# Excalibur1224/Cuda-v-MPI

Hardware: AMD Instinct MI355X
Metric: Riemann subintervals/sec at N=1e9 fp64; |error| vs analytic π (higher is better)
Workload: dtype fp64

## Files before the change

csrc/cli/miint.cpp:

```cpp
#include <algorithm>
#include <cmath>
#include <cstdio>
#include <string>
#include <vector>

#include "cli_common.hpp"
#include "miint/integrator.hpp"
#include "miint/oracle.hpp"
#include "miint/table2d.hpp"
#include "miint/trainscan.hpp"

using namespace miint;

namespace {

struct BenchRow {
  std::string integrand, dtype, rule;
  double n = 0, result = 0, exact = 0, ms = 0;
  int gpus = 1;
  int block = 0, grid = 0;
  bool multistep = false, close_in_launch = false, allreduce_to_host = false;
  BatchDiag diag;
  std::string timeline_file;
  std::string timeline_work;
// ... 200 lines not shown
}

int comm_sweep(const cli::Args& a, const cli::Topology& topo, double max_bytes, int iters) {
  std::vector<size_t> counts;
  for (size_t c = 1; c * 8.0 <= max_bytes; c *= 8) counts.push_back(c);
  if (counts.empty() || counts.back() * 8.0 < max_bytes) counts.push_back(static_cast<size_t>(max_bytes / 8));
  const char* ops[] = {"allreduce", "allgather", "broadcast"};
  std::vector<double> ms(counts.size() * 3, 0.0);
  std::mutex mu;
  auto body = [&](int , int dev, const Comm* comm) {
    DeviceGuard g(dev);
    Stream s;
    RankAgree agree(comm);
    const size_t cmax = counts.back();
    DeviceBuffer<double> a(cmax), b(cmax * static_cast<size_t>(comm->world()));
    MIINT_HIP(hipMemsetAsync(a.get(), 0, a.bytes(), s.get()));
    Event e0, e1;
    for (size_t k = 0; k < counts.size(); ++k)
      for (int op = 0; op < 3; ++op) {
        auto issue = [&] {
          if (op == 0) comm->allreduce_sum(a.get(), b.get(), counts[k], s.get());
          else if (op == 1) comm->allgather(a.get(), b.get(), counts[k], s.get());
          else comm->broadcast(a.get(), counts[k], 0, s.get());
        };
        for (int w = 0; w < 3; ++w) issue();
        s.sync();
        agree.barrier();
        e0.record(s.get());
        for (int i = 0; i < iters; ++i) issue();
        e1.record(s.get());
        e1.sync();
        comm->check_async();
        const double t = agree.max(Event::elapsed_ms(e0, e1) / iters);
        std::lock_guard<std::mutex> l(mu);
        ms[k * 3 + op] = std::max(ms[k * 3 + op], t);
      }
  };
  capture_rccl_log();
  if (!topo.multiproc && topo.world == 1) {
    auto one = RcclComm::init_all({0});
    body(0, 0, one[0].get());
  } else {
    cli::run_ranks(topo, body);
  }
  if (topo.rank0 != 0) return 0;
  const double P = topo.world;
  const RcclTransport tr = rccl_transport();
  const bool share = ranks_share_devices() && topo.world > 1;
  const std::string terr = transport_error(
      tr, topo.world, topo.multiproc ? cli::env_int("LOCAL_WORLD_SIZE", topo.world) : topo.world,
      share);
  if (!terr.empty()) std::fprintf(stderr, "miint comm: transport check: %s\n", terr.c_str());
  for (size_t k = 0; k < counts.size(); ++k)
    for (int op = 0; op < 3; ++op) {
      const double bytes = counts[k] * 8.0 * (op == 1 ? P : 1.0);
      const double t = ms[k * 3 + op];
      const double alg = bytes / (t * 1e-3) / 1e9;
      const double factor = op == 0 ? 2.0 * (P - 1) / P : (op == 1 ? (P - 1) / P : 1.0);
      cli::emit(a, cli::JsonRecord()
                       .add("op", ops[op])
                       .add("gpus", topo.world)
                       .add("bytes", bytes)
                       .add("us", t * 1e3)
                       .add("algbw_GBps", alg)
                       .add("busbw_GBps", alg * factor)
                       .add("ranks_share_gpus", ranks_share_devices() && topo.world > 1)
                       .add("rccl_transport", tr.transport)
                       .add("rccl_nnodes", tr.nnodes)
                       .add("transport_verified", terr.empty()),
                true);
    }
  return 0;
}

}

constexpr const char* kUsage =
    "usage: miint info\n"
    "       miint bench [--integrand pi4] [--n 1e9] [--dtype fp64|fp32|fp32acc] [--rule left]\n"
    "                   [--iters 200] [--gpus G] [--div series_exact|series|ieee] [--unfused] [--no-graph]\n"
    "                   [--block B] [--grid G] [--step-streams S] [--trig-library] [--settle N]\n"
    "                   [--no-multistep] [--slots K] [--close auto|kernel|launch] [--no-ar-host]\n"
    "                   [--work auto|static|queue] [--queue-wg-per-cu W]\n"
    "                   [--diagnose] [--slice R/W] [--timeline FILE]\n"
    "                   (--timeline: after the timed run, one batch from the timeline build of\n"
    "                   the multi-step launch, per-workgroup device-clock stamps as JSON in FILE;\n"
    "                   read it with tools/timeline_report.py. --slice: rank R's share of W)\n"
    "       miint sweep [--gpus G]\n"
    "       miint table2d [--grid 4096] [--gpus G] [--slice R/W] [--no-graph]\n"
    "                     [--step-streams S] [--min-wg W] [--settle-ms MS] [--no-multistep]\n"
    "                     [--phases P] [--graph-steps K]\n"
    "       miint selfcheck\n"
    "       miint comm [--gpus G] [--max-bytes 144e6] [--iters 20]\n"
    "Every record is one JSON line on stdout; --jsonl FILE also appends it to FILE.\n";

int main(int argc, char** argv) {
  try {
    cli::Args a(argc, argv);
    if (cli::usage_requested(a, kUsage)) return 0;
    const std::string cmd = a.positional().empty() ? "info" : a.positional()[0];
    if (cmd == "info") {
      const int nd = device_count();
      std::printf("miint: %d HIP device(s), RCCL %s\n", nd, nd ? RcclComm::version().c_str() : "-");
      for (int d = 0; d < nd; ++d) {
        const DeviceInfo i = device_info(d);
        std::printf("  [%d] %s %s  %d CUs  %.1f GHz  %.1f GB  L2 %d KB  LDS %zu KB/CU (%zu KB/block)\n",
                    d, i.name.c_str(), i.arch.c_str(), i.num_cus, i.clock_khz / 1e6,
                    i.total_mem / 1e9, i.l2_bytes / 1024, i.lds_per_cu / 1024,
                    i.lds_per_block / 1024);
      }
      return 0;
    }
    if (cmd == "selfcheck") return selfcheck();
    {
      int r = 0, w = 0;
      cli::parse_slice(a, &r, &w);
    }
    const cli::Topology topo = cli::topology(a);
    const int iters = static_cast<int>(a.integer("iters", 100));
    const bool graphs = !a.flag("no-graph");
    if (cmd == "bench") {
      RiemannConfig c = make_cfg(a.str("integrand", "pi4"), a.num("n", 1e9), a.str("dtype", "fp64"),
                                 a.str("rule", "left"), a.str("div", "series_exact"));
      c.fused = !a.flag("unfused");
      c.grid = static_cast<int>(a.integer("grid", 0));
      c.block = static_cast<int>(a.integer("block", kRiemannBlock));
      c.step_streams = static_cast<int>(a.integer("step-streams", 0));
      c.multistep = !a.flag("no-multistep");
      c.slots = static_cast<int>(a.integer("slots", c.slots));
      c.close = a.str("close", c.close);
      c.work = a.str("work", c.work);
      c.queue_wg_per_cu = static_cast<int>(a.integer("queue-wg-per-cu", 0));
      c.allreduce_to_host = !a.flag("no-ar-host");
      cli::parse_slice(a, &c.slice_rank, &c.slice_world);
      TimelineRequest tl;
      tl.file = a.str("timeline", "");
      tl.integrand = a.str("integrand", "pi4");
      tl.dtype = a.str("dtype", "fp64");
      tl.div = a.str("div", "series_exact");
      if (!tl.file.empty() && c.close == "launch")
        fail(std::string("--timeline: ") + kTimelineNoCloseInLaunch, __FILE__, __LINE__);
      if (a.flag("trig-library")) set_trig_library(true);
      MIINT_CHECK(riemann_block_ok(c.block), "--block must be 64, 128, 256, 512 or 1024");
      c.waves_per_cu = static_cast<int>(a.integer("waves-per-cu", 32));
      const BenchRow r = bench_one(topo, c, iters, graphs,
                                   static_cast<int>(a.integer("settle", -1)),
                                   a.flag("diagnose"), tl);
      if (topo.rank0 == 0)
        print_row(a, r, a.str("integrand", "pi4").c_str(), a.str("dtype", "fp64").c_str(),
                  a.str("rule", "left").c_str());
      return 0;
    }
    if (cmd == "table2d") {
      Table2DConfig c;
      c.grid = static_cast<int>(a.integer("grid", 4096));
      c.bucket = !a.flag("no-bucket");
      c.chain = !a.flag("no-chain");
      c.step_streams = static_cast<int>(a.integer("step-streams", 0));
      c.min_wg = static_cast<int>(a.integer("min-wg", 0));
      c.settle_ms = a.num("settle-ms", c.settle_ms);
      c.multistep = !a.flag("no-multistep");
      c.phases = static_cast<int>(a.integer("phases", 0));
      c.graph_steps = static_cast<int>(a.integer("graph-steps", 0));
      cli::parse_slice(a, &c.rank, &c.world);
      double value = 0.0, timed = 0.0, ms = 0.0;
      bool bucketed = false, chained = false, multistep = false;
      int streams = 1, phases = 0, resident = 0, min_wg = 0, wgs = 0, gsteps = 0;
      cli::RankFacts facts;
      std::mutex mu;
      cli::run_ranks(topo, [&](int rank, int dev, const Comm* comm) {
        Table2DPlan plan(c, dev, comm);
        RankAgree agree(comm);
        const double v = plan.run();
        const double t = agree.max(plan.time(iters, graphs));
        std::lock_guard<std::mutex> g(mu);
        if (rank == topo.rank0) {
          facts.note(comm);
          value = v;
          timed = plan.last_result();
          bucketed = plan.bucketed() && graphs;
          chained = plan.chained() && graphs;
          multistep = plan.multistep() && graphs;
          streams = chained ? plan.step_streams() : 1;
          phases = multistep ? plan.phases() : 0;
          resident = plan.resident_per_cu();
          min_wg = plan.min_wg();
          wgs = plan.workgroups();
          gsteps = graphs ? plan.graph_steps() : 0;
        }
        if (t > ms) ms = t;
      });
      if (topo.rank0 == 0) {
        cli::JsonRecord r;
        r.add("program", "table2d").add("grid", c.grid);
        r.add("step_streams", streams).add("multistep", multistep).add("phases", phases);
        r.add("resident_per_cu", resident).add("min_wg", min_wg).add("workgroups", wgs);
        r.add("graph_steps", gsteps);
        facts.add(r, topo);
        if (c.world > 1) {
          r.add("slice", std::to_string(c.rank) + "/" + std::to_string(c.world))
              .add("partial", value);
        } else {
          const double want = table2d_oracle(c.grid);
          const double exact = 122000.004 * 122000.004;
          r.add("gpus", topo.world)
              .add("result", value)
              .add("timed_result", timed)
              .add("bucketed_allreduce", bucketed)
              .add("chained", chained)
              .add("midpoint_oracle", want)
              .add("rel_err_vs_oracle", std::fabs(value - want) / want)
              .add("rel_err_vs_exact", std::fabs(value - exact) / exact)
              .add("samples_per_s", static_cast<double>(c.grid) * c.grid / (ms * 1e-3));
        }
// ... 29 lines not shown
```

csrc/include/miint/common.hpp:

```cpp
#pragma once

#include <hip/hip_runtime.h>

#include <cstdint>
#include <stdexcept>
#include <string>

namespace miint {

struct Error : std::runtime_error {
  using std::runtime_error::runtime_error;
};

[[noreturn]] inline void fail(const std::string& what, const char* file, int line) {
  throw Error(std::string(file) + ":" + std::to_string(line) + ": " + what);
}

}

#define MIINT_HIP(expr)                                                                     \
  do {                                                                                      \
    hipError_t miint_e_ = (expr);                                                           \
    if (miint_e_ != hipSuccess)                                                             \
      ::miint::fail(std::string(#expr) + " -> " + hipGetErrorString(miint_e_), __FILE__,    \
                    __LINE__);                                                              \
  } while (0)

#define MIINT_CHECK(cond, msg)                                                   \
  do {                                                                           \
    if (!(cond)) ::miint::fail(std::string("check failed: ") + (msg), __FILE__, __LINE__); \
  } while (0)

namespace miint {

enum class Integrand : int {
  kPi4 = 0,
  kSin = 1,
  kPoly = 2,
  kTrainVel = 3,
  kTable = 4,
};

enum class Rule : int { kLeft = 0, kMid = 1, kRight = 2 };

enum class DivMode : int { kSeries = 0, kIeee = 1, kSeriesDirect = 2, kSeriesExact = 3 };

inline double rule_offset(Rule r) {
  return r == Rule::kLeft ? 0.0 : (r == Rule::kMid ? 0.5 : 1.0);
}

constexpr int kMaxPolyCoeffs = 16;

constexpr int kSinTrig = 28;

struct RiemannParams {
  double a;
  double h;
  double off;
  uint64_t i_begin;
  uint64_t n;
  int integrand;
  int ncoef;
  double coef[kMaxPolyCoeffs];
  double coef_h[kMaxPolyCoeffs];
  double p0, p1;
  double trig[kSinTrig];
  float trig32[kSinTrig];
};

}
```

csrc/include/miint/integrands.hpp:

```cpp
#pragma once

#include <hip/hip_runtime.h>

#include "miint/common.hpp"
#include "miint/fast_trig.hpp"

namespace miint {

template <class D>
struct TileDefaults {
  template <DivMode M>
  __host__ __device__ static constexpr int tile_len() { return 32; }
  template <int U, DivMode M>
  __device__ static constexpr double anchor() { return 0.0; }
  template <int U, DivMode M>
  __device__ __forceinline__ double tile_acc(double x0, double h, double acc) const {
    return acc + static_cast<const D*>(this)->template tile<U, M>(x0, h);
  }
};

struct Pi4 : TileDefaults<Pi4> {
  static constexpr double kScale = 4.0;
  static constexpr int kPairs = 16;
  static constexpr int kSub = 2 * kPairs;
// ... 229 lines not shown
#pragma unroll
      for (int q = 0; q < kSubs; ++q) {
        const int i = q < kSubs / 2 ? kSubs / 2 - 1 - q : q - kSubs / 2;
        if (q < kSubs / 2) {
          ecs[i] = centres_f32(sf, i);
          aqs[i] = slopes_f32(sf, i);
        }
        if (q == 0) subtile_squares<true, true>(t2, tb, aqs[i], ecs[i]);
        else if (q < kSubs / 2) subtile_squares<true, false>(t2, tb, aqs[i], ecs[i]);
        else subtile_squares<false, false>(t2, tb, aqs[i], ecs[i]);
      }
      t2 += tb;
#else
#pragma unroll
      for (int q = 0; q < kSubs; ++q) {
        const int i = q < kSubs / 2 ? kSubs / 2 - 1 - q : q - kSubs / 2;
        if (q < kSubs / 2) {
          ecs[i] = centres_f32(sf, i);
          aqs[i] = slopes_f32(sf, i);
        }
        const float ecq = q < kSubs / 2 ? ecs[i].y : ecs[i].x;
        const float aq = q < kSubs / 2 ? aqs[i].y : aqs[i].x;
        const f32x2 ec = {ecq, ecq}, a = {aq, aq};
#pragma unroll
        for (int j = 0; j < kPairs; ++j) {
          const f32x2 e = __builtin_elementwise_fma(pkf[j], a, ec);
          t2 = __builtin_elementwise_fma(e, e, t2);
          asm volatile("" : "+v"(t2));
        }
      }
#endif
      const double t = lin + (static_cast<double>(t2.x) + static_cast<double>(t2.y));
      return fma(sd.s, t, fma(sd.s, static_cast<double>(U), acc));
    } else {
      return acc + tile<U, M>(xa, h);
    }
  }

  __device__ __forceinline__ double series_exact_point(double xm, double h, int u) const {
    const Seed sd = seed_exact(xm, h);
    const double b2 = 2.0 * sd.b;
    const int q = u / kSub, w = u % kSub;
    const double ec = centre_g(sd, q);
    const double a = centre_slope(sd, b2, q);
    const int j = w >= kSub / 2 ? w - kSub / 2 : kSub / 2 - 1 - w;
    const double kj = w >= kSub / 2 ? pk[j] : -pk[j];
    const double e = fma(kj, a, fma(fma(kj, kj, -kMeanK2), sd.b, ec));
    const SeedF32 sf = seed_f32(sd);
    const int i = q < kSubs / 2 ? kSubs / 2 - 1 - q : q - kSubs / 2;
    const f32x2 ecs = centres_f32(sf, i), aqs = slopes_f32(sf, i);
    const float e_sq = fmaf(static_cast<float>(kj), q < kSubs / 2 ? aqs.y : aqs.x,
                            q < kSubs / 2 ? ecs.y : ecs.x);
    const float sq = e_sq * e_sq;
    return fma(sd.s, e + static_cast<double>(sq), sd.s);
  }

  __device__ __forceinline__ double series_point(double xm, double h, int u) const {
    const Seed sd = seed_half(xm, h);
    const double b2 = 2.0 * sd.b;
    const int q = u / kSub, w = u % kSub;
    const double eh = centre_g(sd, q);
    const double a = centre_slope(sd, b2, q);
    const int j = w >= kSub / 2 ? w - kSub / 2 : kSub / 2 - 1 - w;
    const double c = fma(pk2[j], sd.b, eh);
    const double g = w >= kSub / 2 ? fma(pk[j], a, c) : fma(-pk[j], a, c);
    return sd.s * fma(g, g, 0.75);
  }
};

struct Pi4Wide : TileDefaults<Pi4Wide> {
  static constexpr double kScale = 4.0;
  __device__ __forceinline__ double point(double x) const { return 1.0 / fma(x, x, 1.0); }
  template <int U, DivMode M>
  __device__ __forceinline__ double tile(double x0, double h) const {
    static_assert(M == DivMode::kIeee, "wide-domain Pi4 runs IEEE division only");
    double acc = 0.0;
#pragma unroll
    for (int u = 0; u < U; ++u) acc += point(fma(static_cast<double>(u), h, x0));
    return acc;
  }
};
constexpr double kPi4NarrowMaxX = 0x1p249;

__device__ __forceinline__ void tile_sincos(double th, double& S, double& C) {
  constexpr double kTwoOverPi = 6.36619772367581382433e-01;
  constexpr double kPio2Hi = 1.57079632673412561417e+00;
  constexpr double kPio2Lo = 6.07710050650619224932e-11;
  const double n = rint(th * kTwoOverPi);
  const double r = fma(-n, kPio2Lo, fma(-n, kPio2Hi, th));
  const int q = static_cast<int>(n);
  const double z = r * r, w = z * z;
  const double s26 = fma(z, fma(z, fma(z, fma(z, 1.58969099521155010221e-10,
                                                -2.50507602534068634195e-08),
                                           2.75573137070700676789e-06),
                                      -1.98412698298579493134e-04),
                         8.33333333332248946124e-03);
  const double sr = fma(r * z, fma(z, s26, -1.66666666666666324348e-01), r);
  const double c13 = fma(z, fma(z, 2.48015872894767294178e-05, -1.38888888888741095749e-03),
                         4.16666666666666019037e-02);
  const double c46 = fma(z, fma(z, -1.13596475577881948265e-11, 2.08757232129817482790e-09),
                         -2.75573143513906633035e-07);
  const double rc = fma(w * w, c46, z * c13);
  const double hz = 0.5 * z, cw = 1.0 - hz;
  const double cc = cw + (((1.0 - cw) - hz) + z * rc);
  const bool swap = (q & 1) != 0;
  const double a = swap ? cc : sr, b = swap ? sr : cc;
  S = (q & 2) ? -a : a;
  C = ((q + 1) & 2) ? -b : b;
}

template <int Subs>
struct AngleSeries {
  static constexpr int kPairs = 8;
  static constexpr int kSub = 2 * kPairs;
  static constexpr int kSubs = Subs;
  static constexpr int kSeriesTile = kSub * kSubs;
  static_assert(2 * kPairs + kSubs <= kSinTrig, "RiemannParams::trig layout");
  double ck[kPairs], sk[kPairs];
  double cc[kSubs / 2], sc[kSubs / 2];

  __device__ __forceinline__ void init_trig(const double* trig) {
#pragma unroll
    for (int j = 0; j < kPairs; ++j) {
      ck[j] = trig[j];
      sk[j] = trig[kPairs + j];
    }
#pragma unroll
    for (int i = 0; i < kSubs / 2; ++i) {
      cc[i] = trig[2 * kPairs + 2 * i];
      sc[i] = trig[2 * kPairs + 2 * i + 1];
    }
  }
  __device__ __forceinline__ void centre(double S, double C, int q, double& Sq,
                                         double& Cq) const {
    const int i = q < kSubs / 2 ? kSubs / 2 - 1 - q : q - kSubs / 2;
    const double c = cc[i], s = q < kSubs / 2 ? -sc[i] : sc[i];
    Sq = fma(C, s, S * c);
    Cq = fma(-S, s, C * c);
  }
  template <bool COS>
  __device__ __forceinline__ double tile_sum(double theta_m) const {
    double S, C;
    tile_sincos(theta_m, S, C);
    double t = 0.0;
#pragma unroll
    for (int q = 0; q < kSubs; ++q) {
      double Sq, Cq;
      centre(S, C, q, Sq, Cq);
      const double base = COS ? Cq : Sq, side = COS ? -Sq : Cq;
#pragma unroll
      for (int j = 0; j < kPairs; ++j) {
        const double u = base * ck[j];
        t += fma(side, sk[j], u);
        t += fma(-side, sk[j], u);
        asm volatile("" : "+v"(t));
      }
    }
    return t;
  }
  template <bool COS>
  __device__ __forceinline__ double point_of(double theta_m, int u) const {
    double S, C, Sq, Cq;
    tile_sincos(theta_m, S, C);
    const int q = u / kSub, w = u % kSub;
    centre(S, C, q, Sq, Cq);
    const double base = COS ? Cq : Sq, side = COS ? -Sq : Cq;
// ... 420 lines not shown
```

csrc/include/miint/integrator.hpp:

```cpp
#pragma once

#include <hip/hip_runtime.h>

#include <cstdint>
#include <map>
#include <memory>
#include <string>
#include <vector>

#include "miint/comm.hpp"
#include "miint/common.hpp"
#include "miint/kernels.hpp"
#include "miint/runtime.hpp"

namespace miint {

constexpr int kAutoStepStreams = 4;
constexpr uint64_t kStepStreamsMaxCount = 600000000ull;

struct RiemannConfig {
  Integrand integrand = Integrand::kPi4;
  double a = 0.0, b = 1.0;
  uint64_t n = 1000000000ull;
  Rule rule = Rule::kLeft;
  DType dtype = DType::kF64;
  DivMode div = DivMode::kSeriesExact;
  std::vector<double> coef;
  double p0 = 0.0, p1 = 0.0;
  std::vector<double> table;
  int grid = 0;
  int block = kRiemannBlock;
  int waves_per_cu = 32;
  bool fused = true;
  bool chain = true;
  bool host_direct = true;
  int slots = 16;
  bool bucket = true;
  int rank = 0, world = 1;
  bool force_collective = false;
  bool multistep = true;
  std::string close = "auto";
  std::string work = "auto";
  int queue_wg_per_cu = 0;
  bool allreduce_to_host = true;
  int step_streams = 0;
  int slice_rank = 0, slice_world = 0;
  double timeout_s = 300.0;
};

inline std::string resolve_work(const std::string& work, const char* env, bool pays,
                                bool keeps_static = false) {
  MIINT_CHECK(work == "auto" || work == "static" || work == "queue",
              "work must be auto, static or queue (got " + work + ")");
  if (keeps_static) return "static";
  if (work != "auto") return work;
  if (env && *env) {
    const std::string e(env);
    MIINT_CHECK(e == "static" || e == "queue", "MIINT_MS_WORK must be static or queue (got " + e + ")");
    return e;
  }
  return pays ? "queue" : "static";
}

inline void rank_slice(uint64_t n, int r, int w, uint64_t* begin, uint64_t* count) {
  const uint64_t q = n / static_cast<uint64_t>(w), rem = n % static_cast<uint64_t>(w);
  const uint64_t ur = static_cast<uint64_t>(r);
  *count = q + (ur < rem ? 1 : 0);
  *begin = ur * q + (ur < rem ? ur : rem);
}

struct StepTiming {
  double wall_s = 0.0;
  double device_ms = 0.0;
  int steps = 0;
};

struct OneShotTiming {
  std::string mode;
  int reps = 0;
  double median_us = 0.0, min_us = 0.0, max_us = 0.0;
  double device_median_us = 0.0, device_min_us = 0.0;
  double value = 0.0;
};

struct BatchDiag {
  int steps = 0;
  double compute_us = 0.0;
  double close_us = 0.0;
  double allreduce_us = 0.0;
  double copy_us = 0.0;
  double marker_us = 0.0;
  double device_us = 0.0;
  double staged_us = 0.0;
  double wall_us = 0.0;
  double tail_us() const { return close_us + allreduce_us + copy_us; }
  double boundary_us() const { return device_us - compute_us - tail_us(); }
};

struct BatchTimeline {
  int steps = 0, grid = 0, block = 0;
  int clock_khz = 0;
  std::vector<uint64_t> stamps;
  std::vector<uint64_t> shader_clock;
  std::vector<uint32_t> hw;
  double device_us = 0.0;
  std::vector<double> values;
  std::string work = "static";
  int workgroups = 0;
  std::vector<uint64_t> wg_stamps;
  std::vector<uint64_t> item_stamp;
  std::vector<uint32_t> item_owner;
};
constexpr uint64_t kTimelineUnsetStamp = 0;
constexpr uint32_t kTimelineUnsetId = 0xffffffffu;

class RiemannPlan {
 public:
  RiemannPlan(const RiemannConfig& cfg, int device, const Comm* comm = nullptr);
  ~RiemannPlan();
  RiemannPlan(const RiemannPlan&) = delete;
  RiemannPlan& operator=(const RiemannPlan&) = delete;

  const RiemannConfig& config() const { return cfg_; }
  int device() const { return device_; }
  int rank() const { return rank_; }
  int world() const { return world_; }
  uint64_t begin() const { return params_.i_begin; }
  uint64_t count() const { return params_.n; }
  double h() const { return params_.h; }
  double scale() const { return scale_; }
  LaunchShape shape() const { return shape_; }
  DivMode effective_div() const;
  bool direct() const { return direct_; }

  void enqueue_compute(hipStream_t s, int slot, int host_index) const;
  void enqueue_reduce(hipStream_t s, int slot) const;
  void enqueue_copyout(hipStream_t s, int slot, int host_index) const;
  void enqueue(hipStream_t s, int slot, int host_index) const;

  double* device_result(int slot) const { return result_.get() + slot; }
  double host_result(int host_index) const { return host_[host_index]; }
  int host_capacity() const { return static_cast<int>(host_.size()); }
  int slots() const { return cfg_.slots; }

  double run();
  void capture_graphs();
  void prepare_steps(int steps);
  bool graphs_ready() const { return !graphs_.empty() && graph_error_.empty(); }
  const std::string& graph_error() const { return graph_error_; }
  size_t graph_nodes() const;
  long graph_launches() const { return graph_launches_; }
  long direct_steps() const { return direct_steps_; }

  StepTiming run_steps(int steps, bool pipeline, bool graphs);
  BatchDiag diagnose_batch(int nsteps);
  BatchTimeline timeline_batch(int nsteps, const std::string& form = "auto");
  void barrier();
  OneShotTiming time_one_shot(int reps, const std::string& mode, int warmup = 400);
  void launch_steps(int steps, bool pipeline, bool graphs);
  void sync() const;
  int host_index_of(int k, bool graphs) const;
  hipStream_t compute_stream() const { return compute_.get(); }
  hipStream_t comm_stream() const { return comm_stream_.get(); }

  bool collective() const { return comm_ && (world_ > 1 || cfg_.force_collective); }
  bool bucketed() const { return collective() && cfg_.bucket; }
  bool chained() const { return cfg_.fused && cfg_.chain && (!collective() || bucketed()); }
  bool multistep() const { return chained() && multistep_; }
  bool close_in_launch() const { return multistep() && close_launch_; }
  const char* work() const { return multistep() && work_queue_ ? "queue" : "static"; }
  int queue_workgroups() const { return multistep() && work_queue_ ? queue_wgs_ : 0; }
  bool allreduce_to_host() const {
    return bucketed() && cfg_.allreduce_to_host && ar_host_ok_;
  }
  void check_allreduce_to_host();

 private:
  void enqueue_batch(hipStream_t cs, hipStream_t rs, int nsteps, bool overlap);
  void enqueue_bucket_reduce(hipStream_t s, int nsteps) const;
  void enqueue_chain(hipStream_t s, int nsteps) const;
  void enqueue_chain_streams(hipStream_t cs, int nsteps);
 public:
  int step_streams(int nsteps) const;
 private:
  const Graph* batch_graph(int nsteps);
  bool use_graphs(bool requested, int steps);
  double* result_ptr(int j) const { return direct_ ? host_.device_ptr() + j : result_.get() + j; }

  RiemannConfig cfg_;
  int device_;
  const Comm* comm_;
  int rank_ = 0, world_ = 1;
  bool direct_ = false;
  RiemannParams params_{};
  double scale_ = 1.0;
  LaunchShape shape_{1, kRiemannBlock};
  DeviceBuffer<double> partials_;
  DeviceBuffer<double> slots_;
  DeviceBuffer<double> ms_partials_;
  bool multistep_ = false;
  bool close_launch_ = false;
  bool capturing_ = false;
  bool ar_host_ok_ = true;
  bool ar_host_checked_ = false;
  DeviceBuffer<unsigned int> ms_ticket_;
  bool work_queue_ = false;
  int queue_wgs_ = 0;
  DeviceBuffer<unsigned int> queue_;
  void reset_queue() const;
  void enqueue_multistep(hipStream_t s, int nsteps, bool close_kernel) const;
  DeviceBuffer<uint64_t> qtl_item_stamp_, qtl_wg_stamps_, qtl_shader_;
  DeviceBuffer<uint32_t> qtl_item_owner_, qtl_hw_;
  DeviceBuffer<uint64_t> tl_stamps_, tl_shader_;
  DeviceBuffer<uint32_t> tl_hw_;
  DeviceBuffer<double> result_;
  DeviceBuffer<double> sync_;
  DeviceBuffer<unsigned int> ticket_;
  DeviceBuffer<double> table_;
  PinnedBuffer<double> host_;
  Stream compute_;
  Stream comm_stream_;
  std::vector<Stream> step_streams_;
  std::vector<std::unique_ptr<Event>> ev_step_join_;
  std::vector<std::unique_ptr<Event>> ev_computed_, ev_drained_;
  Event ev_fork_, ev_join_;
  Event ev_t0_, ev_t1_;
  std::map<int, std::unique_ptr<Graph>> graphs_;
  std::string graph_error_;
  long graph_launches_ = 0, direct_steps_ = 0;
  int last_mode_ = -1;
};

}
```

csrc/include/miint/kernels.hpp:

```cpp
#pragma once

#include <hip/hip_runtime.h>

#include <algorithm>
#include <cmath>
#include <cstddef>
#include <cstdint>

#include "miint/common.hpp"

namespace miint {

enum class DType : int { kF64 = 0, kF32 = 1, kF32Acc32 = 2 };
inline bool is_fp32(DType t) { return t == DType::kF32 || t == DType::kF32Acc32; }

constexpr int kRiemannTile = 32;
constexpr int kRiemannBlock = 256;
constexpr int kSeriesHalfSpan = 192;
constexpr int kSeriesHalfSpanF32 = 96;

constexpr int kDirectHalfSpan = 16;

inline bool series_ok(double h) { return kSeriesHalfSpan * (h < 0 ? -h : h) <= 2e-6; }
inline bool series_ok_f32(double h) { return kSeriesHalfSpanF32 * (h < 0 ? -h : h) <= 2e-6; }
inline bool direct_ok(double h) { return kDirectHalfSpan * (h < 0 ? -h : h) <= 2e-6; }

inline DivMode effective_div(DivMode d, double h) {
  if (d == DivMode::kIeee) return d;
  if ((d == DivMode::kSeries || d == DivMode::kSeriesExact) && series_ok(h)) return d;
  return direct_ok(h) ? DivMode::kSeriesDirect : DivMode::kIeee;
}
inline bool series_request(DivMode d) { return d == DivMode::kSeries || d == DivMode::kSeriesExact; }
inline DivMode effective_div(DivMode d, double h, Integrand f) {
  if (f == Integrand::kSin || f == Integrand::kTrainVel || f == Integrand::kTable)
    return series_request(d) ? DivMode::kSeries : DivMode::kIeee;
  if (f != Integrand::kPi4) return DivMode::kIeee;
  return effective_div(d, h);
}

constexpr int kPolySeriesMaxCoeffs = 8;

inline DivMode effective_div(DivMode d, double h, Integrand f, DType t, int ncoef = 0) {
  if (is_fp32(t)) {
    if (d == DivMode::kIeee) return DivMode::kIeee;
    if (f == Integrand::kPi4) return series_ok_f32(h) ? DivMode::kSeries : DivMode::kIeee;
    if (f == Integrand::kPoly)
      return (ncoef >= 1 && ncoef <= kPolySeriesMaxCoeffs) ? DivMode::kSeries : DivMode::kIeee;
    return DivMode::kSeries;
  }
  if (f == Integrand::kPoly)
    return (series_request(d) && ncoef >= 1 && ncoef <= kPolySeriesMaxCoeffs)
               ? DivMode::kSeries
               : DivMode::kIeee;
  return effective_div(d, h, f);
}

constexpr double kTrigSeriesMaxN = 2147418112.0;
inline bool trig_series_in_range(const RiemannParams& p) {
  const Integrand f = static_cast<Integrand>(p.integrand);
  if (f != Integrand::kSin && f != Integrand::kTrainVel) return true;
  const double first = static_cast<double>(p.i_begin) + p.off;
  const double last = static_cast<double>(p.i_begin + (p.n > 0 ? p.n - 1 : 0)) + p.off;
  const double w = f == Integrand::kTrainVel ? 1.0 / p.p0 : 1.0;
  const double n0 = std::fabs(std::fma(first, p.h, p.a) * w) * 6.36619772367581382433e-01;
  const double n1 = std::fabs(std::fma(last, p.h, p.a) * w) * 6.36619772367581382433e-01;
  return n0 <= kTrigSeriesMaxN && n1 <= kTrigSeriesMaxN;
}
constexpr double kPi4SeriesMaxX = 0x1p249;
constexpr double kPi4SeriesMaxXF32 = 0x1p62;
inline bool pi4_series_in_range(const RiemannParams& p, DType t) {
  if (static_cast<Integrand>(p.integrand) != Integrand::kPi4) return true;
  const double lim = is_fp32(t) ? kPi4SeriesMaxXF32 : kPi4SeriesMaxX;
  const double first = static_cast<double>(p.i_begin) + p.off;
  const double last = static_cast<double>(p.i_begin + (p.n > 0 ? p.n - 1 : 0)) + p.off;
  return std::fabs(std::fma(first, p.h, p.a)) < lim && std::fabs(std::fma(last, p.h, p.a)) < lim;
}
inline bool poly_series_in_range(const RiemannParams& p) {
  if (static_cast<Integrand>(p.integrand) != Integrand::kPoly) return true;
  if (!(std::isfinite(p.h) && p.h != 0.0 && std::isfinite(1.0 / p.h))) return false;
  long double hp = 1.0L;
  for (int i = 0; i < p.ncoef && i < kMaxPolyCoeffs; ++i) {
    const double cs = static_cast<double>(static_cast<long double>(p.coef[i]) * hp);
    if (p.coef[i] != 0.0 && !std::isnormal(cs)) return false;
    hp *= static_cast<long double>(p.h);
  }
  return true;
}
inline DivMode effective_div(const RiemannParams& p, DivMode d, DType t) {
  const DivMode e = effective_div(d, p.h, static_cast<Integrand>(p.integrand), t, p.ncoef);
  return (e != DivMode::kIeee &&
          !(trig_series_in_range(p) && pi4_series_in_range(p, t) && poly_series_in_range(p)))
             ? DivMode::kIeee
             : e;
}

struct LaunchShape {
  int grid;
  int block;
};

bool riemann_block_ok(int block);
LaunchShape default_riemann_shape(int num_cus, int waves_per_cu = 32, int block = kRiemannBlock);

void launch_riemann_partials(const RiemannParams& p, DType dtype, DivMode div,
                             LaunchShape shape, const double* table, int table_n,
                             double* partials, hipStream_t stream);

void launch_finalize(const double* partials, int n, double scale, double* out,
                     hipStream_t stream, int block = kRiemannBlock);

constexpr unsigned kUnsetSlotWord = 0xFFFAFFFAu;
void fill_unset_slots(double* p, size_t count, hipStream_t stream);

constexpr int kTicketGroups = 16;
constexpr int kTicketStride = 64;
constexpr int kTicketWords = (kTicketGroups + 1) * kTicketStride;

void launch_riemann_fused(const RiemannParams& p, DType dtype, DivMode div, LaunchShape shape,
                          const double* table, int table_n, double* partials,
                          unsigned int* ticket, double scale, double* out, hipStream_t stream);

void launch_riemann_chained(const RiemannParams& p, DType dtype, DivMode div, LaunchShape shape,
                            const double* table, int table_n, double* partials,
                            const double* prev, int nprev, double scale, double* out_prev,
                            hipStream_t stream);

constexpr int kMaxMultiSteps = 64;
int riemann_multistep_grid(const RiemannParams& p, DType dtype, DivMode div, int block,
                           int num_cus, bool close = false);
void launch_riemann_multistep(const RiemannParams& p, DType dtype, DivMode div,
                              LaunchShape shape, const double* table, int table_n,
                              double* partials, int steps, double scale, double* out,
                              hipStream_t stream, unsigned int* ticket = nullptr,
                              bool close_kernel = true);
constexpr const char* kTimelineNoCloseInLaunch =
    "the timeline instruments the kernel-closed multi-step launch only (not close = launch)";
int riemann_timeline_grid(const RiemannParams& p, DType dtype, DivMode div, int block,
                          int num_cus);
void launch_riemann_timeline(const RiemannParams& p, DType dtype, DivMode div,
                             LaunchShape shape, const double* table, int table_n,
                             double* partials, int steps, double scale, double* out,
                             hipStream_t stream, uint64_t* stamps, uint64_t* shader_clock,
                             uint32_t* hw, unsigned int* ticket = nullptr,
                             bool close_kernel = true);
constexpr int kQueueWords = 2 * kTicketStride;
struct QueueTimeline {
  uint64_t* item_stamp;
  uint32_t* item_owner;
  uint64_t* wg_stamps;
  uint64_t* shader_clock;
  uint32_t* hw;
};
int riemann_queue_grid(const RiemannParams& p, DType dtype, DivMode div, int block, int num_cus,
                       bool timeline = false);
bool riemann_queue_pays(const RiemannParams& p, DType dtype, DivMode div);
void launch_riemann_queue(const RiemannParams& p, DType dtype, DivMode div, LaunchShape shape,
                          int workgroups, const double* table, int table_n, double* partials,
                          int steps, double scale, double* out, hipStream_t stream,
                          unsigned int* queue, bool close_kernel = true,
                          const QueueTimeline* timeline = nullptr);
void launch_multistep_close(const double* partials, int grid, int steps, double scale,
                            double* out, int block, hipStream_t stream);

void launch_riemann_point_values(const RiemannParams& p, DivMode div, const double* table,
                                 int table_n, double* out, hipStream_t stream);

void launch_pi4_recip_narrow(const double* d, uint64_t n, double* out, hipStream_t stream);
void launch_pi4_recip_narrow_f32(const float* d, uint64_t n, float* out, hipStream_t stream);
void set_pi4_library_division(bool on);
bool pi4_ieee_narrow(const RiemannParams& p, DType dtype);
void set_trig_library(bool on);
void set_lds_poison(bool on);
void set_lds_poison_trainscan(bool on);
void set_lds_poison_table(bool on);

int riemann_tile_len(const RiemannParams& p, DType dtype, DivMode div);

double integrand_scale(Integrand f);

int default_reduce_grid(int num_cus);
void launch_sum_array(const double* x, uint64_t n, double scale, double* partials, int grid,
                      double* out, hipStream_t stream);

void launch_interp_fill(const double* table, int table_n, double dt, uint64_t i0, uint64_t n,
                        double* y, hipStream_t stream);

size_t scan_state_bytes(uint64_t n);
void launch_inclusive_scan(const double* in, double* out, uint64_t n, void* state,
                           const double* carry_in, hipStream_t stream);
void launch_interp_scan(const double* table, int table_n, double dt, uint64_t i0, uint64_t n,
                        double* out, void* state, const double* carry_in, hipStream_t stream);
void launch_interp_scan_window(const double* table, int table_n, double dt, uint64_t i0,
                               uint64_t n, uint64_t win_lo, uint64_t win_hi, double* out,
                               void* state, const double* carry_in, hipStream_t stream);
unsigned scan_timeout_flag(const void* state, hipStream_t stream);
void launch_add_carry(double* x, uint64_t n, const double* carry, hipStream_t stream);

struct Table2DParams {
  const double* table;
  int nx, ny;
  double X, Y;
  int gx, gy;
  int row0, row1;
  int min_wg = 0;
};
int table2d_grid(const Table2DParams& p);
const char* table2d_path(const Table2DParams& p);
struct Table2DShapeInfo {
  bool stream;
  int rows_per_wave, tile_rows, tile_cols, grid_x, grid_y, tile;
};
Table2DShapeInfo table2d_shape_info(const Table2DParams& p);
constexpr int kT2AutoPhases = 16;
constexpr long kT2AutoWorkgroups = 4096;
constexpr int kT2MaxPhases = 32;
constexpr int kT2MaxReplaySteps = 1024;
bool table2d_multistep_ok(const Table2DParams& p, int num_cus);
int table2d_multistep_resident(const Table2DParams& p);
int table2d_multistep_phases(const Table2DParams& p, int num_cus, int steps, int want = 0);
void launch_table2d_multistep(const Table2DParams& p, double* partials, int steps, double* outs,
                              hipStream_t stream, int phases = 1);
void launch_table2d_partials(const Table2DParams& p, double* partials, hipStream_t stream);
void launch_table2d_fused(const Table2DParams& p, double* partials, unsigned* ticket,
                          double* out, hipStream_t stream);
void launch_table2d_chained(const Table2DParams& p, double* partials, const double* prev,
                            double* prev_out, hipStream_t stream);
void launch_table2d_finalize(const double* partials, int n, double* out, hipStream_t stream);
void launch_outer_product(const double* v, int n, double* table, hipStream_t stream);

}
```

csrc/kernels/riemann.hip:

```cpp
#include <hip/hip_runtime.h>

#include <atomic>
#include <cmath>
#include <string>

#include "miint/common.hpp"
#include "miint/handoff.hpp"
#include "miint/integrands.hpp"
#include "miint/integrands_f32.hpp"
#include "miint/kernels.hpp"
#include "miint/wave_reduce.hpp"

namespace miint {
namespace {

constexpr int B = kRiemannBlock;
constexpr int kMaxBlock = 1024;

__device__ __forceinline__ uint64_t readlane_u64(uint64_t v, int lane) {
  const uint32_t lo = __builtin_amdgcn_readlane(static_cast<uint32_t>(v), lane);
  const uint32_t hi = __builtin_amdgcn_readlane(static_cast<uint32_t>(v >> 32), lane);
  return (static_cast<uint64_t>(hi) << 32) | lo;
}

template <class F> struct AccOf { using type = double; };

struct TileSplit {
  uint64_t lanes, q;
  uint32_t bs, rem;
};
template <int T>
__device__ __forceinline__ TileSplit tile_split(uint64_t n) {
  const uint32_t bs = blockDim.x;
  const uint64_t lanes = static_cast<uint64_t>(gridDim.x) * bs;
  const uint64_t ntile = n / T;
  const uint64_t q = ntile / lanes;
  return {lanes, q, bs, static_cast<uint32_t>(ntile - q * lanes)};
}

template <DivMode M, class F>
__device__ __forceinline__ typename AccOf<F>::type lane_sum(const RiemannParams& p, const F& f,
                                                            unsigned block, const TileSplit& sp) {
  using Acc = typename AccOf<F>::type;
  constexpr int T = F::template tile_len<M>();
  const uint64_t lanes = sp.lanes;
  const uint32_t b0 = block * sp.bs;
  const uint32_t g32 = b0 + threadIdx.x;
  const uint64_t gid = g32;
  const uint32_t w0 =
      b0 + static_cast<uint32_t>(__builtin_amdgcn_readfirstlane(threadIdx.x / kWave)) * kWave;
  const bool all_extra = w0 + (kWave - 1) < sp.rem;
  const bool extra = !all_extra && g32 < sp.rem;
  const double base = static_cast<double>(p.i_begin) + p.off;
  const double istep = static_cast<double>(lanes * T);
  double ib = base + static_cast<double>(gid * T) + F::template anchor<T, M>();
  Acc acc = 0;
  for (uint64_t left = readlane_u64(sp.q + (all_extra ? 1 : 0), 0); left != 0; --left, ib += istep)
    acc = f.template tile_acc<T, M>(fma(ib, p.h, p.a), p.h, acc);
  if (extra) acc = f.template tile_acc<T, M>(fma(ib, p.h, p.a), p.h, acc);
  const uint64_t done = (sp.q * lanes + sp.rem) * T;
  for (uint64_t k = gid; k < p.n - done; k += lanes)
    acc += static_cast<Acc>(f.point(fma(base + static_cast<double>(done + k), p.h, p.a)));
  return acc;
}
template <DivMode M, class F>
__device__ __forceinline__ typename AccOf<F>::type lane_sum(const RiemannParams& p, const F& f,
                                                            unsigned block) {
  return lane_sum<M>(p, f, block, tile_split<F::template tile_len<M>()>(p.n));
}

constexpr int kMaxTable = 2048;


struct Pi4F32 : TileDefaults<Pi4F32> {
  static constexpr double kScale = 4.0;
  __device__ __forceinline__ double point(double xd) const {
    const float x = static_cast<float>(xd);
    return static_cast<double>(1.0f / fmaf(x, x, 1.0f));
  }
  __device__ __forceinline__ static f32x2 recip_narrow(f32x2 d) {
    const f32x2 one = {1.0f, 1.0f};
    const f32x2 nd = -d;
    f32x2 r = {__builtin_amdgcn_rcpf(d.x), __builtin_amdgcn_rcpf(d.y)};
    r = pk_fma(pk_fma(nd, r, one), r, r);
    const f32x2 q = pk_fma(pk_fma(nd, r, one), r, r);
    return pk_fma(pk_fma(nd, q, one), r, q);
// ... 111 lines not shown
      acc0 += 1.0f / fmaf(xa, xa, 1.0f);
      acc1 += 1.0f / fmaf(xb, xb, 1.0f);
    }
    return static_cast<double>(acc0) + static_cast<double>(acc1);
  }
  template <int UU, DivMode M>
  __device__ __forceinline__ double tile_acc(double x0d, double h, double acc) const {
    return acc + tile<UU, M>(x0d, h);
  }
};
constexpr double kPi4F32NarrowMaxX = 0x1p49;

struct Pi4F32Acc32 : Pi4F32 {
  template <int UU, DivMode M>
  __device__ __forceinline__ float tile_acc(double xmd, double h, float acc) const {
    if constexpr (M == DivMode::kSeries) {
      static_assert(UU == kSubs * kSubLen, "fp32 series tiles are kSubs 32-sample sub-tiles");
      const float xm = static_cast<float>(xmd);
      const float hf = static_cast<float>(h);
      const float dm = fmaf(xm, xm, 1.0f);
      float s = __builtin_amdgcn_rcpf(dm);
      s = fmaf(s, fmaf(-dm, s, 1.0f), s);
      const float em = fmaf(-dm, s, 1.0f);
      const float a = (-2.0f * hf) * xm * s;
      const float b = -(hf * hf) * s;
      const f32x2 bb = {b, b};
      const f32x2 aa = {a, a};
      const f32x2 emv = {em, em};
      f32x2 ecs[kSubs / 2], aqs[kSubs / 2];
#pragma unroll
      for (int p2 = 0; p2 < kSubs / 2; ++p2) {
        const f32x2 c0v = {(2 * p2 - 0.5f * (kSubs - 1)) * kSubLen,
                           (2 * p2 + 1 - 0.5f * (kSubs - 1)) * kSubLen};
        ecs[p2] = pk_fma(c0v, pk_fma(c0v, bb, aa), emv);
        aqs[p2] = pk_fma(c0v + c0v, bb, aa);
      }
      f32x2 t, t1;
#pragma unroll
      for (int q = 0; q < kSubs; ++q) {
        const float ec = (q & 1) ? ecs[q / 2].y : ecs[q / 2].x;
        const float aq = (q & 1) ? aqs[q / 2].y : aqs[q / 2].x;
        const f32x2 av = {aq, aq};
        f32x2 cc = pk_fma(f32x2{0.25f, 2.25f}, bb, f32x2{ec, ec});
#pragma unroll
        for (int j = 0; j < kSubLen / 2; j += 2) {
          const f32x2 k0 = {j + 0.5f, -(j + 0.5f)};
          const f32x2 k1 = {j + 1.5f, -(j + 1.5f)};
          const f32x2 e0 = pk_fma(k0, av, f32x2{cc.x, cc.x});
          const f32x2 e1 = pk_fma(k1, av, f32x2{cc.y, cc.y});
          if (q == 0 && j == 0) {
            t = e0;
            t1 = e1;
          } else {
            t += e0;
            t1 += e1;
          }
          if (j + 2 < kSubLen / 2)
            cc = pk_fma(f32x2{4.0f * j + 6.0f, 4.0f * j + 10.0f}, bb, cc);
        }
      }
      t += t1;
      return fmaf(s, static_cast<float>(UU) + (t.x + t.y), acc);
    } else {
      const float x0 = static_cast<float>(xmd);
      const float hf = static_cast<float>(h);
      const f32x2 xb = {x0, x0}, hh = {hf, hf}, one = {1.0f, 1.0f};
      f32x2 a2 = {0.0f, 0.0f};
#pragma unroll
      for (int u = 0; u < UU; u += 2) {
        const f32x2 uu = {static_cast<float>(u), static_cast<float>(u + 1)};
        const f32x2 x = pk_fma(uu, hh, xb);
        a2 += recip_narrow(pk_fma(x, x, one));
      }
      return acc + (a2.x + a2.y);
    }
  }
};
template <> struct AccOf<Pi4F32Acc32> { using type = float; };

static_assert(2 * AngleSeries<12>::kPairs + 12 == kSinTrig, "trig table sized for Sin");
static_assert(Pi4::kSeriesTile / 2 == kSeriesHalfSpan &&
                  Pi4F32::kSubs * Pi4F32::kSubLen / 2 == kSeriesHalfSpanF32,
              "kSeriesHalfSpan(F32) must be half the Pi4 series tile lengths");

template <class F> struct Maker;
template <> struct Maker<Pi4> {
  static constexpr int kLds = 1;
  __device__ static Pi4 make(const RiemannParams&, const double*, int, double*) {
    Pi4 f;
    f.init();
    return f;
  }
};
template <> struct Maker<Pi4Wide> {
  static constexpr int kLds = 1;
  __device__ static Pi4Wide make(const RiemannParams&, const double*, int, double*) { return {}; }
};
template <> struct Maker<Pi4F32Wide> {
  static constexpr int kLds = 1;
  __device__ static Pi4F32Wide make(const RiemannParams&, const double*, int, double*) {
    return {};
  }
};
template <> struct Maker<Pi4F32Acc32> {
  static constexpr int kLds = 1;
  __device__ static Pi4F32Acc32 make(const RiemannParams&, const double*, int, double*) {
    return {};
  }
};
template <> struct Maker<Pi4F32> {
  static constexpr int kLds = 1;
  __device__ static Pi4F32 make(const RiemannParams&, const double*, int, double*) { return {}; }
};
template <> struct Maker<Sin> {
  static constexpr int kLds = 1;
  __device__ static Sin make(const RiemannParams& p, const double*, int, double*) {
    Sin f;
    f.init(p.trig);
    return f;
  }
};
template <> struct Maker<SinLib> {
  static constexpr int kLds = 1;
  __device__ static SinLib make(const RiemannParams&, const double*, int, double*) { return {}; }
};
template <int NC> struct Maker<Poly<NC>> {
  static constexpr int kLds = 1;
  __device__ static Poly<NC> make(const RiemannParams& p, const double*, int, double*) {
    Poly<NC> f;
    f.init(p.coef, p.ncoef);
    return f;
  }
};
template <> struct Maker<TrainVel> {
  static constexpr int kLds = 1;
  __device__ static TrainVel make(const RiemannParams& p, const double*, int, double*) {
    TrainVel f;
    f.init_trig(p.trig);
    f.inv_ts = 1.0 / p.p0;
    f.vs = p.p1;
    return f;
  }
};
template <> struct Maker<TrainVelLib> {
  static constexpr int kLds = 1;
  __device__ static TrainVelLib make(const RiemannParams& p, const double*, int, double*) {
    TrainVelLib f;
    f.inv_ts = 1.0 / p.p0;
    f.vs = p.p1;
    return f;
  }
};
template <> struct Maker<SinF32> {
  static constexpr int kLds = 1;
  __device__ static SinF32 make(const RiemannParams& p, const double*, int, double*) {
    SinF32 f;
    f.init(p.trig32);
    return f;
  }
};
template <> struct Maker<TrainVelF32> {
  static constexpr int kLds = 1;
  __device__ static TrainVelF32 make(const RiemannParams& p, const double*, int, double*) {
    TrainVelF32 f;
    f.init_trig(p.trig32);
    f.inv_ts = 1.0 / p.p0;
    f.vs = p.p1;
    return f;
  }
};
template <int NC> struct Maker<PolyF32<NC>> {
  static constexpr int kLds = 1;
// ... 406 lines not shown
  unsigned* done = queue + kTicketStride;
  unsigned c = 0;
  if (threadIdx.x == 0) c = queue_claim(head);
  if (!one_wave) {
    if (threadIdx.x == 0) next_item[1] = c;
    __syncthreads();
    c = next_item[1];
  }
  unsigned i = __builtin_amdgcn_readfirstlane(c);
  unsigned sbase = 0;
  for (unsigned seq = 0; i < total; ++seq) {
    unsigned nxt = 0;
    if (threadIdx.x == 0) nxt = queue_claim(head);
    while (i - sbase >= nb) sbase += nb;
    const unsigned vb = i - sbase;
    RiemannParams q = p;
    asm volatile("" : "+s"(q.a));
    const Acc l = lane_sum<M>(q, f, vb, sp);
    asm volatile("" : "+v"(nxt));
    if (!one_wave && threadIdx.x == 0) next_item[seq & 1] = nxt;
    double v;
    if constexpr (__is_same(Acc, double)) v = block_sum_dyn(l, red[seq & 1]);
    else v = static_cast<double>(block_sum_dyn(l, red_acc[seq & 1]));
    if (threadIdx.x == 0) {
      if constexpr (TL) {
        unsigned wg = blockIdx.x;
        asm volatile("" : "+v"(wg));
        tl.item_stamp[i] = timeline_realtime_after(v);
        tl.item_owner[i] = wg;
      }
      partials[i] = v;
    }
    i = __builtin_amdgcn_readfirstlane(one_wave ? nxt : next_item[seq & 1]);
  }
  if (threadIdx.x == 0) {
    if constexpr (TL) {
      const unsigned long long t = timeline_realtime();
      unsigned long long* clk = timeline_row(tl.shader_clock, 2);
      clk[0] = te.clk;
      clk[1] = timeline_shader_clock();
      unsigned long long* st = timeline_row(tl.wg_stamps, 2);
      st[0] = te.t;
      st[1] = t;
      unsigned xcc, hw;
      asm volatile("s_getreg_b32 %0, hwreg(HW_REG_XCC_ID)" : "=s"(xcc));
      asm volatile("s_getreg_b32 %0, hwreg(HW_REG_HW_ID)" : "=s"(hw));
      unsigned* id = timeline_row(tl.hw, 2);
      id[0] = xcc;
      id[1] = hw;
    }
    const unsigned d = __hip_atomic_fetch_add(done, 1u, __ATOMIC_RELAXED, __HIP_MEMORY_SCOPE_AGENT);
    if (d == gridDim.x - 1) {
      __hip_atomic_store(head, 0u, __ATOMIC_RELAXED, __HIP_MEMORY_SCOPE_AGENT);
      __hip_atomic_store(done, 0u, __ATOMIC_RELAXED, __HIP_MEMORY_SCOPE_AGENT);
    }
  }
}
template <DivMode M, class F>
__global__ __launch_bounds__(kMaxBlock) void riemann_queue_kernel(
    RiemannParams p, const double* table, int table_n, double* partials, int steps, unsigned nb,
    unsigned* queue) {
  queue_body<M, F>(p, table, table_n, partials, steps, nb, queue);
}
template <DivMode M, class F>
__global__ __launch_bounds__(kMaxBlock) kFullOccupancy void riemann_queue_kernel_o8(
    RiemannParams p, const double* table, int table_n, double* partials, int steps, unsigned nb,
    unsigned* queue) {
  queue_body<M, F>(p, table, table_n, partials, steps, nb, queue);
}
template <DivMode M, class F>
__global__ __launch_bounds__(kMaxBlock) void riemann_queue_timeline_kernel(
    RiemannParams p, const double* table, int table_n, double* partials, int steps, unsigned nb,
    unsigned* queue, QueueTimelineOut tl) {
  queue_body<M, F, true>(p, table, table_n, partials, steps, nb, queue, tl);
}
template <DivMode M, class F>
__global__ __launch_bounds__(kMaxBlock) kFullOccupancy void riemann_queue_timeline_kernel_o8(
    RiemannParams p, const double* table, int table_n, double* partials, int steps, unsigned nb,
    unsigned* queue, QueueTimelineOut tl) {
  queue_body<M, F, true>(p, table, table_n, partials, steps, nb, queue, tl);
}
template <DivMode M, class F>
constexpr bool queue_pays() {
  return M == DivMode::kSeriesExact && __is_same(F, Pi4);
}

__global__ __launch_bounds__(kMaxBlock) void multistep_close_kernel(const double* partials,
                                                                   int nb, double scale,
                                                                   double* out) {
  __shared__ double red[kMaxBlock / kWave];
  const double t = ordered_partials<0, false>(partials + static_cast<size_t>(blockIdx.x) * nb, nb);
  const double tot = block_sum_dyn(t, red);
  if (threadIdx.x == 0) out[blockIdx.x] = tot * scale;
}

template <DivMode M, class F>
__global__ __launch_bounds__(B) void point_values_kernel(RiemannParams p, const double* table,
                                                         int table_n, double* out) {
  constexpr int T = F::template tile_len<M>();
  __shared__ double lds[lds_words<M, F>()];
  const F f = make_functor<M, F>(p, table, table_n, lds);
  const uint64_t t = static_cast<uint64_t>(blockIdx.x) * B + threadIdx.x;
  if (t * T >= p.n) return;
  const double x0 = fma(static_cast<double>(p.i_begin) + p.off + static_cast<double>(t * T),
                        p.h, p.a);
  const double xm = fma(0.5 * (T - 1), p.h, x0);
  const bool full = (t + 1) * T <= p.n;
  for (int u = 0; u < T && t * T + u < p.n; ++u) {
    const double x = fma(static_cast<double>(u), p.h, x0);
    double v;
    if constexpr (M == DivMode::kSeries && __is_same(F, Pi4)) {
      v = full ? f.series_point(xm, p.h, u) : f.point(x);
    } else if constexpr (M == DivMode::kSeriesExact && __is_same(F, Pi4)) {
      v = full ? f.series_exact_point(xm, p.h, u) : f.point(x);
    } else if constexpr (M == DivMode::kSeries && IsPolyF64<F>::value) {
      v = full ? f.series_point(xm, u) : f.point(x);
    } else if constexpr (M == DivMode::kSeries && __is_same(F, Table)) {
      v = full ? f.series_point(xm, p.h, u) : f.point(x);
    } else if constexpr (M == DivMode::kSeries && (__is_same(F, Sin) || __is_same(F, TrainVel))) {
      v = full ? f.series_point(xm, u) : f.point(x);
    } else if constexpr (M == DivMode::kSeriesDirect && __is_same(F, Pi4)) {
      const Pi4::Seed sd = Pi4::seed(xm, p.h);
      const double e = fma(-fma(x, x, 1.0), sd.s, 1.0);
      v = fma(sd.s, e + e * e, sd.s);
    } else if constexpr (M == DivMode::kIeee && __is_same(F, Pi4)) {
      v = full ? Pi4::recip_narrow(fma(x, x, 1.0)) : f.point(x);
    } else if constexpr (M == DivMode::kIeee &&
                         (__is_same(F, Sin) || __is_same(F, SinLib) ||
                          __is_same(F, TrainVel) || __is_same(F, TrainVelLib))) {
      v = full ? f.template ieee_point<T>(x0, p.h, u) : f.point(x);
    } else {
      v = f.point(x);
    }
    out[t * T + u] = v * F::kScale;
  }
}

__global__ __launch_bounds__(B) void recip_narrow_kernel(const double* d, uint64_t n,
                                                         double* out) {
  const uint64_t stride = static_cast<uint64_t>(gridDim.x) * B;
  for (uint64_t i = static_cast<uint64_t>(blockIdx.x) * B + threadIdx.x; i < n; i += stride)
    out[i] = Pi4::recip_narrow(d[i]);
}
__global__ __launch_bounds__(B) void recip_narrow_f32_kernel(const float* d, uint64_t n,
                                                             float* out) {
  const uint64_t stride = static_cast<uint64_t>(gridDim.x) * B;
  for (uint64_t i = static_cast<uint64_t>(blockIdx.x) * B + threadIdx.x; i < n; i += stride)
    out[i] = Pi4F32::recip_narrow(f32x2{d[i], d[i]}).x;
}

template <DivMode M, class F>
void launch_partials_t(const RiemannParams& p, LaunchShape shape, const double* table,
                       int table_n, double* partials, hipStream_t stream) {
  if constexpr (occupancy_hint<M, F>())
    riemann_kernel_o8<M, F><<<shape.grid, shape.block, 0, stream>>>(p, table, table_n, partials);
  else
    riemann_kernel<M, F><<<shape.grid, shape.block, 0, stream>>>(p, table, table_n, partials);
}
template <DivMode M, class F>
void launch_fused_t(const RiemannParams& p, LaunchShape shape, const double* table, int table_n,
                    double* partials, unsigned* ticket, double scale, double* out,
                    hipStream_t stream) {
  if constexpr (occupancy_hint<M, F>())
    riemann_fused_kernel_o8<M, F>
        <<<shape.grid, shape.block, 0, stream>>>(p, table, table_n, partials, ticket, scale, out);
  else
    riemann_fused_kernel<M, F>
        <<<shape.grid, shape.block, 0, stream>>>(p, table, table_n, partials, ticket, scale, out);
}

template <DivMode M, class F>
void launch_chained_t(const RiemannParams& p, LaunchShape shape, const double* table,
                      int table_n, double* partials, const double* prev, int nprev, double scale,
                      double* out_prev, hipStream_t stream) {
  if constexpr (occupancy_hint<M, F>())
    riemann_chained_kernel_o8<M, F><<<shape.grid, shape.block, 0, stream>>>(p, table, table_n, partials,
                                                                  prev, nprev, scale, out_prev);
  else
    riemann_chained_kernel<M, F><<<shape.grid, shape.block, 0, stream>>>(p, table, table_n, partials,
                                                               prev, nprev, scale, out_prev);
}

template <DivMode M, class F, bool CLOSE>
void launch_multistep_c(const RiemannParams& p, LaunchShape shape, const double* table,
                        int table_n, double* partials, int steps, unsigned rot,
                        unsigned* ticket, double scale, double* out, hipStream_t stream) {
  if constexpr (multistep_o8<M, F>())
    riemann_multistep_kernel_o8<M, F, CLOSE><<<shape.grid, shape.block, 0, stream>>>(
        p, table, table_n, partials, steps, rot, ticket, scale, out);
  else
    riemann_multistep_kernel<M, F, CLOSE><<<shape.grid, shape.block, 0, stream>>>(
        p, table, table_n, partials, steps, rot, ticket, scale, out);
}
template <DivMode M, class F>
void launch_multistep_t(const RiemannParams& p, LaunchShape shape, const double* table,
                        int table_n, double* partials, int steps, unsigned rot,
                        unsigned* ticket, double scale, double* out, hipStream_t stream) {
  if constexpr (multistep_pays<M, F>()) {
    if constexpr (multistep_close_ok<M, F>()) {
      if (ticket) {
        launch_multistep_c<M, F, true>(p, shape, table, table_n, partials, steps, rot, ticket,
                                       scale, out, stream);
        return;
      }
    } else {
      MIINT_CHECK(ticket == nullptr, "this integrand closes multi-step batches by a kernel");
    }
    launch_multistep_c<M, F, false>(p, shape, table, table_n, partials, steps, rot, ticket,
                                    scale, out, stream);
  } else {
    fail("this integrand/division keeps chained batches (no multi-step kernel)", __FILE__,
         __LINE__);
  }
}
template <DivMode M, class F, bool CLOSE>
int multistep_occupancy(int block) {
  int n = 0;
  if constexpr (multistep_o8<M, F>())
    MIINT_HIP(hipOccupancyMaxActiveBlocksPerMultiprocessor(
        &n, reinterpret_cast<const void*>(&riemann_multistep_kernel_o8<M, F, CLOSE>), block, 0));
  else
    MIINT_HIP(hipOccupancyMaxActiveBlocksPerMultiprocessor(
        &n, reinterpret_cast<const void*>(&riemann_multistep_kernel<M, F, CLOSE>), block, 0));
  return n;
}
template <DivMode M, class F>
// ... 3 lines not shown
  else if constexpr (!multistep_close_ok<M, F>())
    *out = close ? 0 : multistep_occupancy<M, F, false>(block);
  else
    *out = close ? multistep_occupancy<M, F, true>(block) : multistep_occupancy<M, F, false>(block);
}

template <DivMode M, class F>
void launch_timeline_t(const RiemannParams& p, LaunchShape shape, const double* table,
                       int table_n, double* partials, int steps, unsigned rot, TimelineOut tl,
                       hipStream_t stream) {
  if constexpr (!multistep_pays<M, F>())
    fail("this integrand/division keeps chained batches (no multi-step kernel, no timeline)",
         __FILE__, __LINE__);
  else if constexpr (multistep_o8<M, F>())
    riemann_timeline_kernel_o8<M, F><<<shape.grid, shape.block, 0, stream>>>(
        p, table, table_n, partials, steps, rot, tl);
  else
    riemann_timeline_kernel<M, F><<<shape.grid, shape.block, 0, stream>>>(
        p, table, table_n, partials, steps, rot, tl);
}
template <DivMode M, class F>
void timeline_per_cu_t(int block, int* out) {
  *out = 0;
  if constexpr (multistep_pays<M, F>()) {
    if constexpr (multistep_o8<M, F>())
      MIINT_HIP(hipOccupancyMaxActiveBlocksPerMultiprocessor(
          out, reinterpret_cast<const void*>(&riemann_timeline_kernel_o8<M, F>), block, 0));
    else
      MIINT_HIP(hipOccupancyMaxActiveBlocksPerMultiprocessor(
          out, reinterpret_cast<const void*>(&riemann_timeline_kernel<M, F>), block, 0));
  }
}

template <DivMode M, class F>
void launch_queue_t(const RiemannParams& p, LaunchShape shape, int wgs, const double* table,
                    int table_n, double* partials, int steps, unsigned* queue,
                    const QueueTimelineOut* tl, hipStream_t stream) {
  const unsigned nb = static_cast<unsigned>(shape.grid);
  if constexpr (!multistep_pays<M, F>()) {
    fail("this integrand/division keeps chained batches (no multi-step kernel, no queue)",
         __FILE__, __LINE__);
  } else if constexpr (multistep_o8<M, F>()) {
    if (tl)
      riemann_queue_timeline_kernel_o8<M, F><<<wgs, shape.block, 0, stream>>>(
          p, table, table_n, partials, steps, nb, queue, *tl);
    else
      riemann_queue_kernel_o8<M, F><<<wgs, shape.block, 0, stream>>>(p, table, table_n, partials,
                                                                     steps, nb, queue);
  } else {
    if (tl)
      riemann_queue_timeline_kernel<M, F><<<wgs, shape.block, 0, stream>>>(
          p, table, table_n, partials, steps, nb, queue, *tl);
    else
      riemann_queue_kernel<M, F><<<wgs, shape.block, 0, stream>>>(p, table, table_n, partials,
                                                                  steps, nb, queue);
  }
}
template <DivMode M, class F>
void queue_per_cu_t(int block, bool timeline, int* out) {
  *out = 0;
  if constexpr (multistep_pays<M, F>()) {
    const void* k;
    if constexpr (multistep_o8<M, F>())
      k = timeline ? reinterpret_cast<const void*>(&riemann_queue_timeline_kernel_o8<M, F>)
                   : reinterpret_cast<const void*>(&riemann_queue_kernel_o8<M, F>);
    else
      k = timeline ? reinterpret_cast<const void*>(&riemann_queue_timeline_kernel<M, F>)
                   : reinterpret_cast<const void*>(&riemann_queue_kernel<M, F>);
    MIINT_HIP(hipOccupancyMaxActiveBlocksPerMultiprocessor(out, k, block, 0));
  }
}

std::atomic<bool> g_pi4_library_division{false};
std::atomic<bool> g_trig_library{false};
inline bool trig_library() { return g_trig_library.load(std::memory_order_relaxed); }
inline bool pi4_narrow(const RiemannParams& p, double max_x = kPi4NarrowMaxX) {
  if (g_pi4_library_division.load(std::memory_order_relaxed)) return false;
  const double first = static_cast<double>(p.i_begin) + p.off;
  const double last = static_cast<double>(p.i_begin + (p.n > 0 ? p.n - 1 : 0)) + p.off;
  return std::fabs(std::fma(first, p.h, p.a)) < max_x &&
         std::fabs(std::fma(last, p.h, p.a)) < max_x;
}

template <template <DivMode, class> class Op, class... A>
void dispatch(const RiemannParams& p, DType dtype, DivMode m, A&&... a) {
  const Integrand f = static_cast<Integrand>(p.integrand);
  if (dtype == DType::kF32Acc32) {
    MIINT_CHECK(f == Integrand::kPi4, "fp32 accumulation (fp32acc) is implemented for pi4 only");
    if (m == DivMode::kSeries) Op<DivMode::kSeries, Pi4F32Acc32>::run(a...);
    else if (pi4_narrow(p, kPi4F32NarrowMaxX)) Op<DivMode::kIeee, Pi4F32Acc32>::run(a...);
    else fail("fp32acc: coordinates beyond 2^49 need the wide division (use fp32)", __FILE__,
              __LINE__);
    return;
  }
  if (dtype == DType::kF32) {
    const bool ser = m == DivMode::kSeries;
    switch (f) {
      case Integrand::kPi4:
        if (ser) Op<DivMode::kSeries, Pi4F32>::run(a...);
        else if (pi4_narrow(p, kPi4F32NarrowMaxX)) Op<DivMode::kIeee, Pi4F32>::run(a...);
        else Op<DivMode::kIeee, Pi4F32Wide>::run(a...);
        return;
      case Integrand::kSin:
        if (ser) Op<DivMode::kSeries, SinF32>::run(a...);
        else if (!trig_series_in_range(p)) Op<DivMode::kIeee, Sin>::run(a...);
        else Op<DivMode::kIeee, SinF32>::run(a...);
        return;
      case Integrand::kTrainVel:
        if (ser) Op<DivMode::kSeries, TrainVelF32>::run(a...);
        else if (!trig_series_in_range(p)) Op<DivMode::kIeee, TrainVel>::run(a...);
        else Op<DivMode::kIeee, TrainVelF32>::run(a...);
        return;
      case Integrand::kTable:
        if (ser) Op<DivMode::kSeries, TableF32>::run(a...);
        else Op<DivMode::kIeee, TableF32>::run(a...);
        return;
      case Integrand::kPoly:
        if (ser && p.ncoef <= 4) Op<DivMode::kSeries, PolyF32<4>>::run(a...);
        else if (ser && p.ncoef <= 6) Op<DivMode::kSeries, PolyF32<6>>::run(a...);
        else if (ser && p.ncoef == 7) Op<DivMode::kSeries, PolyF32<7>>::run(a...);
        else if (ser && p.ncoef <= 8) Op<DivMode::kSeries, PolyF32<8>>::run(a...);
        else if (p.ncoef <= 4) Op<DivMode::kIeee, PolyF32<4>>::run(a...);
        else if (p.ncoef <= 8) Op<DivMode::kIeee, PolyF32<8>>::run(a...);
        else Op<DivMode::kIeee, PolyF32<16>>::run(a...);
        return;
    }
    fail("unknown integrand", __FILE__, __LINE__);
  }
  switch (f) {
    case Integrand::kPi4:
      if (m == DivMode::kSeries) Op<DivMode::kSeries, Pi4>::run(a...);
      else if (m == DivMode::kSeriesExact) Op<DivMode::kSeriesExact, Pi4>::run(a...);
      else if (m == DivMode::kSeriesDirect) Op<DivMode::kSeriesDirect, Pi4>::run(a...);
      else if (pi4_narrow(p)) Op<DivMode::kIeee, Pi4>::run(a...);
      else Op<DivMode::kIeee, Pi4Wide>::run(a...);
      return;
    case Integrand::kSin:
      if (m == DivMode::kSeries) Op<DivMode::kSeries, Sin>::run(a...);
      else if (trig_library()) Op<DivMode::kIeee, SinLib>::run(a...);
      else Op<DivMode::kIeee, Sin>::run(a...);
      return;
    case Integrand::kPoly:
      if (m == DivMode::kSeries && p.ncoef <= 4) Op<DivMode::kSeries, Poly<4>>::run(a...);
      else if (m == DivMode::kSeries && p.ncoef <= 6) Op<DivMode::kSeries, Poly<6>>::run(a...);
      else if (m == DivMode::kSeries && p.ncoef == 7) Op<DivMode::kSeries, Poly<7>>::run(a...);
      else if (m == DivMode::kSeries && p.ncoef <= 8) Op<DivMode::kSeries, Poly<8>>::run(a...);
      else if (p.ncoef <= 4) Op<DivMode::kIeee, Poly<4>>::run(a...);
      else if (p.ncoef <= 8) Op<DivMode::kIeee, Poly<8>>::run(a...);
      else Op<DivMode::kIeee, Poly<16>>::run(a...);
      return;
    case Integrand::kTrainVel:
      if (m == DivMode::kSeries) Op<DivMode::kSeries, TrainVel>::run(a...);
      else if (trig_library()) Op<DivMode::kIeee, TrainVelLib>::run(a...);
      else Op<DivMode::kIeee, TrainVel>::run(a...);
      return;
    case Integrand::kTable:
      if (m == DivMode::kSeries) Op<DivMode::kSeries, Table>::run(a...);
      else Op<DivMode::kIeee, Table>::run(a...);
      return;
  }
  fail("unknown integrand", __FILE__, __LINE__);
}

template <DivMode M, class F> struct PartialsOp {
  template <class... A> static void run(A... a) { launch_partials_t<M, F>(a...); }
};
template <DivMode M, class F> struct FusedOp {
  template <class... A> static void run(A... a) { launch_fused_t<M, F>(a...); }
};
template <DivMode M, class F> struct ChainedOp {
  template <class... A> static void run(A... a) { launch_chained_t<M, F>(a...); }
};
template <DivMode M, class F> struct MultiStepOp {
  template <class... A> static void run(A... a) { launch_multistep_t<M, F>(a...); }
};
template <DivMode M, class F> struct MultiStepOccOp {
  static void run(int block, bool close, int* out) { multistep_per_cu_t<M, F>(block, close, out); }
};
template <DivMode M, class F> struct TimelineOp {
  template <class... A> static void run(A... a) { launch_timeline_t<M, F>(a...); }
};
template <DivMode M, class F> struct TimelineOccOp {
  static void run(int block, int* out) { timeline_per_cu_t<M, F>(block, out); }
};
template <DivMode M, class F> struct QueueOp {
  template <class... A> static void run(A... a) { launch_queue_t<M, F>(a...); }
};
template <DivMode M, class F> struct QueueOccOp {
  static void run(int block, bool timeline, int* out) { queue_per_cu_t<M, F>(block, timeline, out); }
};
template <DivMode M, class F> struct QueuePaysOp {
  static void run(bool* out) { *out = multistep_pays<M, F>() && queue_pays<M, F>(); }
};
template <DivMode M, class F> struct TileLenOp {
  static void run(int* out) { *out = F::template tile_len<M>(); }
};
template <DivMode M, class F> struct PointsOp {
  static void run(const RiemannParams& p, const double* table, int table_n, double* out,
                  hipStream_t stream) {
    constexpr int T = F::template tile_len<M>();
    const uint64_t ntile = (p.n + T - 1) / T;
    const int grid = static_cast<int>((ntile + B - 1) / B);
    point_values_kernel<M, F><<<grid, B, 0, stream>>>(p, table, table_n, out);
  }
};

}

bool riemann_block_ok(int block) {
  return block == 64 || block == 128 || block == 256 || block == 512 || block == 1024;
}

LaunchShape default_riemann_shape(int num_cus, int waves_per_cu, int block) {
  MIINT_CHECK(riemann_block_ok(block), "unsupported Riemann block size");
// ... 165 lines not shown
  static_assert(sizeof(unsigned long long) == sizeof(uint64_t), "stamp words are 64-bit");
  const TimelineOut tl{reinterpret_cast<unsigned long long*>(stamps),
                       reinterpret_cast<unsigned long long*>(shader_clock), hw};
  dispatch<TimelineOp>(p, dtype, eff, prepared(p, eff), shape, table, table_n, partials, steps,
                       rot, tl, stream);
  MIINT_HIP(hipGetLastError());
  if (!close_kernel) return;
  launch_multistep_close(partials, shape.grid, steps, scale, out, shape.block, stream);
}

int riemann_queue_grid(const RiemannParams& p, DType dtype, DivMode div, int block, int num_cus,
                       bool timeline) {
  MIINT_CHECK(riemann_block_ok(block), "unsupported Riemann block size");
  int per_cu = 0;
  dispatch<QueueOccOp>(p, dtype, effective_div(p, div, dtype), block, timeline, &per_cu);
  return per_cu * num_cus;
}

bool riemann_queue_pays(const RiemannParams& p, DType dtype, DivMode div) {
  bool pays = false;
  dispatch<QueuePaysOp>(p, dtype, effective_div(p, div, dtype), &pays);
  return pays;
}

void launch_riemann_queue(const RiemannParams& p, DType dtype, DivMode div, LaunchShape shape,
                          int workgroups, const double* table, int table_n, double* partials,
                          int steps, double scale, double* out, hipStream_t stream,
                          unsigned int* queue, bool close_kernel, const QueueTimeline* timeline) {
  check_shape(shape);
  check_params(p, table, table_n);
  MIINT_CHECK(workgroups >= 1 && workgroups <= (1 << 20), "queue launch: workgroups out of range");
  MIINT_CHECK(steps >= 1 && steps <= kMaxMultiSteps, "queue launch: 1..64 steps");
  MIINT_CHECK(partials != nullptr && out != nullptr && queue != nullptr,
              "queue launch needs partials, results and the queue words");
  static_assert(sizeof(unsigned long long) == sizeof(uint64_t), "stamp words are 64-bit");
  QueueTimelineOut tl{};
  if (timeline) {
    MIINT_CHECK(timeline->item_stamp && timeline->item_owner && timeline->wg_stamps &&
                    timeline->shader_clock && timeline->hw,
                "queue timeline launch needs its five buffers");
    tl = {reinterpret_cast<unsigned long long*>(timeline->item_stamp), timeline->item_owner,
          reinterpret_cast<unsigned long long*>(timeline->wg_stamps),
          reinterpret_cast<unsigned long long*>(timeline->shader_clock), timeline->hw};
  }
  const DivMode eff = effective_div(p, div, dtype);
  dispatch<QueueOp>(p, dtype, eff, prepared(p, eff), shape, workgroups, table, table_n, partials,
                    steps, queue, timeline ? &tl : nullptr, stream);
  MIINT_HIP(hipGetLastError());
  if (!close_kernel) return;
  launch_multistep_close(partials, shape.grid, steps, scale, out, shape.block, stream);
}

void launch_multistep_close(const double* partials, int grid, int steps, double scale,
                            double* out, int block, hipStream_t stream) {
  MIINT_CHECK(steps >= 1 && steps <= kMaxMultiSteps && grid >= 1 && riemann_block_ok(block),
              "multi-step close: 1..64 steps, a Riemann block size");
  multistep_close_kernel<<<steps, block, 0, stream>>>(partials, grid, scale, out);
  MIINT_HIP(hipGetLastError());
}

void launch_riemann_point_values(const RiemannParams& p, DivMode div, const double* table,
                                 int table_n, double* out, hipStream_t stream) {
  check_params(p, table, table_n);
  MIINT_CHECK(p.n >= 1, "empty range");
  const DivMode eff = effective_div(p, div, DType::kF64);
  dispatch<PointsOp>(p, DType::kF64, eff, prepared(p, eff), table, table_n, out, stream);
  MIINT_HIP(hipGetLastError());
}

void set_pi4_library_division(bool on) { g_pi4_library_division.store(on); }
bool pi4_ieee_narrow(const RiemannParams& p, DType dtype) {
  return pi4_narrow(p, is_fp32(dtype) ? kPi4F32NarrowMaxX : kPi4NarrowMaxX);
}
void set_trig_library(bool on) { g_trig_library.store(on); }

void launch_pi4_recip_narrow(const double* d, uint64_t n, double* out, hipStream_t stream) {
  if (n == 0) return;
  const uint64_t blocks = (n + B - 1) / B;
  const int grid = static_cast<int>(blocks < 8192 ? blocks : 8192);
  recip_narrow_kernel<<<grid, B, 0, stream>>>(d, n, out);
  MIINT_HIP(hipGetLastError());
}

void launch_pi4_recip_narrow_f32(const float* d, uint64_t n, float* out, hipStream_t stream) {
  if (n == 0) return;
  const uint64_t blocks = (n + B - 1) / B;
  const int grid = static_cast<int>(blocks < 8192 ? blocks : 8192);
  recip_narrow_f32_kernel<<<grid, B, 0, stream>>>(d, n, out);
  MIINT_HIP(hipGetLastError());
}

}
```

csrc/python/module.cpp:

```cpp
#include <pybind11/numpy.h>
#include <pybind11/pybind11.h>
#include <pybind11/stl.h>

#include <algorithm>
#include <cmath>
#include <cstdint>
#include <string>
#include <vector>

#include "miint/comm.hpp"
#include "miint/expr.hpp"
#include "miint/fast_trig.hpp"
#include "miint/host.hpp"
#include "miint/integrator.hpp"
#include "miint/kernels.hpp"
#include "miint/oracle.hpp"
#include "miint/runtime.hpp"
#include "miint/selftest.hpp"
#include "miint/table2d.hpp"
#include "miint/trace.hpp"
#include "miint/trainscan.hpp"

namespace py = pybind11;
using namespace miint;

namespace {

template <typename T>
T* ptr(uintptr_t p) { return reinterpret_cast<T*>(p); }
hipStream_t stream(uintptr_t s) { return reinterpret_cast<hipStream_t>(s); }

RiemannParams make_params(int integrand, double a, double h, double off, uint64_t i_begin,
                          uint64_t n, const std::vector<double>& coef, double p0, double p1) {
  RiemannParams p{};
  p.a = a;
  p.h = h;
  p.off = off;
  p.i_begin = i_begin;
  p.n = n;
  p.integrand = integrand;
  MIINT_CHECK(coef.size() <= static_cast<size_t>(kMaxPolyCoeffs), "too many coefficients");
  p.ncoef = static_cast<int>(coef.size());
  for (size_t i = 0; i < coef.size(); ++i) p.coef[i] = coef[i];
  p.p0 = p0;
  p.p1 = p1;
  return p;
}

using ParamRows = py::object;
std::vector<double> param_rows(const ParamRows& obj, int nparams, uint64_t* rows) {
  auto arr = py::array_t<double, py::array::c_style | py::array::forcecast>::ensure(obj);
  if (!arr) {
    PyErr_Clear();
    fail("expression sweep: params must be K rows of " + std::to_string(nparams) +
             " numbers (a list of rows or a 2-D float64 array)", __FILE__, __LINE__);
  }
  if (arr.size() == 0 && arr.ndim() >= 1 && arr.shape(0) == 0) {
    *rows = 0;
    return {};
  }
  MIINT_CHECK(arr.ndim() == 2, "expression sweep: params must be 2-D (K rows x nparams)");
  MIINT_CHECK(arr.shape(1) == nparams,
              "expression sweep: rows of " + std::to_string(arr.shape(1)) +
                  " values, the expression was built for nparams = " + std::to_string(nparams));
  *rows = static_cast<uint64_t>(arr.shape(0));
  return std::vector<double>(arr.data(), arr.data() + arr.size());
}

template <class... A>
auto compiled(std::string (*compile)(A...)) {
  return [compile](A... a) {
    std::string code;
    {
      py::gil_scoped_release nogil;
      code = compile(a...);
    }
    return py::bytes(code);
  };
}

}

static const char* scan_algo_name(ScanAlgo a) {
  return a == ScanAlgo::kFused ? "fused" : a == ScanAlgo::kOnePass ? "onepass" : "lookback";
}
static ScanAlgo scan_algo_of(const std::string& s) {
  MIINT_CHECK(s == "fused" || s == "lookback" || s == "onepass",
              "algo must be onepass|fused|lookback");
  return s == "fused" ? ScanAlgo::kFused : s == "onepass" ? ScanAlgo::kOnePass : ScanAlgo::kLookback;
}

PYBIND11_MODULE(_miint, m) {
  m.doc() = "miint: MI355X-native numerical integration (HIP/gfx950 kernels, RCCL, hipGraph)";
  py::register_exception<miint::Error>(m, "MiintError", PyExc_RuntimeError);
  install_crash_handler_from_env();

  py::enum_<Integrand>(m, "Integrand")
      .value("pi4", Integrand::kPi4)
      .value("sin", Integrand::kSin)
      .value("poly", Integrand::kPoly)
      .value("train", Integrand::kTrainVel)
      .value("table", Integrand::kTable);
  py::enum_<Rule>(m, "Rule").value("left", Rule::kLeft).value("mid", Rule::kMid).value("right", Rule::kRight);
  py::enum_<DType>(m, "DType")
      .value("fp64", DType::kF64)
      .value("fp32", DType::kF32)
      .value("fp32acc", DType::kF32Acc32);
  py::enum_<DivMode>(m, "DivMode")
      .value("series", DivMode::kSeries)
      .value("ieee", DivMode::kIeee)
      .value("series_direct", DivMode::kSeriesDirect)
      .value("series_exact", DivMode::kSeriesExact);

  m.attr("TICKET_WORDS") = kTicketWords;
  m.attr("UNSET_SLOT_WORD") = kUnsetSlotWord;
  m.def("fill_unset_slots", [](uintptr_t p, size_t count, uintptr_t s) {
    fill_unset_slots(ptr<double>(p), count, stream(s));
  });
  m.attr("RIEMANN_TILE") = kRiemannTile;
  m.attr("RIEMANN_BLOCK") = kRiemannBlock;
  m.def("series_ok", &series_ok);
  m.def("series_ok_f32", &series_ok_f32);
  m.def("integrand_scale", &integrand_scale);

  m.def("device_count", &device_count);
  m.def("device_info", [](int d) {
    DeviceInfo i = device_info(d);
    py::dict r;
// ... 68 lines not shown
      .def_static("version", &RcclComm::version);
  py::class_<LoopbackComm, Comm>(m, "LoopbackComm");
  py::class_<LoopbackGroup, std::shared_ptr<LoopbackGroup>>(m, "LoopbackGroup",
      "W logical ranks on one device (test transport; drive rank r from its own thread)")
      .def(py::init(&LoopbackGroup::create), py::arg("world"), py::arg("device") = 0,
           py::arg("timeout_s") = 120.0)
      .def_property_readonly("world", &LoopbackGroup::world)
      .def_property_readonly("device", &LoopbackGroup::device)
      .def("comm", &LoopbackGroup::comm, py::arg("rank"), py::return_value_policy::reference_internal)
      .def("barrier", &LoopbackGroup::barrier, py::arg("rank"), py::call_guard<py::gil_scoped_release>())
      .def("mark_broken", &LoopbackGroup::mark_broken)
      .def_property_readonly("broken", &LoopbackGroup::broken)
      .def_property_readonly("collectives", &LoopbackGroup::collectives)
      .def_property_readonly("graph_launches", &LoopbackGroup::graph_launches);
  m.def(
      "rendezvous_unique_id",
      [](const std::string& addr, int port, int rank, int world, double timeout_s) {
        std::string id;
        {
          py::gil_scoped_release rel;
          id = rendezvous_unique_id(addr, port, rank, world, timeout_s);
        }
        return py::bytes(id);
      },
      py::arg("addr"), py::arg("port"), py::arg("rank"), py::arg("world"),
      py::arg("timeout_s") = 120.0);
  auto transport_dict = [](const RcclTransport& t) {
    py::dict d;
    d["transport"] = t.transport;
    d["nranks"] = t.nranks;
    d["nnodes"] = t.nnodes;
    d["local_ranks"] = t.local_ranks;
    d["connections"] = t.connections;
    d["comms"] = t.comms;
    d["uses_net"] = t.uses_net();
    d["log"] = t.log;
    return d;
  };
  m.def("parse_rccl_log", [transport_dict](const std::string& text) {
    return transport_dict(parse_rccl_log(text));
  });
  m.def("capture_rccl_log", &capture_rccl_log,
        "route RCCL's INIT log into a per-process file (call before the first RCCL call)");
  m.def("rccl_log_path", &rccl_log_path);
  m.def("rccl_transport", [transport_dict]() { return transport_dict(rccl_transport()); });
  m.def(
      "transport_error",
      [](const std::string& log_text, int world, int local_world, bool share) {
        return transport_error(parse_rccl_log(log_text), world, local_world, share);
      },
      "the native CLIs' fail-closed transport verdict on an RCCL INIT log (\"\" = ok)",
      py::arg("log_text"), py::arg("world"), py::arg("local_world"), py::arg("share"));

  py::class_<RiemannConfig>(m, "RiemannConfig")
      .def(py::init<>())
      .def_readwrite("integrand", &RiemannConfig::integrand)
      .def_readwrite("a", &RiemannConfig::a)
      .def_readwrite("b", &RiemannConfig::b)
      .def_readwrite("n", &RiemannConfig::n)
      .def_readwrite("rule", &RiemannConfig::rule)
      .def_readwrite("dtype", &RiemannConfig::dtype)
      .def_readwrite("div", &RiemannConfig::div)
      .def_readwrite("coef", &RiemannConfig::coef)
      .def_readwrite("p0", &RiemannConfig::p0)
      .def_readwrite("p1", &RiemannConfig::p1)
      .def_readwrite("table", &RiemannConfig::table)
      .def_readwrite("grid", &RiemannConfig::grid)
      .def_readwrite("block", &RiemannConfig::block)
      .def_readwrite("waves_per_cu", &RiemannConfig::waves_per_cu)
      .def_readwrite("fused", &RiemannConfig::fused)
      .def_readwrite("slots", &RiemannConfig::slots)
      .def_readwrite("bucket", &RiemannConfig::bucket)
      .def_readwrite("rank", &RiemannConfig::rank)
      .def_readwrite("world", &RiemannConfig::world)
      .def_readwrite("force_collective", &RiemannConfig::force_collective)
      .def_readwrite("step_streams", &RiemannConfig::step_streams)
      .def_readwrite("multistep", &RiemannConfig::multistep)
      .def_readwrite("slice_rank", &RiemannConfig::slice_rank)
      .def_readwrite("slice_world", &RiemannConfig::slice_world)
      .def_readwrite("timeout_s", &RiemannConfig::timeout_s)
      .def_readwrite("host_direct", &RiemannConfig::host_direct)
      .def_readwrite("close", &RiemannConfig::close)
      .def_readwrite("work", &RiemannConfig::work)
      .def_readwrite("queue_wg_per_cu", &RiemannConfig::queue_wg_per_cu)
      .def_readwrite("allreduce_to_host", &RiemannConfig::allreduce_to_host)
      .def_readwrite("chain", &RiemannConfig::chain);

  py::class_<RiemannPlan>(m, "RiemannPlan")
      .def(py::init<const RiemannConfig&, int, const Comm*>(), py::arg("config"),
           py::arg("device"), py::arg("comm") = nullptr, py::keep_alive<1, 4>())
      .def_property_readonly("device", &RiemannPlan::device)
      .def_property_readonly("rank", &RiemannPlan::rank)
      .def_property_readonly("world", &RiemannPlan::world)
      .def("step_streams", &RiemannPlan::step_streams, py::arg("nsteps"))
      .def_property_readonly("begin", &RiemannPlan::begin)
      .def_property_readonly("count", &RiemannPlan::count)
      .def_property_readonly("h", &RiemannPlan::h)
      .def_property_readonly("scale", &RiemannPlan::scale)
      .def_property_readonly("grid", [](const RiemannPlan& p) { return p.shape().grid; })
      .def_property_readonly("block", [](const RiemannPlan& p) { return p.shape().block; })
      .def_property_readonly("effective_div", &RiemannPlan::effective_div)
      .def_property_readonly("compute_stream", [](const RiemannPlan& p) { return reinterpret_cast<uintptr_t>(p.compute_stream()); })
      .def_property_readonly("comm_stream", [](const RiemannPlan& p) { return reinterpret_cast<uintptr_t>(p.comm_stream()); })
      .def("run", &RiemannPlan::run, py::call_guard<py::gil_scoped_release>())
      .def("capture_graphs", &RiemannPlan::capture_graphs, py::call_guard<py::gil_scoped_release>())
      .def("prepare_steps", &RiemannPlan::prepare_steps, py::arg("steps"),
           py::call_guard<py::gil_scoped_release>())
      .def_property_readonly("graph_launches", &RiemannPlan::graph_launches)
      .def_property_readonly("direct_steps", &RiemannPlan::direct_steps)
      .def("launch_steps", &RiemannPlan::launch_steps, py::arg("steps"), py::arg("pipeline") = true,
           py::arg("graphs") = true, py::call_guard<py::gil_scoped_release>())
      .def("sync", &RiemannPlan::sync, py::call_guard<py::gil_scoped_release>())
      .def("run_steps", [](RiemannPlan& p, int steps, bool pipeline, bool graphs) {
             StepTiming t;
             {
               py::gil_scoped_release nogil;
               t = p.run_steps(steps, pipeline, graphs);
             }
             py::dict r;
             r["wall_s"] = t.wall_s;
             r["device_ms"] = t.device_ms;
             r["steps"] = t.steps;
             return r;
           }, py::arg("steps"), py::arg("pipeline") = true, py::arg("graphs") = true)
      .def("barrier", &RiemannPlan::barrier, py::call_guard<py::gil_scoped_release>())
      .def("time_one_shot", [](RiemannPlan& p, int reps, const std::string& mode, int warmup) {
             OneShotTiming t;
             {
               py::gil_scoped_release nogil;
               t = p.time_one_shot(reps, mode, warmup);
             }
             py::dict r;
             r["mode"] = t.mode;
             r["reps"] = t.reps;
             r["median_us"] = t.median_us;
             r["min_us"] = t.min_us;
             r["max_us"] = t.max_us;
             r["device_median_us"] = t.device_median_us;
             r["device_min_us"] = t.device_min_us;
             r["value"] = t.value;
             return r;
           }, py::arg("reps"), py::arg("mode") = "direct", py::arg("warmup") = 400)
      .def("diagnose_batch", [](RiemannPlan& p, int steps) {
             BatchDiag d;
             {
               py::gil_scoped_release nogil;
               d = p.diagnose_batch(steps);
             }
             py::dict r;
             r["steps"] = d.steps;
             r["compute_us"] = d.compute_us;
             r["close_us"] = d.close_us;
             r["allreduce_us"] = d.allreduce_us;
             r["copy_us"] = d.copy_us;
             r["tail_us"] = d.tail_us();
             r["boundary_us"] = d.boundary_us();
             r["marker_us"] = d.marker_us;
             r["device_us"] = d.device_us;
             r["staged_us"] = d.staged_us;
             r["wall_us"] = d.wall_us;
             return r;
           }, py::arg("steps"))
      .def("timeline_batch", [](RiemannPlan& p, int steps, const std::string& form) {
             BatchTimeline t;
             {
               py::gil_scoped_release nogil;
               t = p.timeline_batch(steps, form);
             }
             auto arr64 = [](const std::vector<uint64_t>& v, py::ssize_t rows, py::ssize_t cols) {
               py::array_t<uint64_t> a({rows, cols});
               std::copy(v.begin(), v.end(), a.mutable_data());
               return a;
             };
             const bool queue = t.work == "queue";
             const py::ssize_t rows = queue ? t.workgroups : t.grid;
             py::array_t<uint32_t> hw({rows, py::ssize_t(2)});
             std::copy(t.hw.begin(), t.hw.end(), hw.mutable_data());
             py::dict r;
             r["steps"] = t.steps;
             r["grid"] = t.grid;
             r["block"] = t.block;
             r["clock_khz"] = t.clock_khz;
             r["device_us"] = t.device_us;
             r["work"] = t.work;
             if (queue) {
               r["workgroups"] = t.workgroups;
               r["wg_stamps"] = arr64(t.wg_stamps, rows, 2);
               r["item_stamp"] = arr64(t.item_stamp, t.steps, t.grid);
               py::array_t<uint32_t> owner({static_cast<py::ssize_t>(t.steps),
                                            static_cast<py::ssize_t>(t.grid)});
               std::copy(t.item_owner.begin(), t.item_owner.end(), owner.mutable_data());
               r["item_owner"] = owner;
             } else {
               r["stamps"] = arr64(t.stamps, t.grid, t.steps + 2);
             }
             r["shader_clock"] = arr64(t.shader_clock, rows, 2);
             r["hw"] = hw;
             r["values"] = t.values;
             return r;
           }, py::arg("steps"), py::arg("form") = "auto")
      .def("host_result", &RiemannPlan::host_result)
      .def_property_readonly("host_capacity", &RiemannPlan::host_capacity)
      .def_property_readonly("slots", &RiemannPlan::slots)
      .def_property_readonly("bucketed", &RiemannPlan::bucketed)
      .def_property_readonly("chained", &RiemannPlan::chained)
      .def_property_readonly("multistep", &RiemannPlan::multistep)
      .def_property_readonly("close_in_launch", &RiemannPlan::close_in_launch)
      .def_property_readonly("work", [](const RiemannPlan& p) { return std::string(p.work()); })
      .def_property_readonly("queue_workgroups", &RiemannPlan::queue_workgroups)
      .def_property_readonly("allreduce_to_host", &RiemannPlan::allreduce_to_host)
      .def_property_readonly("direct", &RiemannPlan::direct)
      .def_property_readonly("graph_nodes", &RiemannPlan::graph_nodes)
      .def_property_readonly("graphs_ready", &RiemannPlan::graphs_ready)
      .def_property_readonly("graph_error", &RiemannPlan::graph_error)
      .def_property_readonly("collective", &RiemannPlan::collective)
      .def("host_index_of", &RiemannPlan::host_index_of, py::arg("k"), py::arg("graphs"))
      .def("enqueue", [](const RiemannPlan& p, uintptr_t s, int slot, int hidx) { p.enqueue(stream(s), slot, hidx); })
      .def("device_result", [](const RiemannPlan& p, int slot) { return reinterpret_cast<uintptr_t>(p.device_result(slot)); });

  m.def("launch_riemann_partials",
        [](int integrand, double a, double h, double off, uint64_t i_begin, uint64_t n,
           std::vector<double> coef, double p0, double p1, DType dtype, DivMode div, int grid,
           uintptr_t table, int table_n, uintptr_t partials, uintptr_t s) {
          const RiemannParams p = make_params(integrand, a, h, off, i_begin, n, coef, p0, p1);
          launch_riemann_partials(p, dtype, div, {grid, kRiemannBlock}, ptr<const double>(table),
                                  table_n, ptr<double>(partials), stream(s));
        });
  m.def("riemann_tile_len",
        [](int integrand, double a, double h, double off, uint64_t i_begin, uint64_t n,
           std::vector<double> coef, double p0, double p1, DType dtype, DivMode div) {
          return riemann_tile_len(make_params(integrand, a, h, off, i_begin, n, coef, p0, p1),
                                  dtype, div);
        });
  m.def("riemann_effective_div",
        [](int integrand, double a, double h, double off, uint64_t i_begin, uint64_t n,
           std::vector<double> coef, double p0, double p1, DType dtype, DivMode div) {
          return effective_div(make_params(integrand, a, h, off, i_begin, n, coef, p0, p1), div,
                               dtype);
        });
  m.def("riemann_pi4_ieee_narrow",
        [](int integrand, double a, double h, double off, uint64_t i_begin, uint64_t n,
           std::vector<double> coef, double p0, double p1, DType dtype) {
          return pi4_ieee_narrow(make_params(integrand, a, h, off, i_begin, n, coef, p0, p1),
                                 dtype);
        });
  m.def("resolve_work",
        [](const std::string& work, py::object env, bool pays, bool keeps_static) {
          const std::string e = env.is_none() ? std::string() : env.cast<std::string>();
          return resolve_work(work, env.is_none() ? nullptr : e.c_str(), pays, keeps_static);
        },
        py::arg("work"), py::arg("env") = py::none(), py::arg("pays") = false,
        py::arg("keeps_static") = false);
  m.def("riemann_queue_pays",
        [](int integrand, double a, double h, double off, uint64_t i_begin, uint64_t n,
           std::vector<double> coef, double p0, double p1, DType dtype, DivMode div) {
          return riemann_queue_pays(make_params(integrand, a, h, off, i_begin, n, coef, p0, p1),
                                    dtype, div);
        });
  m.attr("TRIG_SERIES_MAX_N") = kTrigSeriesMaxN;
  m.attr("FAST_TRIG_MAX_N") = kFastTrigMaxN;
  m.attr("PI4_SERIES_MAX_X") = kPi4SeriesMaxX;
  m.attr("PI4_F32_SERIES_MAX_X") = kPi4SeriesMaxXF32;
  m.def("launch_riemann_fused",
        [](int integrand, double a, double h, double off, uint64_t i_begin, uint64_t n,
           std::vector<double> coef, double p0, double p1, DType dtype, DivMode div, int grid,
           uintptr_t table, int table_n, uintptr_t partials, uintptr_t ticket, double scale,
           uintptr_t out, uintptr_t s) {
          const RiemannParams p = make_params(integrand, a, h, off, i_begin, n, coef, p0, p1);
          launch_riemann_fused(p, dtype, div, {grid, kRiemannBlock}, ptr<const double>(table),
                               table_n, ptr<double>(partials), ptr<unsigned>(ticket), scale,
                               ptr<double>(out), stream(s));
        });
  m.def("launch_riemann_point_values",
        [](int integrand, double a, double h, double off, uint64_t i_begin, uint64_t n,
           std::vector<double> coef, double p0, double p1, DivMode div, uintptr_t table,
           int table_n, uintptr_t out, uintptr_t s) {
          const RiemannParams p = make_params(integrand, a, h, off, i_begin, n, coef, p0, p1);
          launch_riemann_point_values(p, div, ptr<const double>(table), table_n, ptr<double>(out),
                                      stream(s));
        });
  m.def("launch_pi4_recip_narrow", [](uintptr_t d, uint64_t n, uintptr_t out, uintptr_t s) {
    launch_pi4_recip_narrow(ptr<const double>(d), n, ptr<double>(out), stream(s));
  });
  m.def("launch_pi4_recip_narrow_f32", [](uintptr_t d, uint64_t n, uintptr_t out, uintptr_t s) {
    launch_pi4_recip_narrow_f32(ptr<const float>(d), n, ptr<float>(out), stream(s));
  });
  m.def("set_lds_poison", &set_lds_poison, py::arg("on"),
        "validation: staged-window kernels fill their LDS with NaN first (current device)");
  m.def("set_trig_library", &set_trig_library, py::arg("on"),
        "validation: kIeee sin/cos by ocml per sample (SinLib / TrainVelLib)");
  m.def("fast_trig_host", [](uintptr_t x, uint64_t n, int shift, uintptr_t val, uintptr_t ulp) {
    const double* xs = reinterpret_cast<const double*>(x);
    double* v = reinterpret_cast<double*>(val);
    double* e = reinterpret_cast<double*>(ulp);
    for (uint64_t i = 0; i < n; ++i) {
      double out;
      if (!fast_trig_point(xs[i], shift, out)) {
        v[i] = e[i] = std::nan("");
        continue;
      }
      const long double ref = shift ? cosl(static_cast<long double>(xs[i]))
                                    : sinl(static_cast<long double>(xs[i]));
      const double rd = static_cast<double>(ref);
      const double sp = std::nextafter(std::fabs(rd), INFINITY) - std::fabs(rd);
      v[i] = out;
      e[i] = static_cast<double>((static_cast<long double>(out) - ref) / sp);
    }
  });
  m.def("set_pi4_library_division", &set_pi4_library_division,
        "validation: kIeee Pi4 launches use the full library division (bitwise the same sums)");
  m.def("riemann_block_ok", &riemann_block_ok);
  m.def("launch_finalize", [](uintptr_t partials, int n, double scale, uintptr_t out, uintptr_t s,
                              int block) {
    launch_finalize(ptr<const double>(partials), n, scale, ptr<double>(out), stream(s), block);
  }, py::arg("partials"), py::arg("n"), py::arg("scale"), py::arg("out"), py::arg("stream"),
     py::arg("block") = kRiemannBlock);
  m.def("default_riemann_grid", [](int cus, int waves) { return default_riemann_shape(cus, waves).grid; });
  m.def("default_reduce_grid", &default_reduce_grid);
  m.def("launch_sum_array", [](uintptr_t x, uint64_t n, double scale, uintptr_t partials, int grid,
                               uintptr_t out, uintptr_t s) {
    launch_sum_array(ptr<const double>(x), n, scale, ptr<double>(partials), grid, ptr<double>(out), stream(s));
  });
  m.def("launch_interp_fill", [](uintptr_t table, int tn, double dt, uint64_t i0, uint64_t n,
                                 uintptr_t y, uintptr_t s) {
    launch_interp_fill(ptr<const double>(table), tn, dt, i0, n, ptr<double>(y), stream(s));
  });
  m.def("scan_state_bytes", &scan_state_bytes);
  m.def("launch_inclusive_scan", [](uintptr_t in, uintptr_t out, uint64_t n, uintptr_t state,
                                    uintptr_t carry, uintptr_t s) {
    launch_inclusive_scan(ptr<const double>(in), ptr<double>(out), n, ptr<void>(state),
                          ptr<const double>(carry), stream(s));
  });
  m.def("launch_interp_scan", [](uintptr_t table, int tn, double dt, uint64_t i0, uint64_t n,
                                 uint64_t win_lo, uint64_t win_hi, uintptr_t out, uintptr_t state,
                                 uintptr_t carry, uintptr_t s) {
    launch_interp_scan_window(ptr<const double>(table), tn, dt, i0, n, win_lo, win_hi,
                              ptr<double>(out), ptr<void>(state), ptr<const double>(carry), stream(s));
  });
  m.def("scan_timeout_flag", [](uintptr_t state, uintptr_t s) { return scan_timeout_flag(ptr<const void>(state), stream(s)); });
  m.def("launch_add_carry", [](uintptr_t x, uint64_t n, uintptr_t carry, uintptr_t s) {
    launch_add_carry(ptr<double>(x), n, ptr<const double>(carry), stream(s));
  });
  m.def("table2d_grid", [](int nx, int ny, double X, double Y, int gx, int gy, int row0, int row1) {
    Table2DParams p{nullptr, nx, ny, X, Y, gx, gy, row0, row1};
    return table2d_grid(p);
  });
  m.def("table2d_path", [](int nx, int ny, double X, double Y, int gx, int gy, int row0, int row1) {
    Table2DParams p{nullptr, nx, ny, X, Y, gx, gy, row0, row1};
    return std::string(table2d_path(p));
  });
  m.def("table2d_shape_info", [](int nx, int ny, double X, double Y, int gx, int gy, int row0,
                                 int row1, int min_wg) {
    Table2DParams p{nullptr, nx, ny, X, Y, gx, gy, row0, row1, min_wg};
    const Table2DShapeInfo i = table2d_shape_info(p);
    py::dict d;
    d["stream"] = i.stream;
    d["rows_per_wave"] = i.rows_per_wave;
    d["tile_rows"] = i.tile_rows;
    d["tile_cols"] = i.tile_cols;
    d["grid"] = py::make_tuple(i.grid_x, i.grid_y);
    d["tile"] = i.tile;
    return d;
  }, py::arg("nx"), py::arg("ny"), py::arg("X"), py::arg("Y"), py::arg("gx"), py::arg("gy"),
     py::arg("row0"), py::arg("row1"), py::arg("min_wg") = 0);
  m.def("launch_table2d_partials", [](uintptr_t table, int nx, int ny, double X, double Y, int gx,
                                      int gy, int row0, int row1, uintptr_t partials, uintptr_t s) {
// ... 489 lines not shown
```

csrc/runtime/integrator.cpp:

```cpp
#include "miint/integrator.hpp"

#include <algorithm>
#include <atomic>
#include <cstdlib>
#include <cstring>
#include <limits>
#include <string>
#include <vector>

#include "miint/fault.hpp"
#include "miint/trace.hpp"

namespace miint {

namespace {
constexpr int kHostRing = 4096;
}

RiemannPlan::RiemannPlan(const RiemannConfig& cfg, int device, const Comm* comm)
    : cfg_(cfg), device_(device), comm_(comm), compute_((set_device(device), Stream())),
      comm_stream_(), ev_fork_(false), ev_join_(false) {
  MIINT_CHECK(cfg.n >= 1, "n must be >= 1");
  MIINT_CHECK(cfg.b != cfg.a, "empty interval");
  MIINT_CHECK(cfg.slots >= 1 && cfg.slots <= 64, "slots must be in [1, 64]");
  if (comm) {
    rank_ = comm->rank();
    world_ = comm->world();
    MIINT_CHECK(comm->device() == device, "communicator bound to another device");
  } else {
    MIINT_CHECK(cfg.world >= 1 && cfg.rank >= 0 && cfg.rank < cfg.world, "bad rank/world");
    rank_ = cfg.rank;
    world_ = cfg.world;
  }
  direct_ = cfg.host_direct && !(comm_ && (world_ > 1 || cfg.force_collective));
  DeviceGuard g(device);
  params_.a = cfg.a;
  params_.h = (cfg.b - cfg.a) / static_cast<double>(cfg.n);
  params_.off = rule_offset(cfg.rule);
  if (cfg.slice_world > 0) {
    MIINT_CHECK(cfg.slice_rank >= 0 && cfg.slice_rank < cfg.slice_world, "bad slice rank");
    rank_slice(cfg.n, cfg.slice_rank, cfg.slice_world, &params_.i_begin, &params_.n);
  } else {
    rank_slice(cfg.n, rank_, world_, &params_.i_begin, &params_.n);
  }
  params_.integrand = static_cast<int>(cfg.integrand);
  params_.ncoef = static_cast<int>(cfg.coef.size());
  MIINT_CHECK(cfg.coef.size() <= static_cast<size_t>(kMaxPolyCoeffs), "too many coefficients");
  for (size_t i = 0; i < cfg.coef.size(); ++i) params_.coef[i] = cfg.coef[i];
  params_.p0 = cfg.p0;
  params_.p1 = cfg.p1;
  scale_ = params_.h * integrand_scale(cfg.integrand);

  const DeviceInfo info = device_info(device);
  MIINT_CHECK(riemann_block_ok(cfg.block),
              "block must be 64, 128, 256, 512 or 1024 threads (got " + std::to_string(cfg.block) +
                  ")");
  const uint64_t bs = static_cast<uint64_t>(cfg.block);
  shape_ = default_riemann_shape(info.num_cus, cfg.waves_per_cu, cfg.block);
  if (cfg.grid > 0) shape_.grid = cfg.grid;
  const uint64_t tl = static_cast<uint64_t>(riemann_tile_len(params_, cfg.dtype, cfg.div));
  const uint64_t tiles = (params_.n + tl - 1) / tl;
  const uint64_t need = std::max<uint64_t>(1, (tiles + bs - 1) / bs);
  shape_.grid = static_cast<int>(std::min<uint64_t>(static_cast<uint64_t>(shape_.grid), need));
  if (cfg.grid <= 0) {
    const uint64_t cus = static_cast<uint64_t>(info.num_cus);
    const uint64_t four =
        std::max<uint64_t>(cus, (tiles + 4 * bs - 1) / (4 * bs));
    uint64_t g = std::min<uint64_t>(static_cast<uint64_t>(shape_.grid), four);
    if (g > cus) g -= g % cus;
    shape_.grid = static_cast<int>(g);
  }
  MIINT_CHECK(cfg.close == "auto" || cfg.close == "kernel" || cfg.close == "launch",
              "close must be auto, kernel or launch (got " + cfg.close + ")");
  if (cfg.multistep && chained()) {
    const int res_kernel =
        riemann_multistep_grid(params_, cfg.dtype, cfg.div, cfg.block, info.num_cus, false);
    close_launch_ = cfg.close == "launch";
    const int res_close =
        close_launch_
            ? riemann_multistep_grid(params_, cfg.dtype, cfg.div, cfg.block, info.num_cus, true)
            : 0;
    if (res_close == 0) close_launch_ = false;
    const int resident = close_launch_ ? res_close : res_kernel;
    if (resident > 0 && cfg.grid <= 0 && shape_.grid > resident) shape_.grid = resident;
    multistep_ = resident > 0 && shape_.grid <= resident;
    if (!multistep_) close_launch_ = false;
  }
  {
    const std::string w =
        resolve_work(cfg.work, std::getenv("MIINT_MS_WORK"),
                     multistep_ && riemann_queue_pays(params_, cfg.dtype, cfg.div),
                     !multistep_ || close_launch_);
    MIINT_CHECK(cfg.queue_wg_per_cu >= 0, "queue_wg_per_cu must be >= 0");
    const int per_cu_max =
        w == "queue" ? riemann_queue_grid(params_, cfg.dtype, cfg.div, cfg.block, 1) : 0;
    if (per_cu_max > 0) {
      const int per_cu =
          cfg.queue_wg_per_cu > 0 ? std::min(cfg.queue_wg_per_cu, per_cu_max) : per_cu_max;
      const uint64_t items = static_cast<uint64_t>(shape_.grid) * static_cast<uint64_t>(cfg.slots);
      queue_wgs_ = static_cast<int>(
          std::min<uint64_t>(static_cast<uint64_t>(per_cu) * info.num_cus, items));
      work_queue_ = true;
    }
  }

  const int lanes = step_streams(cfg.slots);
  partials_ = DeviceBuffer<double>(2 * static_cast<size_t>(std::max(1, lanes)) *
                                   static_cast<size_t>(shape_.grid));
  for (int l = 1; l < lanes; ++l) {
    step_streams_.emplace_back();
    ev_step_join_.emplace_back(new Event(false));
  }
  slots_ = DeviceBuffer<double>(static_cast<size_t>(shape_.grid));
  fill_unset_slots(slots_.get(), slots_.size(), nullptr);
  if (multistep_)
    ms_partials_ = DeviceBuffer<double>(static_cast<size_t>(cfg.slots) * shape_.grid);
  if (close_launch_) {
    ms_ticket_ = DeviceBuffer<unsigned int>(kTicketWords);
    MIINT_HIP(hipMemset(ms_ticket_.get(), 0, ms_ticket_.bytes()));
  }
  if (work_queue_) {
    queue_ = DeviceBuffer<unsigned int>(kQueueWords);
    MIINT_HIP(hipMemset(queue_.get(), 0, queue_.bytes()));
  }
  result_ = DeviceBuffer<double>(static_cast<size_t>(cfg.slots));
  sync_ = DeviceBuffer<double>(1);
  MIINT_HIP(hipMemset(sync_.get(), 0, sync_.bytes()));
  ticket_ = DeviceBuffer<unsigned int>(kTicketWords);
  MIINT_HIP(hipMemset(ticket_.get(), 0, ticket_.bytes()));
  MIINT_HIP(hipMemset(result_.get(), 0, result_.bytes()));
  if (cfg.integrand == Integrand::kTable) {
    MIINT_CHECK(cfg.table.size() >= 2, "table integrand needs a table");
    table_ = DeviceBuffer<double>(cfg.table.size());
    MIINT_HIP(hipMemcpy(table_.get(), cfg.table.data(), table_.bytes(), hipMemcpyHostToDevice));
  }
  host_ = PinnedBuffer<double>(static_cast<size_t>(std::max(kHostRing, cfg.slots)));
  for (int i = 0; i < cfg.slots; ++i) {
    ev_computed_.emplace_back(new Event(false));
    ev_drained_.emplace_back(new Event(false));
  }
  MIINT_HIP(hipDeviceSynchronize());
}

RiemannPlan::~RiemannPlan() {
  (void)hipSetDevice(device_);
  (void)hipStreamSynchronize(compute_.get());
  (void)hipStreamSynchronize(comm_stream_.get());
  for (const auto& s : step_streams_) (void)hipStreamSynchronize(s.get());
}

// ... 628 lines not shown
```

cuda_v_mpi_amd/integrate.py:

```python
from __future__ import annotations

import dataclasses
import math
import time

import torch

from .models import integrands
from .parallel import decomposition
from .parallel.dist import DistContext, native_comm


@dataclasses.dataclass
class IntegrationResult:
    value: float
    analytic: float
    n: int
    integrand: str
    rule: str
    dtype: str
    gpus: int
    seconds_wall: float
    seconds_device: float

    @property
    def abs_err(self) -> float:
        return abs(self.value - self.analytic)

    @property
    def rel_err(self) -> float:
        return self.abs_err / abs(self.analytic) if self.analytic else float("nan")

    @property
    def subintervals_per_s(self) -> float:
        t = self.seconds_device if self.seconds_device > 0 else self.seconds_wall
        return self.n / t if t > 0 else float("nan")

    def as_dict(self) -> dict:
        d = dataclasses.asdict(self)
        d.update(abs_err=self.abs_err, rel_err=self.rel_err,
                 subintervals_per_s=self.subintervals_per_s)
        return d


class Integrator:
    def __init__(self, integrand: str | integrands.IntegrandSpec = "pi4", n: int = 10**9,
                 rule: str = "left", dtype: str = "fp64", div: str = "series_exact",
                 backend: str = "hip", ctx: DistContext | None = None, comm: str = "native",
                 fused: bool = True, grid: int = 0, slots: int = 16, a: float | None = None,
                 b: float | None = None, force_collective: bool = False, bucket: bool = True,
                 chain: bool = True, comm_obj=None, threads: int = 0,
                 slice_of: tuple[int, int] | None = None, step_streams: int = 0,
                 block: int = 256, multistep: bool = True, close: str = "auto",
                 allreduce_to_host: bool = True, timeout_s: float = 300.0,
                 work: str = "auto", queue_wg_per_cu: int = 0, **spec_kw):
        spec = integrands.get(integrand, **spec_kw) if isinstance(integrand, str) else integrand
        if a is not None or b is not None:
            spec = dataclasses.replace(spec, a=spec.a if a is None else a,
                                       b=spec.b if b is None else b)
        if n < 1:
            raise ValueError("n must be >= 1")
        if rule not in ("left", "mid", "right"):
            raise ValueError("rule must be left|mid|right")
        if dtype not in ("fp64", "fp32", "fp32acc"):
            raise ValueError("dtype must be fp64|fp32|fp32acc")
        self.spec, self.n, self.rule, self.dtype, self.div = spec, int(n), rule, dtype, div
        self.backend, self.comm_kind = backend, comm
        if comm_obj is not None:
            ctx = DistContext(rank=comm_obj.rank, world=comm_obj.world, device=comm_obj.device,
                              backend=comm_obj.kind)
        self.ctx = ctx or DistContext()
        self.begin, self.count = decomposition.rank_slice(self.n, self.ctx.rank, self.ctx.world)
        self._plan = None
        self._comm = None
        self._pool = None
        if backend in ("hip", "host"):
            from ._native import native

            m = native()
            if backend == "hip" and m.device_count() < 1:
                raise RuntimeError("backend='hip' needs a HIP device; use backend='host' or "
                                   "'cpu' explicitly")
            cfg = m.RiemannConfig()
            cfg.integrand = getattr(m.Integrand, spec.name)
            cfg.a, cfg.b, cfg.n = spec.a, spec.b, self.n
            cfg.rule = getattr(m.Rule, rule)
            cfg.dtype = getattr(m.DType, dtype)
            cfg.div = getattr(m.DivMode, div)
            cfg.coef = list(spec.coef)
            cfg.p0, cfg.p1 = spec.p0, spec.p1
            cfg.table = spec.native_table()
            cfg.grid, cfg.fused, cfg.slots = grid, fused, slots
            cfg.block = block
            cfg.force_collective = force_collective
            cfg.bucket = bucket
            cfg.chain = chain
            cfg.step_streams = step_streams
            cfg.multistep = multistep
            cfg.close = close
            if work not in ("auto", "static", "queue"):
                raise ValueError("work must be auto|static|queue")
            cfg.work = work
            cfg.queue_wg_per_cu = queue_wg_per_cu
            cfg.allreduce_to_host = allreduce_to_host
            cfg.timeout_s = timeout_s
            if slice_of is not None:
                cfg.slice_rank, cfg.slice_world = int(slice_of[0]), int(slice_of[1])
            self._m = m
            if backend == "host":
                self._cfg = cfg
                self._pool = m.HostPool(threads)
                return
            if comm_obj is not None:
                self._comm = comm_obj
                self._plan = m.RiemannPlan(cfg, comm_obj.device, comm_obj)
            elif (self.ctx.world > 1 or force_collective) and comm == "native":
                self._comm = native_comm(self.ctx)
                self._plan = m.RiemannPlan(cfg, self.ctx.device, self._comm)
            else:
                cfg.rank, cfg.world = self.ctx.rank, self.ctx.world
                self._plan = m.RiemannPlan(cfg, self.ctx.device)
        elif backend != "cpu":
            raise ValueError("backend must be 'hip', 'host' or 'cpu'")

    @property
    def plan(self):
        return self._plan

    @property
    def h(self) -> float:
        return (self.spec.b - self.spec.a) / self.n

    def describe(self) -> dict:
        d = dict(integrand=self.spec.name, n=self.n, rule=self.rule, dtype=self.dtype,
                 backend=self.backend, rank=self.ctx.rank, world=self.ctx.world,
                 begin=self.begin, count=self.count)
        if self._plan is not None:
            d.update(grid=self._plan.grid, block=self._plan.block,
                     div=str(self._plan.effective_div).split(".")[-1])
        return d

    def _torch_reduce(self, value: float) -> float:
        dev = "cuda" if self.ctx.backend == "nccl" else "cpu"
        t = torch.tensor([value], dtype=torch.float64, device=dev)
        self.ctx.all_reduce_sum(t)
        return float(t.item())

    def _cpu_local(self) -> float:
        spec, h = self.spec, self.h
        off = {"left": 0.0, "mid": 0.5, "right": 1.0}[self.rule]
        dt = torch.float64 if self.dtype == "fp64" else torch.float32
        chunk = 1 << 22
        parts = []
        for s in range(self.begin, self.begin + self.count, chunk):
            i = torch.arange(s, min(self.begin + self.count, s + chunk), dtype=torch.float64)
            x = (spec.a + (i + off) * h).to(dt)
            parts.append(float(spec.f_torch(x).to(torch.float64).sum()))
        return math.fsum(parts) * h

    def run(self) -> IntegrationResult:
        t0 = time.perf_counter()
        dev_s = 0.0
        if self.backend == "cpu":
            value = self._torch_reduce(self._cpu_local()) if self.ctx.world > 1 else self._cpu_local()
        elif self.backend == "host":
            t = time.perf_counter()
            value = self._m.host_riemann(self._cfg, self.begin, self.count, self._pool)
            dev_s = time.perf_counter() - t
            if self.ctx.world > 1:
                value = self._torch_reduce(value)
        else:
            if self._comm is not None or self.ctx.world == 1:
                t = self._plan.run_steps(1, pipeline=False, graphs=False)
                value = self._plan.host_result(0)
                dev_s = t["device_ms"] * 1e-3
            else:
                t = self._plan.run_steps(1, pipeline=False, graphs=False)
                value = self._torch_reduce(self._plan.host_result(0))
                dev_s = t["device_ms"] * 1e-3
        wall = time.perf_counter() - t0
        return IntegrationResult(value=value, analytic=self.spec.analytic(), n=self.n,
                                 integrand=self.spec.name, rule=self.rule, dtype=self.dtype,
                                 gpus=self.ctx.world, seconds_wall=wall, seconds_device=dev_s)

    def run_steps(self, steps: int, pipeline: bool = True, graphs: bool = True) -> dict:
        if self._plan is None:
# ... 263 lines not shown
```

cuda_v_mpi_amd/ops/kernels.py:

```python
from __future__ import annotations

import math

import torch

from .._native import native
from ..models.integrands import IntegrandSpec

_RULE_OFF = {"left": 0.0, "mid": 0.5, "right": 1.0}


def _stream() -> int:
    return torch.cuda.current_stream().cuda_stream


def _check(t: torch.Tensor, dtype=torch.float64, name: str = "tensor") -> None:
    if not t.is_cuda:
        raise ValueError(f"{name} must be on a HIP device (got {t.device})")
    if t.dtype != dtype:
        raise ValueError(f"{name} must be {dtype} (got {t.dtype})")
    if not t.is_contiguous():
        raise ValueError(f"{name} must be contiguous")


def _device() -> torch.device:
    if not torch.cuda.is_available():
        raise RuntimeError("HIP device required (torch.cuda.is_available() is False)")
    return torch.device("cuda", torch.cuda.current_device())


def _enums(dtype: str, div: str):
    m = native()
    return getattr(m.DType, dtype), getattr(m.DivMode, div)


def default_grid() -> int:
    m = native()
    cus = torch.cuda.get_device_properties(torch.cuda.current_device()).multi_processor_count
    return m.default_riemann_grid(cus, 32)


def riemann_partials(spec: IntegrandSpec, n: int, rule: str = "left", dtype: str = "fp64",
                     div: str = "series_exact", grid: int | None = None, i_begin: int = 0,
                     n_local: int | None = None) -> torch.Tensor:
    m = native()
    dev = _device()
    grid = grid or default_grid()
    n_local = n if n_local is None else n_local
    h = (spec.b - spec.a) / n
    partials = torch.empty(grid, dtype=torch.float64, device=dev)
    table = _table_tensor(spec, dev)
    dt, dv = _enums(dtype, div)
    m.launch_riemann_partials(spec.native_id, spec.a, h, _RULE_OFF[rule], i_begin, n_local,
                              list(spec.coef), spec.p0, spec.p1, dt, dv, grid,
                              table.data_ptr() if table is not None else 0,
                              table.numel() if table is not None else 0,
                              partials.data_ptr(), _stream())
    return partials


_TABLE_CACHE: dict = {}


def _table_tensor(spec: IntegrandSpec, dev: torch.device):
    if spec.name != "table":
        return None
    key = (dev.index, spec.table)
    t = _TABLE_CACHE.get(key)
    if t is None:
        t = torch.tensor(spec.native_table(), dtype=torch.float64, device=dev)
        _TABLE_CACHE[key] = t
    return t


def finalize(partials: torch.Tensor, scale: float, out: torch.Tensor | None = None) -> torch.Tensor:
    _check(partials, name="partials")
    out = torch.empty(1, dtype=torch.float64, device=partials.device) if out is None else out
    native().launch_finalize(partials.data_ptr(), partials.numel(), scale, out.data_ptr(), _stream())
    return out


def unset_slots(n: int, device) -> torch.Tensor:
    word = native().UNSET_SLOT_WORD
    bits = (word << 32) | word
    return torch.full((n,), bits - (1 << 64), dtype=torch.int64, device=device).view(torch.float64)


class FusedWorkspace:

    def __init__(self, grid: int, device: torch.device | None = None):
        dev = device or _device()
        self.grid = grid
        self.partials = unset_slots(grid, dev)
        self.ticket = torch.zeros(native().TICKET_WORDS, dtype=torch.int32, device=dev)


def riemann(spec: IntegrandSpec, n: int, rule: str = "left", dtype: str = "fp64",
            div: str = "series_exact", grid: int | None = None, i_begin: int = 0,
            n_local: int | None = None, out: torch.Tensor | None = None,
            workspace: FusedWorkspace | None = None, fused: bool = True) -> torch.Tensor:
    m = native()
    dev = _device()
    grid = grid or (workspace.grid if workspace else default_grid())
    n_local = n if n_local is None else n_local
    h = (spec.b - spec.a) / n
    scale = h * spec.scale
    out = torch.empty(1, dtype=torch.float64, device=dev) if out is None else out
    if not fused:
        p = riemann_partials(spec, n, rule, dtype, div, grid, i_begin, n_local)
        return finalize(p, scale, out)
    ws = workspace or FusedWorkspace(grid, dev)
    table = _table_tensor(spec, dev)
    dt, dv = _enums(dtype, div)
    m.launch_riemann_fused(spec.native_id, spec.a, h, _RULE_OFF[rule], i_begin, n_local,
                           list(spec.coef), spec.p0, spec.p1, dt, dv, ws.grid,
                           table.data_ptr() if table is not None else 0,
                           table.numel() if table is not None else 0,
                           ws.partials.data_ptr(), ws.ticket.data_ptr(), scale, out.data_ptr(),
                           _stream())
    return out


def point_values(spec: IntegrandSpec, n: int, rule: str = "left", div: str = "series",
                 i_begin: int = 0, n_local: int | None = None) -> torch.Tensor:
    m = native()
    dev = _device()
    n_local = n if n_local is None else n_local
    out = torch.empty(n_local, dtype=torch.float64, device=dev)
    table = _table_tensor(spec, dev)
    m.launch_riemann_point_values(spec.native_id, spec.a, (spec.b - spec.a) / n, _RULE_OFF[rule],
                                  i_begin, n_local, list(spec.coef), spec.p0, spec.p1,
                                  getattr(m.DivMode, div),
                                  table.data_ptr() if table is not None else 0,
                                  table.numel() if table is not None else 0,
                                  out.data_ptr(), _stream())
    return out


def pi4_recip_narrow(d: torch.Tensor) -> torch.Tensor:
    f32 = d.dtype == torch.float32
    _check(d, dtype=torch.float32 if f32 else torch.float64, name="d")
    out = torch.empty_like(d)
    launch = native().launch_pi4_recip_narrow_f32 if f32 else native().launch_pi4_recip_narrow
    launch(d.data_ptr(), d.numel(), out.data_ptr(), _stream())
    return out


def sum_array(x: torch.Tensor, scale: float = 1.0) -> torch.Tensor:
    _check(x, name="x")
    m = native()
    cus = torch.cuda.get_device_properties(x.device).multi_processor_count
    grid = m.default_reduce_grid(cus)
    partials = torch.empty(grid, dtype=torch.float64, device=x.device)
    out = torch.empty(1, dtype=torch.float64, device=x.device)
    m.launch_sum_array(x.data_ptr(), x.numel(), scale, partials.data_ptr(), grid, out.data_ptr(),
                       _stream())
    return out


def profile_tensor(device=None) -> torch.Tensor:
    from ..models import integrands
    dev = device or _device()
    return _table_tensor(integrands.table(), torch.device(dev))


def _scan_table(table: torch.Tensor | None, dev) -> torch.Tensor:
    if table is None:
        return profile_tensor(dev)
    _check(table, name="table")
    if table.dim() != 1:
        raise ValueError("table must be one-dimensional")
    return table


def interp_fill(n: int, i0: int = 0, dt: float = 1e-4, out: torch.Tensor | None = None,
                table: torch.Tensor | None = None) -> torch.Tensor:
    dev = _device()
    tab = _scan_table(table, dev)
    out = torch.empty(n, dtype=torch.float64, device=dev) if out is None else out
    _check(out, name="out")
    native().launch_interp_fill(tab.data_ptr(), tab.numel(), dt, i0, n, out.data_ptr(), _stream())
    return out


def _scan_state(n: int, dev) -> torch.Tensor:
    nbytes = native().scan_state_bytes(n)
    return torch.empty(nbytes, dtype=torch.uint8, device=dev)


def inclusive_scan(x: torch.Tensor, carry: torch.Tensor | None = None,
                   out: torch.Tensor | None = None) -> torch.Tensor:
    _check(x, name="x")
    out = torch.empty_like(x) if out is None else out
    st = _scan_state(x.numel(), x.device)
    native().launch_inclusive_scan(x.data_ptr(), out.data_ptr(), x.numel(), st.data_ptr(),
                                   carry.data_ptr() if carry is not None else 0, _stream())
    _check_timeout(st)
    return out


def interp_scan(n: int, i0: int = 0, dt: float = 1e-4, window: tuple[int, int] | None = None,
                carry: torch.Tensor | None = None,
                table: torch.Tensor | None = None) -> torch.Tensor:
    dev = _device()
    tab = _scan_table(table, dev)
    out = torch.empty(n, dtype=torch.float64, device=dev)
    st = _scan_state(n, dev)
    lo, hi = window if window is not None else (0, (1 << 64) - 1)
    native().launch_interp_scan(tab.data_ptr(), tab.numel(), dt, i0, n, lo, hi, out.data_ptr(),
                                st.data_ptr(), carry.data_ptr() if carry is not None else 0,
                                _stream())
    _check_timeout(st)
    return out


def trainscan(n: int, i0: int = 0, dt: float = 1e-4, window: tuple[int, int] | None = None,
              carries: torch.Tensor | None = None, algo: str = "fused",
              table: torch.Tensor | None = None):
    if algo not in ("fused", "fold", "onepass"):
        raise ValueError("algo must be fused|fold|onepass")
    if algo == "onepass" and carries is not None:
        raise ValueError("the one-pass scan takes no carries (single-GPU form)")
    if algo == "fold" and carries is not None:
        raise RuntimeError("fold mode is single-GPU (no rank carries)")
    m = native()
    if algo == "fold" and not m.trainscan_fold_applies(dt, n):
        raise RuntimeError("fold mode needs dt = 1/sps and at most 64 blocks of 256 tiles")
# ... 196 lines not shown
```

cuda_v_mpi_amd/utils/pi4_truth.py:

```python
from __future__ import annotations

import dataclasses
import math
from fractions import Fraction

import mpmath
import numpy as np

from .trig_truth import RULE_OFF, U32, U64

PREC = 200
MP = mpmath.MPContext()
MP.prec = 2 * PREC

SCALE = 4.0
TILE64 = 384
TILE32 = 192
TILE_PER_SAMPLE = 32
HALF_SPAN_H = 2.0e-6
BLOCK = 256
WAVE = 64

PI4_NARROW_MAX_X = 2.0 ** 249
PI4_F32_NARROW_MAX_X = 2.0 ** 49
PI4_SERIES_MAX_X = 2.0 ** 249
PI4_F32_SERIES_MAX_X = 2.0 ** 62

EM_RAW64 = 2.0 ** -22
EM_NEWTON32 = 2.0 ** -23
SECOND_ORDER = 1.0 + 1.0e-5

PATHS = ("fp64-series_exact", "fp64-series", "fp64-series_direct", "fp64-ieee",
         "fp32-series", "fp32-ieee", "fp32acc-series", "fp32acc-ieee")
SERIES_PATHS = ("fp64-series_exact", "fp64-series", "fp64-series_direct", "fp32-series",
                "fp32acc-series")


def tile_len(path: str) -> int:
    return {"fp64-series_exact": TILE64, "fp64-series": TILE64, "fp32-series": TILE32,
            "fp32acc-series": TILE32}.get(path, TILE_PER_SAMPLE)


def seed_residual(path: str) -> float:
    return {"fp64-series_exact": EM_RAW64, "fp64-series": EM_RAW64,
            "fp64-series_direct": 2.0 ** -45}.get(path, EM_NEWTON32)


def _mpq(fr: Fraction):
    return MP.mpf(fr.numerator) / MP.mpf(fr.denominator)


@dataclasses.dataclass(frozen=True)
class Geometry:
    a: float
    h: float
    off: Fraction
    i_begin: int
    count: int

    def x(self, i) -> Fraction:
        return Fraction(self.a) + (self.i_begin + Fraction(i) + self.off) * Fraction(self.h)

    @property
    def x_abs_max(self) -> float:
        return float(max(abs(self.x(0)), abs(self.x(self.count - 1))))

    @property
    def x_abs_min(self) -> float:
        x0, x1 = self.x(0), self.x(self.count - 1)
        return 0.0 if (x0 <= 0 <= x1 or x1 <= 0 <= x0) else float(min(abs(x0), abs(x1)))


def geometry(spec, n: int, rule: str, i_begin: int = 0, count: int | None = None) -> Geometry:
    if spec.name != "pi4":
        raise ValueError("pi4_truth covers pi4")
    h = (spec.b - spec.a) / n
    count = n if count is None else count
    if count < 1 or i_begin < 0:
        raise ValueError("need count >= 1 and i_begin >= 0")
    return Geometry(float(spec.a), h, RULE_OFF[rule], int(i_begin), int(count))


def f_true(x: Fraction):
    return 1 / (1 + _mpq(x) ** 2)


def true_values(g: Geometry):
    exact = [f_true(g.x(i)) for i in range(g.count)]
    return np.array([float(v) for v in exact], dtype=np.float64), exact


def direct_sum(g: Geometry):
    return MP.fsum(f_true(g.x(i)) for i in range(g.count))


def progression_sum(x0: Fraction, h: Fraction, m: int):
    if h == 0:
        return m * f_true(x0)
    if h < 0:
        x0, h = x0 + (m - 1) * h, -h
    wr = x0 / h
    mag = abs(wr) + 1 / h + m + 2
    bits = 2 * PREC + 3 * (mag.numerator.bit_length() - mag.denominator.bit_length() + 2)
    with MP.workprec(max(MP.prec, bits)):
        hh = _mpq(h)
        w = MP.mpc(_mpq(wr), -1 / hh)
        return +((MP.digamma(m + w) - MP.digamma(w)).imag / hh)


def true_sum(g: Geometry):
    return progression_sum(g.x(0), Fraction(g.h), g.count)


def true_value(g: Geometry):
    return MP.mpf(SCALE) * MP.mpf(g.h) * true_sum(g)


def rnd64(fr: Fraction) -> float:
    try:
        return float(fr)
    except OverflowError:
        return math.inf if fr > 0 else -math.inf


def rnd32(fr: Fraction) -> np.float32:
    if fr == 0:
        return np.float32(0.0)
    sign, q = (-1.0 if fr < 0 else 1.0), abs(fr)
    e = q.numerator.bit_length() - q.denominator.bit_length()
    if Fraction(2) ** e > q:
        e -= 1
    e = max(e, -126)
    scaled = q / Fraction(2) ** (e - 23)
    n, r = divmod(scaled.numerator, scaled.denominator)
    if 2 * r > scaled.denominator or (2 * r == scaled.denominator and n & 1):
        n += 1
    v = math.ldexp(float(n), e - 23)
    return np.float32(sign * v) if v < 2.0 ** 128 else np.float32(sign * math.inf)


def _fr(v) -> Fraction:
    return Fraction(float(v))


def fma64(a: float, b: float, c: float) -> float:
    if not (math.isfinite(a) and math.isfinite(b) and math.isfinite(c)):
        return a * b + c
    return rnd64(_fr(a) * _fr(b) + _fr(c))


def fma32(a, b, c) -> np.float32:
    a, b, c = float(a), float(b), float(c)
    if not (math.isfinite(a) and math.isfinite(b) and math.isfinite(c)):
        return np.float32(a * b + c)
    return rnd32(_fr(a) * _fr(b) + _fr(c))


def recip64(d: float) -> float:
    return 0.0 if math.isinf(d) else rnd64(1 / _fr(d))


def recip32(d) -> np.float32:
    return np.float32(0.0) if math.isinf(float(d)) else rnd32(1 / _fr(d))


def _pow2(v: float) -> bool:
    return v != 0.0 and math.frexp(abs(v))[0] == 0.5


def coords_exact(g: Geometry) -> bool:
    if not _pow2(g.h):
        return False
    q = Fraction(abs(g.h)) / 2
    if (Fraction(g.a) / q).denominator != 1:
        return False
    far = max(abs(g.x(0)), abs(g.x(g.count - 1))) + 512 * Fraction(abs(g.h))
    return far / q < 2 ** 53


def base_index(g: Geometry) -> float:
    return float(g.i_begin) + float(g.off)


def tile_anchor(g: Geometry, path: str, tile: int = 0) -> float:
    T = tile_len(path)
    mid = path in ("fp64-series_exact", "fp64-series", "fp32-series", "fp32acc-series")
    ib = base_index(g) + float(tile * T) + (0.5 * (T - 1) if mid else 0.0)
    return fma64(ib, g.h, g.a)


def ulp32(v: float) -> float:
    a = max(abs(v), 2.0 ** -126)
    return 2.0 ** (math.frexp(a)[1] - 24)


def rel_slope(g: Geometry) -> float:
    lo, hi = g.x_abs_min, g.x_abs_max
    if lo <= 1.0 <= hi:
        return 1.0
    x = hi if hi < 1.0 else lo
    return 2.0 * x / (1.0 + x * x) if x < 1e150 else 2.0 / x


def coord_rel(g: Geometry, roundings64: int, fp32: bool = False, exact: bool | None = None) -> float:
    exact = coords_exact(g) if exact is None else exact
    dx = 0.0 if exact else roundings64 * 0.5 * math.ulp(g.x_abs_max)
    if fp32:
        dx += 0.5 * ulp32(g.x_abs_max)
    return rel_slope(g) * dx * SECOND_ORDER


def _offsets(T: int):
    return [Fraction(2 * j + 1 - T, 2) for j in range(T)]


def defined_inputs(path: str, g: Geometry, tile: int = 0) -> dict:
    xa = tile_anchor(g, path, tile)
    if path in ("fp32-series", "fp32acc-series"):
        xm = np.float32(xa)
        hf = np.float32(g.h)
        return {"xm": _fr(xm), "h": _fr(hf), "dm": _fr(fma32(xm, xm, np.float32(1.0)))}
    if path == "fp64-series":
        return {"xm": _fr(xa), "h": Fraction(g.h), "dm": _fr(fma64(xa, xa, 1.0))}
    if path == "fp64-series_exact":
        return {"xm": _fr(xa), "h": Fraction(g.h), "dm": 1 + _fr(xa) ** 2}
    raise ValueError(path)


def defined_tile_sum(path: str, g: Geometry, tile: int = 0):
    T = tile_len(path)
    if path == "fp64-series_direct":
        x0 = tile_anchor(g, path, tile)
        tot = MP.mpf(0)
        for u in range(T):
            x = fma64(float(u), g.h, x0)
            tot += 1 / _mpq(_fr(fma64(x, x, 1.0)))
        return tot
    p = defined_inputs(path, g, tile)
    return MP.fsum(1 / _mpq(p["dm"] + 2 * p["xm"] * p["h"] * k + p["h"] ** 2 * k * k)
                   for k in _offsets(T))


def _per_sample_kind(path: str) -> str:
    if path.startswith("fp64"):
        return "fp64"
    return "fp32acc" if path.startswith("fp32acc") else "fp32"


def model_point(path: str, g: Geometry, i: int):
    x = fma64(base_index(g) + float(i), g.h, g.a)
    if _per_sample_kind(path) == "fp64":
        return recip64(fma64(x, x, 1.0))
    with np.errstate(over="ignore"):
        xf = np.float32(x)
    return float(recip32(fma32(xf, xf, np.float32(1.0))))


def model_tile(path: str, g: Geometry, tile: int = 0):
    if path.split("-")[1] != "ieee":
        raise ValueError("bitwise models exist for the per-sample (ieee) tiles")
    x0 = tile_anchor(g, path, tile)
    kind = _per_sample_kind(path)
    if kind == "fp64":
        acc = 0.0
        for u in range(TILE_PER_SAMPLE):
            x = fma64(float(u), g.h, x0)
            acc += recip64(fma64(x, x, 1.0))
        return acc
    lanes = [np.float32(0.0), np.float32(0.0)]
    with np.errstate(all="ignore"):
        x0f, hf, one = np.float32(x0), np.float32(g.h), np.float32(1.0)
        for u in range(TILE_PER_SAMPLE):
            x = fma32(np.float32(u), hf, x0f)
            lanes[u & 1] = np.float32(lanes[u & 1] + recip32(fma32(x, x, one)))
        if kind == "fp32":
            return float(lanes[0]) + float(lanes[1])
        return float(np.float32(lanes[0] + lanes[1]))


def _dpp_sum(v: list, add, steps: int) -> list:
    perms = (lambda i: i ^ 1, lambda i: i ^ 2, lambda i: (i & ~7) | (7 - (i & 7)),
             lambda i: (i & ~15) | (15 - (i & 15)))
    for p in perms[:steps]:
        v = [add(v[i], v[p(i)]) for i in range(len(v))]
    return v


def model_block_sum(lane_values: list, add=lambda a, b: a + b, zero=0.0):
    nw = len(lane_values) // WAVE
    totals = []
    for w in range(nw):
        v = _dpp_sum(list(lane_values[w * WAVE:(w + 1) * WAVE]), add, 4)
        v = [add(v[i], v[(i // 16) * 16 - 1]) if (i // 16) in (1, 3) else v[i] for i in range(WAVE)]
        v = [add(v[i], v[31]) if i >= 32 else v[i] for i in range(WAVE)]
        totals.append(v[63])
    if nw == 1:
        return totals[0]
    r = totals + [zero] * (WAVE - nw)
    return _dpp_sum(r, add, 2 if nw <= 4 else 4)[0]


def model_partials(path: str, g: Geometry, grid: int, block: int = BLOCK) -> list:
    T = tile_len(path)
    if g.count >= T and path.split("-")[1] != "ieee":
        raise ValueError("no bitwise model of a series tile")
    kind = _per_sample_kind(path)
    f32 = kind == "fp32acc"
    zero = np.float32(0.0) if f32 else 0.0
    add = (lambda a, b: np.float32(a + b)) if f32 else (lambda a, b: a + b)
    lanes = grid * block
    ntile = g.count // T
    done = ntile * T
    acc = [zero] * lanes
    for t in range(ntile):
        lane = t % lanes
        v = model_tile(path, g, t)
        acc[lane] = add(acc[lane], np.float32(v) if f32 else v)
    for k in range(g.count - done):
        lane = k % lanes
        v = model_point(path, g, done + k)
        acc[lane] = add(acc[lane], np.float32(v) if f32 else v)
    return [float(model_block_sum(acc[b * block:(b + 1) * block], add, zero)) for b in range(grid)]


def underflow_floor(g: Geometry, fp32: bool) -> float:
    x = g.x_abs_max
    if fp32:
        return 0.0 if x < 2.0 ** 63 else (2.0 ** -149 if x < 1.8e19 else 2.0 ** -127)
    return 0.0 if x < 2.0 ** 511 else (2.0 ** -1074 if x < 1.3e154 else 2.0 ** -1023)


def point_bound(path: str, g: Geometry, vals: np.ndarray, full_tile: bool = True) -> np.ndarray:
    div = path.split("-")[1]
    v = np.abs(np.asarray(vals, dtype=np.float64))
    half_ulp = 0.5 * np.array([math.ulp(t) for t in v]) + underflow_floor(g, False)
    if div == "ieee" or not full_tile:
        rel = coord_rel(g, 2) + U64
        return v * rel * SECOND_ORDER + half_ulp
    h = abs(g.h)
    if div == "series_direct":
        E = seed_residual(path) + 16.0 * h * (1.0 + 16.0 * h)
        rel = coord_rel(g, 2) + U64 + 3.0 * U64 * E + E ** 3 / (1.0 - E)
    elif div == "series":
        E = EM_RAW64 + 192.0 * h * (1.0 + 192.0 * h)
        rel = (coord_rel(g, 2) + U64 + 3.0 * 2.0 ** -54 + 2.0 ** -53
               + 2.0 * U64 * (192.0 * h + (192.0 * h) ** 2) + E ** 3 / (1.0 - E))
    elif div == "series_exact":
        E = EM_RAW64 + 192.0 * h * (1.0 + 192.0 * h)
        off_unit = 2.0 ** -54 if g.x_abs_max + 192.0 * h > 1.0 else 0.0
        rel = (coord_rel(g, 2) + off_unit + 4.0 * U64 * EM_RAW64 + 4.0 * U64 * E + 2.2e-18
               + E ** 3 / (1.0 - E))
    else:
        raise ValueError(path)
    return v * rel * SECOND_ORDER + half_ulp


def point32_bound(g: Geometry, v: float) -> float:
    rel = coord_rel(g, 1, fp32=True) + U32
    return abs(v) * rel * SECOND_ORDER + 0.5 * ulp32(v) + underflow_floor(g, True)


def tile_defn_rel(path: str, g: Geometry) -> float:
    h = abs(g.h)
    T = tile_len(path)
    E = seed_residual(path) + (T / 2) * h * (1.0 + (T / 2) * h)
    if path in ("fp32-series", "fp32acc-series"):
        de = U32 * (EM_NEWTON32 + 287.5 * h + (2 * 9216 + 6400 + 2480) * h * h + 10.0 * E)
        sums = 49.0 * U32 * E
        fold = 2.0 * U64 if path == "fp32-series" else 2.0 * U32 + U64
        rel = (de + sums + E * E / (1.0 - E)) * (1.0 + 2.0 * E) + fold
    elif path == "fp64-series":
        rel = (3.0 * 2.0 ** -54 + 2.0 * U64 * (192.0 * h + (192.0 * h) ** 2)
               + E ** 3 / (1.0 - E)) * (1.0 + 2.0 * E) + 2.0 ** -45 + U64
    elif path == "fp64-series_exact":
        off_unit = 2.0 ** -54 if g.x_abs_max + 192.0 * h > 1.0 else 0.0
        rel = (off_unit + 4.0 * U64 * EM_RAW64 + 2.0 * U64 * E
               + 2.0 * U64 * (192.0 * h) ** 2 / 3.0 + 2.2e-18 + 96.0 * U32 * E * E
               + 2.0 * U64 * E + E ** 3 / (1.0 - E)) * (1.0 + 2.0 * E) + 2.0 * U64
    elif path == "fp64-series_direct":
        rel = (19.0 * U64 * E + 33.0 * U64 * E * E + E ** 3 / (1.0 - E)) * (1.0 + 2.0 * E) + U64
    else:
        raise ValueError(path)
    return rel * SECOND_ORDER


def defn_truth_rel(path: str, g: Geometry) -> float:
    h = abs(g.h)
    if path == "fp64-series_exact":
        rel = coord_rel(g, 1)
    elif path == "fp64-series":
        rel = coord_rel(g, 1) + U64 * (1.0 + 2.0 * 192.0 * h)
    elif path == "fp64-series_direct":
        rel = coord_rel(g, 2) + U64
    elif path in ("fp32-series", "fp32acc-series"):
        ex32 = fp32_coords_exact(g)
        rel = (coord_rel(g, 1, fp32=not ex32) + (0.0 if _pow2(g.h) else rel_slope(g) * 96.0 * h * U32)
               + U32 * (1.0 + 2.0 * 96.0 * h))
    else:
        raise ValueError(path)
    return rel * SECOND_ORDER


def fp32_coords_exact(g: Geometry) -> bool:
    if not (coords_exact(g) and _pow2(g.h)) or g.count < TILE32:
        return False
    last = g.count // TILE32 - 1
    for t in (0, last):
        xm = tile_anchor(g, "fp32-series", t)
        if float(np.float32(xm)) != xm:
            return False
    far = max(abs(tile_anchor(g, "fp32-series", 0)), abs(tile_anchor(g, "fp32-series", last)))
    return (Fraction(192) * Fraction(abs(g.h)) / Fraction(ulp32(far))).denominator == 1


def ieee_rel(path: str, g: Geometry, point: bool = False) -> float:
    if path.startswith("fp64"):
        return (coord_rel(g, 1 if point else 2) + 2.0 * U64) * SECOND_ORDER
    dx = 0.0 if point else 0.5 * ulp32(g.x_abs_max) + 31.0 * abs(g.h) * U32
    return (coord_rel(g, 1, fp32=True) + rel_slope(g) * dx + 2.0 * U32) * SECOND_ORDER


def tile_truth_bound(path: str, g: Geometry, true_tile_sum: float) -> float:
    S = abs(true_tile_sum)
    T = tile_len(path)
    if path in SERIES_PATHS:
        rel = tile_defn_rel(path, g) + defn_truth_rel(path, g)
    elif path == "fp64-ieee":
        rel = ieee_rel(path, g) + 32.0 * U64
    else:
        rel = ieee_rel(path, g) + 16.0 * U32 + (U32 if path.startswith("fp32acc") else U64)
    return S * rel * SECOND_ORDER + T * underflow_floor(g, not path.startswith("fp64"))


def launch_depth(count: int, tile: int, grid: int, block: int = BLOCK) -> int:
    lanes = grid * block
    tiles = count // tile
    rem = count - tiles * tile
    return (-(-tiles // lanes) + -(-rem // lanes)) + 10 + -(-grid // block) + 10


def launch_sum_bound(path: str, g: Geometry, true_total: float, grid: int, block: int = BLOCK) -> float:
    T = tile_len(path)
    S = abs(true_total)
    if path in SERIES_PATHS:
        rel = tile_defn_rel(path, g) + defn_truth_rel(path, g)
    elif path == "fp64-ieee":
        rel = ieee_rel(path, g) + 32.0 * U64
    else:
        rel = ieee_rel(path, g) + 16.0 * U32 + (U32 if path.startswith("fp32acc") else U64)
    ipath = path.split("-")[0] + "-ieee"
    rel = max(rel, ieee_rel(ipath, g, point=True))
    depth = launch_depth(g.count, T, grid, block)
    if path.startswith("fp32acc"):
        fin = -(-grid // block) + 10
        acc = (depth - fin) * U32 + fin * U64
    else:
        acc = depth * U64
    return S * (rel + acc) * SECOND_ORDER + g.count * underflow_floor(g, not path.startswith("fp64"))


def launch_value_bound(path: str, g: Geometry, true_total: float, grid: int, block: int = BLOCK) -> float:
    s = SCALE * abs(g.h)
    return s * (launch_sum_bound(path, g, true_total, grid, block) + U64 * abs(true_total))


def emulate_f32_tile(path: str, g: Geometry, tile: int = 0, seed_rel: float = 0.0,
                     defect: str | None = None) -> float:
    f = np.float32
    one = f(1.0)
    xm, hf = f(tile_anchor(g, path, tile)), f(g.h)
    dm = fma32(xm, xm, one)
    s = rnd32(_fr(recip32(dm)) * (1 + Fraction(seed_rel)))
    s = fma32(s, fma32(-dm, s, one), s)
    em = fma32(-dm, s, one)
    a = rnd32(_fr(rnd32(_fr(f(-2.0) * hf) * _fr(xm))) * _fr(s))
    b = rnd32(-_fr(rnd32(_fr(hf) * _fr(hf))) * _fr(s))
    lanes = {"t.x": None, "t.y": None, "t1.x": None, "t1.y": None}

    def add(key, v):
        lanes[key] = v if lanes[key] is None else f(lanes[key] + v)

    for q in range(6):
        c0 = f((q - 2.5) * 32)
        ec = fma32(c0, fma32(c0, b, a), em)
        aq = fma32(f(c0 + c0), b, a)
        cc = [fma32(f(0.25), b, ec), fma32(f(2.25), b, ec)]
        for j in range(0, 16, 2):
            k0, k1 = f(j + 0.5), f(j + 1.5)
            add("t.x", fma32(k0, aq, cc[0]))
            add("t.y", fma32(-k0, aq, cc[0]))
            add("t1.x", fma32(k1, aq, cc[1]))
            add("t1.y", fma32(-k1, aq, cc[1]))
            if j + 2 < 16:
                cc = [fma32(f(4.0 * j + 6.0), b, cc[0]), fma32(f(4.0 * j + 10.0), b, cc[1])]
    tx, ty = f(lanes["t.x"] + lanes["t1.x"]), f(lanes["t.y"] + lanes["t1.y"])
    t = f(tx + ty)
    if path == "fp32acc-series" or defect == "fold32":
        return float(fma32(s, f(f(192.0) + t), f(0.0)))
    return fma64(float(s), 192.0 + float(t), 0.0)
```

Before: 32020 billion.

## Add long 1536-sample pi4 series_exact tile using packed fp32 square sums

Adds a Pi4Long integrand that spans 1536-sample tiles: one fp64 reciprocal seed per tile, with per-sample quadratic corrections computed as packed fp32 FMAs in inline assembly (v_pk_fma_f32 with op_sel and neg modifiers). Sub-tile centres are pipelined into the next sub-tile's instruction stream. The aim is to amortise the fp64 seed over four times more samples and push most of the work onto packed fp32 throughput. A tile option (auto/short/long plus an environment variable) selects the form, with admission limited by step size. Error bounds in the truth model are extended to cover it, and a modifier-check kernel is added to validate the op_sel semantics.

```diff
diff --git a/csrc/cli/miint.cpp b/csrc/cli/miint.cpp
--- a/csrc/cli/miint.cpp
+++ b/csrc/cli/miint.cpp
@@ -306,6 +306,7 @@
     "                   [--block B] [--grid G] [--step-streams S] [--trig-library] [--settle N]\n"
     "                   [--no-multistep] [--slots K] [--close auto|kernel|launch] [--no-ar-host]\n"
     "                   [--work auto|static|queue] [--queue-wg-per-cu W]\n"
+    "                   [--tile auto|short|long]\n"
     "                   [--diagnose] [--slice R/W] [--timeline FILE]\n"
     "                   (--timeline: after the timed run, one batch from the timeline build of\n"
     "                   the multi-step launch, per-workgroup device-clock stamps as JSON in FILE;\n"
@@ -354,6 +355,7 @@
       c.slots = static_cast<int>(a.integer("slots", c.slots));
       c.close = a.str("close", c.close);
       c.work = a.str("work", c.work);
+      c.tile = a.str("tile", c.tile);
       c.queue_wg_per_cu = static_cast<int>(a.integer("queue-wg-per-cu", 0));
       c.allreduce_to_host = !a.flag("no-ar-host");
       cli::parse_slice(a, &c.slice_rank, &c.slice_world);
diff --git a/csrc/include/miint/common.hpp b/csrc/include/miint/common.hpp
--- a/csrc/include/miint/common.hpp
+++ b/csrc/include/miint/common.hpp
@@ -66,6 +66,8 @@
   double p0, p1;
   double trig[kSinTrig];
   float trig32[kSinTrig];
+  int tile;
 };
+constexpr int kTileAuto = 0, kTileShort = 1, kTileLong = 2;
 
 }
diff --git a/csrc/include/miint/integrands.hpp b/csrc/include/miint/integrands.hpp
--- a/csrc/include/miint/integrands.hpp
+++ b/csrc/include/miint/integrands.hpp
@@ -335,6 +335,178 @@
 };
 constexpr double kPi4NarrowMaxX = 0x1p249;
 
+struct Pi4Long : TileDefaults<Pi4Long> {
+  static constexpr double kScale = 4.0;
+  static constexpr int kKPairs = 16;
+  static constexpr int kSub = 4 * kKPairs;
+  static constexpr int kSubs = 24;
+  static constexpr int kTile = kSub * kSubs;
+  static constexpr double kSumK2 =
+      (static_cast<double>(kTile) * kTile * kTile - kTile) / 12.0;
+  static_assert(kSumK2 == 301989760.0, "sum of squared midpoint offsets of a 1536-sample tile");
+  static constexpr double kMeanK2 = (kSub * kSub - 1) / 12.0;
+  static_assert(kMeanK2 == 341.25, "mean of k^2 over a 64-sample sub-tile");
+
+  template <DivMode M>
+  __host__ __device__ static constexpr int tile_len() {
+    static_assert(M == DivMode::kSeriesExact, "the long tile is a series_exact tile");
+    return kTile;
+  }
+  template <int U, DivMode M>
+  __device__ static constexpr double anchor() { return 0.5 * (U - 1); }
+
+  typedef float f32x2 __attribute__((ext_vector_type(2)));
+  f32x2 pkf[kKPairs];
+  f32x2 pcf[kSubs / 2];
+
+  __device__ __forceinline__ void init() {
+#pragma unroll
+    for (int j = 0; j < kKPairs; ++j) {
+      const f32x2 kk = {j + 0.5f, j + kKPairs + 0.5f};
+      pkf[j] = __builtin_bit_cast(f32x2, Pi4::opaque_s(__builtin_bit_cast(double, kk)));
+    }
+#pragma unroll
+    for (int i = 0; i < kSubs / 2; ++i) {
+      const float c0 = kSub * (i + 0.5f);
+      const f32x2 cc = {c0, -c0};
+      pcf[i] = __builtin_bit_cast(f32x2, Pi4::opaque_s(__builtin_bit_cast(double, cc)));
+    }
+  }
+
+  __device__ __forceinline__ double point(double x) const { return 1.0 / fma(x, x, 1.0); }
+
+  __device__ __forceinline__ static Pi4::Seed seed_exact(double xm, double h) {
+    const double dm = fma(xm, xm, 1.0);
+    const double s = __builtin_amdgcn_rcp(dm);
+    const double q = xm * s;
+    const double qe = fma(xm, s, -q);
+    const double em = fma(-xm, qe, fma(-xm, q, 1.0 - s));
+    return {s, em, (-2.0 * h) * q, -(h * h) * s};
+  }
+  struct SeedF32 {
+    f32x2 p1, p2;
+  };
+  __device__ __forceinline__ static SeedF32 seed_f32(const Pi4::Seed& sd) {
+    const float b = static_cast<float>(sd.b);
+    return {{static_cast<float>(sd.a), b}, {static_cast<float>(fma(kMeanK2, sd.b, sd.em)), b + b}};
+  }
+
+#define MIINT_LC_IN(C0N, CN) \
+  "v_pk_fma_f32 %[" CN "], %[" C0N "], %[p1], %[p1] op_sel:[0,1,0] op_sel_hi:[1,1,0]\n\t"
+#define MIINT_LC_A(C0N, AN) \
+  "v_pk_fma_f32 %[" AN "], %[" C0N "], %[p2], %[p1] op_sel:[0,1,0] op_sel_hi:[1,1,0]\n\t"
+#define MIINT_LC_C(C0N, CN) \
+  "v_pk_fma_f32 %[" CN "], %[" C0N "], %[" CN "], %[p2] op_sel_hi:[1,1,0]\n\t"
+#define MIINT_L_LO "0"
+#define MIINT_L_HI "1"
+#define MIINT_L_PAIRS2(K, HALF)                                                            \
+  "v_pk_fma_f32 %[e0], %[" K "], %[a], %[c] op_sel:[0," HALF "," HALF "] op_sel_hi:[0," HALF \
+  "," HALF "] neg_hi:[1,0,0]\n\t"                                                          \
+  "v_pk_fma_f32 %[e1], %[" K "], %[a], %[c] op_sel:[1," HALF "," HALF "] op_sel_hi:[1," HALF \
+  "," HALF "] neg_hi:[1,0,0]\n\t"                                                          \
+  "v_pk_fma_f32 %[ta], %[e0], %[e0], %[ta]\n\t"                                            \
+  "v_pk_fma_f32 %[tb], %[e1], %[e1], %[tb]\n\t"
+#define MIINT_L_REST(HALF)                                                                   \
+  MIINT_L_PAIRS2("k4", HALF) MIINT_L_PAIRS2("k5", HALF) MIINT_L_PAIRS2("k6", HALF)           \
+  MIINT_L_PAIRS2("k7", HALF) MIINT_L_PAIRS2("k8", HALF) MIINT_L_PAIRS2("k9", HALF)           \
+  MIINT_L_PAIRS2("k10", HALF) MIINT_L_PAIRS2("k11", HALF) MIINT_L_PAIRS2("k12", HALF)        \
+  MIINT_L_PAIRS2("k13", HALF) MIINT_L_PAIRS2("k14", HALF) MIINT_L_PAIRS2("k15", HALF)
+#define MIINT_L_SUBTILE(HALF)                                                                \
+  MIINT_L_PAIRS2("k0", HALF) MIINT_L_PAIRS2("k1", HALF) MIINT_L_PAIRS2("k2", HALF)           \
+  MIINT_L_PAIRS2("k3", HALF) MIINT_L_REST(HALF)
+#define MIINT_L_SUBTILE_NEXT(HALF)                                                           \
+  MIINT_L_PAIRS2("k0", HALF) MIINT_LC_IN("c0n", "cn") MIINT_L_PAIRS2("k1", HALF)             \
+  MIINT_LC_A("c0n", "an") MIINT_L_PAIRS2("k2", HALF) MIINT_LC_C("c0n", "cn")                 \
+  MIINT_L_PAIRS2("k3", HALF) MIINT_L_REST(HALF)
+#define MIINT_L_IN                                                                            \
+  [k0] "s"(pkf[0]), [k1] "s"(pkf[1]), [k2] "s"(pkf[2]), [k3] "s"(pkf[3]), [k4] "s"(pkf[4]),   \
+  [k5] "s"(pkf[5]), [k6] "s"(pkf[6]), [k7] "s"(pkf[7]), [k8] "s"(pkf[8]), [k9] "s"(pkf[9]),   \
+  [k10] "s"(pkf[10]), [k11] "s"(pkf[11]), [k12] "s"(pkf[12]), [k13] "s"(pkf[13]),             \
+  [k14] "s"(pkf[14]), [k15] "s"(pkf[15]), [a] "v"(a), [c] "v"(c)
+  template <bool Hi>
+  __device__ __forceinline__ void subtile_squares(f32x2& ta, f32x2& tb, f32x2 a, f32x2 c) const {
+    static_assert(kKPairs == 16, "the statement names 16 pair constants");
+    f32x2 e0, e1;
+    if constexpr (Hi) {
+      asm volatile(MIINT_L_SUBTILE(MIINT_L_HI)
+                   : [e0] "=&v"(e0), [e1] "=&v"(e1), [ta] "+v"(ta), [tb] "+v"(tb)
+                   : MIINT_L_IN);
+    } else {
+      asm volatile(MIINT_L_SUBTILE(MIINT_L_LO)
+                   : [e0] "=&v"(e0), [e1] "=&v"(e1), [ta] "+v"(ta), [tb] "+v"(tb)
+                   : MIINT_L_IN);
+    }
+  }
+  __device__ __forceinline__ void subtile_squares_next(f32x2& ta, f32x2& tb, f32x2 a, f32x2 c,
+                                                       f32x2 c0n, const SeedF32& sf, f32x2& an,
+                                                       f32x2& cn) const {
+    f32x2 e0, e1;
+    asm volatile(MIINT_L_SUBTILE_NEXT(MIINT_L_HI)
+                 : [e0] "=&v"(e0), [e1] "=&v"(e1), [an] "=&v"(an), [cn] "=&v"(cn), [ta] "+v"(ta),
+                   [tb] "+v"(tb)
+                 : MIINT_L_IN, [c0n] "s"(c0n), [p1] "v"(sf.p1), [p2] "v"(sf.p2));
+  }
+  __device__ __forceinline__ static void first_centres(f32x2 c0n, const SeedF32& sf, f32x2& an,
+                                                       f32x2& cn) {
+    asm volatile(MIINT_LC_IN("c0n", "cn") MIINT_LC_A("c0n", "an") MIINT_LC_C("c0n", "cn")
+                 : [an] "=&v"(an), [cn] "=&v"(cn)
+                 : [c0n] "s"(c0n), [p1] "v"(sf.p1), [p2] "v"(sf.p2));
+  }
+#undef MIINT_LC_IN
+#undef MIINT_LC_A
+#undef MIINT_LC_C
+#undef MIINT_L_LO
+#undef MIINT_L_HI
+#undef MIINT_L_PAIRS2
+#undef MIINT_L_REST
+#undef MIINT_L_SUBTILE
+#undef MIINT_L_SUBTILE_NEXT
+#undef MIINT_L_IN
+
+  template <int U, DivMode M>
+  __device__ __forceinline__ double tile_acc(double xa, double h, double acc) const {
+    static_assert(M == DivMode::kSeriesExact && U == kTile, "1536-sample series_exact tiles");
+    const Pi4::Seed sd = seed_exact(xa, h);
+    const double lin = fma(kSumK2, sd.b, static_cast<double>(U) * sd.em);
+    const SeedF32 sf = seed_f32(sd);
+    f32x2 ta = {0.0f, 0.0f}, tb = {0.0f, 0.0f};
+    f32x2 a[2], c[2];
+    first_centres(pcf[0], sf, a[0], c[0]);
+#pragma unroll
+    for (int i = 0; i < kSubs / 2; ++i) {
+      if (i + 1 < kSubs / 2)
+        subtile_squares_next(ta, tb, a[i & 1], c[i & 1], pcf[i + 1], sf, a[(i + 1) & 1],
+                             c[(i + 1) & 1]);
+      else
+        subtile_squares<true>(ta, tb, a[i & 1], c[i & 1]);
+      subtile_squares<false>(ta, tb, a[i & 1], c[i & 1]);
+    }
+    ta += tb;
+    const double t = lin + (static_cast<double>(ta.x) + static_cast<double>(ta.y));
+    return fma(sd.s, t, fma(sd.s, static_cast<double>(U), acc));
+  }
+
+  __device__ __forceinline__ double series_exact_point(double xm, double h, int u) const {
+    const Pi4::Seed sd = seed_exact(xm, h);
+    const double K = static_cast<double>(u) - 0.5 * (kTile - 1);
+    const double e = fma(K, fma(K, sd.b, sd.a), sd.em);
+    const SeedF32 sf = seed_f32(sd);
+    const int q = u / kSub, w = u % kSub;
+    const bool hi = q < kSubs / 2;
+    const int i = hi ? kSubs / 2 - 1 - q : q - kSubs / 2;
+    const float c0 = kSub * (i + 0.5f);
+    const f32x2 cc = {c0, -c0};
+    const f32x2 A = {sf.p1.x, sf.p1.x}, B = {sf.p1.y, sf.p1.y};
+    const f32x2 B2 = {sf.p2.y, sf.p2.y}, base = {sf.p2.x, sf.p2.x};
+    const f32x2 cs = __builtin_elementwise_fma(cc, __builtin_elementwise_fma(cc, B, A), base);
+    const f32x2 as = __builtin_elementwise_fma(cc, B2, A);
+    const float k = static_cast<float>(w) - 0.5f * (kSub - 1);
+    const float e_sq = fmaf(k, hi ? as.y : as.x, hi ? cs.y : cs.x);
+    const float sq = e_sq * e_sq;
+    return fma(sd.s, e + static_cast<double>(sq), sd.s);
+  }
+};
+
 __device__ __forceinline__ void tile_sincos(double th, double& S, double& C) {
   constexpr double kTwoOverPi = 6.36619772367581382433e-01;
   constexpr double kPio2Hi = 1.57079632673412561417e+00;
diff --git a/csrc/include/miint/integrator.hpp b/csrc/include/miint/integrator.hpp
--- a/csrc/include/miint/integrator.hpp
+++ b/csrc/include/miint/integrator.hpp
@@ -41,6 +41,7 @@
   bool multistep = true;
   std::string close = "auto";
   std::string work = "auto";
+  std::string tile = "auto";
   int queue_wg_per_cu = 0;
   bool allreduce_to_host = true;
   int step_streams = 0;
@@ -169,6 +170,7 @@
   bool multistep() const { return chained() && multistep_; }
   bool close_in_launch() const { return multistep() && close_launch_; }
   const char* work() const { return multistep() && work_queue_ ? "queue" : "static"; }
+  const char* tile() const { return long_tile_ ? "long" : "short"; }
   int queue_workgroups() const { return multistep() && work_queue_ ? queue_wgs_ : 0; }
   bool allreduce_to_host() const {
     return bucketed() && cfg_.allreduce_to_host && ar_host_ok_;
@@ -199,6 +201,7 @@
   DeviceBuffer<double> slots_;
   DeviceBuffer<double> ms_partials_;
   bool multistep_ = false;
+  bool long_tile_ = false;
   bool close_launch_ = false;
   bool capturing_ = false;
   bool ar_host_ok_ = true;
diff --git a/csrc/include/miint/kernels.hpp b/csrc/include/miint/kernels.hpp
--- a/csrc/include/miint/kernels.hpp
+++ b/csrc/include/miint/kernels.hpp
@@ -92,6 +92,39 @@
           !(trig_series_in_range(p) && pi4_series_in_range(p, t) && poly_series_in_range(p)))
              ? DivMode::kIeee
              : e;
+}
+
+constexpr int kSeriesHalfSpanLong = 768;
+constexpr bool kPi4LongTileAuto = true;
+inline bool series_ok_long(double h) {
+  const double ah = h < 0 ? -h : h;
+  return ah > 0.0 && kSeriesHalfSpanLong * ah <= 2e-6;
+}
+inline bool pi4_long_admitted(const RiemannParams& p, DType t, DivMode d) {
+  return static_cast<Integrand>(p.integrand) == Integrand::kPi4 && t == DType::kF64 &&
+         d == DivMode::kSeriesExact && series_ok_long(p.h) &&
+         effective_div(p, d, t) == DivMode::kSeriesExact;
+}
+inline bool pi4_tile_long(const RiemannParams& p, DType t, DivMode d, const char* env,
+                          bool auto_long = false) {
+  MIINT_CHECK(p.tile == kTileAuto || p.tile == kTileShort || p.tile == kTileLong,
+              "tile must be auto, short or long");
+  const bool ok = pi4_long_admitted(p, t, d);
+  if (p.tile == kTileLong)
+    MIINT_CHECK(ok, "tile = long needs fp64 pi4 with div = series_exact and a step of at most "
+                    "2e-6 / 768 (N >= 3.84e8 on a unit interval); this launch's does not admit it");
+  if (p.tile != kTileAuto) return p.tile == kTileLong;
+  if (env && *env) {
+    const std::string e(env);
+    MIINT_CHECK(e == "short" || e == "long", "MIINT_PI4_TILE must be short or long (got " + e + ")");
+    return ok && e == "long";
+  }
+  return ok && auto_long;
+}
+inline int tile_form_of(const std::string& s) {
+  MIINT_CHECK(s == "auto" || s == "short" || s == "long",
+              "tile must be auto, short or long (got " + s + ")");
+  return s == "auto" ? kTileAuto : s == "short" ? kTileShort : kTileLong;
 }
 
 struct LaunchShape {
@@ -169,6 +202,8 @@
 void launch_pi4_recip_narrow_f32(const float* d, uint64_t n, float* out, hipStream_t stream);
 void set_pi4_library_division(bool on);
 bool pi4_ieee_narrow(const RiemannParams& p, DType dtype);
+void launch_pk_modifier_check(const float* ac, uint64_t n, float ka, float kb, float* out,
+                              hipStream_t stream);
 void set_trig_library(bool on);
 void set_lds_poison(bool on);
 void set_lds_poison_trainscan(bool on);
diff --git a/csrc/kernels/riemann.hip b/csrc/kernels/riemann.hip
--- a/csrc/kernels/riemann.hip
+++ b/csrc/kernels/riemann.hip
@@ -2,6 +2,7 @@
 
 #include <atomic>
 #include <cmath>
+#include <cstdlib>
 #include <string>
 
 #include "miint/common.hpp"
@@ -279,12 +280,22 @@
 static_assert(Pi4::kSeriesTile / 2 == kSeriesHalfSpan &&
                   Pi4F32::kSubs * Pi4F32::kSubLen / 2 == kSeriesHalfSpanF32,
               "kSeriesHalfSpan(F32) must be half the Pi4 series tile lengths");
+static_assert(Pi4Long::kTile / 2 == kSeriesHalfSpanLong,
+              "kSeriesHalfSpanLong must be half the long Pi4 tile");
 
 template <class F> struct Maker;
 template <> struct Maker<Pi4> {
   static constexpr int kLds = 1;
   __device__ static Pi4 make(const RiemannParams&, const double*, int, double*) {
     Pi4 f;
+    f.init();
+    return f;
+  }
+};
+template <> struct Maker<Pi4Long> {
+  static constexpr int kLds = 1;
+  __device__ static Pi4Long make(const RiemannParams&, const double*, int, double*) {
+    Pi4Long f;
     f.init();
     return f;
   }
@@ -857,7 +868,7 @@
 }
 template <DivMode M, class F>
 constexpr bool queue_pays() {
-  return M == DivMode::kSeriesExact && __is_same(F, Pi4);
+  return M == DivMode::kSeriesExact && (__is_same(F, Pi4) || __is_same(F, Pi4Long));
 }
 
 __global__ __launch_bounds__(kMaxBlock) void multistep_close_kernel(const double* partials,
@@ -887,6 +898,8 @@
     if constexpr (M == DivMode::kSeries && __is_same(F, Pi4)) {
       v = full ? f.series_point(xm, p.h, u) : f.point(x);
     } else if constexpr (M == DivMode::kSeriesExact && __is_same(F, Pi4)) {
+      v = full ? f.series_exact_point(xm, p.h, u) : f.point(x);
+    } else if constexpr (__is_same(F, Pi4Long)) {
       v = full ? f.series_exact_point(xm, p.h, u) : f.point(x);
     } else if constexpr (M == DivMode::kSeries && IsPolyF64<F>::value) {
       v = full ? f.series_point(xm, u) : f.point(x);
@@ -917,6 +930,39 @@
   for (uint64_t i = static_cast<uint64_t>(blockIdx.x) * B + threadIdx.x; i < n; i += stride)
     out[i] = Pi4::recip_narrow(d[i]);
 }
+__global__ __launch_bounds__(B) void pk_modifier_check_kernel(const float* ac, uint64_t n,
+                                                              float ka, float kb, float* out) {
+  typedef float f32x2 __attribute__((ext_vector_type(2)));
+  const f32x2 kk = __builtin_bit_cast(
+      f32x2, Pi4::opaque_s(__builtin_bit_cast(double, f32x2{ka, kb})));
+  const f32x2 kan = __builtin_bit_cast(
+      f32x2, Pi4::opaque_s(__builtin_bit_cast(double, f32x2{ka, -ka})));
+  const f32x2 kbn = __builtin_bit_cast(
+      f32x2, Pi4::opaque_s(__builtin_bit_cast(double, f32x2{kb, -kb})));
+  const uint64_t i = static_cast<uint64_t>(blockIdx.x) * B + threadIdx.x;
+  if (i >= n) return;
+  const f32x2 a = {ac[4 * i], ac[4 * i + 1]}, c = {ac[4 * i + 2], ac[4 * i + 3]};
+  f32x2 r[8];
+  asm volatile(
+      "v_pk_fma_f32 %[r0], %[kk], %[a], %[c] op_sel:[0,0,0] op_sel_hi:[0,0,0] neg_hi:[1,0,0]\n\t"
+      "v_pk_fma_f32 %[r1], %[kk], %[a], %[c] op_sel:[1,0,0] op_sel_hi:[1,0,0] neg_hi:[1,0,0]\n\t"
+      "v_pk_fma_f32 %[r2], %[kk], %[a], %[c] op_sel:[0,1,1] op_sel_hi:[0,1,1] neg_hi:[1,0,0]\n\t"
+      "v_pk_fma_f32 %[r3], %[kk], %[a], %[c] op_sel:[1,1,1] op_sel_hi:[1,1,1] neg_hi:[1,0,0]\n\t"
+      : [r0] "=&v"(r[0]), [r1] "=&v"(r[1]), [r2] "=&v"(r[2]), [r3] "=&v"(r[3])
+      : [kk] "s"(kk), [a] "v"(a), [c] "v"(c));
+  asm volatile(
+      "v_pk_fma_f32 %[r0], %[ka], %[a], %[c] op_sel_hi:[1,0,0]\n\t"
+      "v_pk_fma_f32 %[r1], %[kb], %[a], %[c] op_sel_hi:[1,0,0]\n\t"
+      "v_pk_fma_f32 %[r2], %[ka], %[a], %[c] op_sel:[0,1,1]\n\t"
+      "v_pk_fma_f32 %[r3], %[kb], %[a], %[c] op_sel:[0,1,1]\n\t"
+      : [r0] "=&v"(r[4]), [r1] "=&v"(r[5]), [r2] "=&v"(r[6]), [r3] "=&v"(r[7])
+      : [ka] "s"(kan), [kb] "s"(kbn), [a] "v"(a), [c] "v"(c));
+#pragma unroll
+  for (int j = 0; j < 8; ++j) {
+    out[16 * i + 2 * j] = r[j].x;
+    out[16 * i + 2 * j + 1] = r[j].y;
+  }
+}
 __global__ __launch_bounds__(B) void recip_narrow_f32_kernel(const float* d, uint64_t n,
                                                              float* out) {
   const uint64_t stride = static_cast<uint64_t>(gridDim.x) * B;
@@ -1086,9 +1132,14 @@
          std::fabs(std::fma(last, p.h, p.a)) < max_x;
 }
 
+inline bool pi4_long(const RiemannParams& p, DType dtype, DivMode m) {
+  return pi4_tile_long(p, dtype, m, std::getenv("MIINT_PI4_TILE"));
+}
+
 template <template <DivMode, class> class Op, class... A>
 void dispatch(const RiemannParams& p, DType dtype, DivMode m, A&&... a) {
   const Integrand f = static_cast<Integrand>(p.integrand);
+  if (p.tile != kTileAuto && p.tile != kTileShort) (void)pi4_tile_long(p, dtype, m, nullptr);
   if (dtype == DType::kF32Acc32) {
     MIINT_CHECK(f == Integrand::kPi4, "fp32 accumulation (fp32acc) is implemented for pi4 only");
     if (m == DivMode::kSeries) Op<DivMode::kSeries, Pi4F32Acc32>::run(a...);
@@ -1134,6 +1185,8 @@
   switch (f) {
     case Integrand::kPi4:
       if (m == DivMode::kSeries) Op<DivMode::kSeries, Pi4>::run(a...);
+      else if (m == DivMode::kSeriesExact && pi4_long(p, dtype, m))
+        Op<DivMode::kSeriesExact, Pi4Long>::run(a...);
       else if (m == DivMode::kSeriesExact) Op<DivMode::kSeriesExact, Pi4>::run(a...);
       else if (m == DivMode::kSeriesDirect) Op<DivMode::kSeriesDirect, Pi4>::run(a...);
       else if (pi4_narrow(p)) Op<DivMode::kIeee, Pi4>::run(a...);
@@ -1465,6 +1518,15 @@
   MIINT_HIP(hipGetLastError());
 }
 
+void launch_pk_modifier_check(const float* ac, uint64_t n, float ka, float kb, float* out,
+                              hipStream_t stream) {
+  if (n == 0) return;
+  MIINT_CHECK(n <= (uint64_t(1) << 24), "modifier check: at most 2^24 elements");
+  const int grid = static_cast<int>((n + B - 1) / B);
+  pk_modifier_check_kernel<<<grid, B, 0, stream>>>(ac, n, ka, kb, out);
+  MIINT_HIP(hipGetLastError());
+}
+
 void launch_pi4_recip_narrow_f32(const float* d, uint64_t n, float* out, hipStream_t stream) {
   if (n == 0) return;
   const uint64_t blocks = (n + B - 1) / B;
diff --git a/csrc/python/module.cpp b/csrc/python/module.cpp
--- a/csrc/python/module.cpp
+++ b/csrc/python/module.cpp
@@ -31,7 +31,8 @@
 hipStream_t stream(uintptr_t s) { return reinterpret_cast<hipStream_t>(s); }
 
 RiemannParams make_params(int integrand, double a, double h, double off, uint64_t i_begin,
-                          uint64_t n, const std::vector<double>& coef, double p0, double p1) {
+                          uint64_t n, const std::vector<double>& coef, double p0, double p1,
+                          const std::string& tile = "auto") {
   RiemannParams p{};
   p.a = a;
   p.h = h;
@@ -44,6 +45,7 @@
   for (size_t i = 0; i < coef.size(); ++i) p.coef[i] = coef[i];
   p.p0 = p0;
   p.p1 = p1;
+  p.tile = tile_form_of(tile);
   return p;
 }
 
@@ -278,6 +280,7 @@
       .def_readwrite("host_direct", &RiemannConfig::host_direct)
       .def_readwrite("close", &RiemannConfig::close)
       .def_readwrite("work", &RiemannConfig::work)
+      .def_readwrite("tile", &RiemannConfig::tile)
       .def_readwrite("queue_wg_per_cu", &RiemannConfig::queue_wg_per_cu)
       .def_readwrite("allreduce_to_host", &RiemannConfig::allreduce_to_host)
       .def_readwrite("chain", &RiemannConfig::chain);
@@ -403,6 +406,7 @@
       .def_property_readonly("multistep", &RiemannPlan::multistep)
       .def_property_readonly("close_in_launch", &RiemannPlan::close_in_launch)
       .def_property_readonly("work", [](const RiemannPlan& p) { return std::string(p.work()); })
+      .def_property_readonly("tile", [](const RiemannPlan& p) { return std::string(p.tile()); })
       .def_property_readonly("queue_workgroups", &RiemannPlan::queue_workgroups)
       .def_property_readonly("allreduce_to_host", &RiemannPlan::allreduce_to_host)
       .def_property_readonly("direct", &RiemannPlan::direct)
@@ -414,20 +418,37 @@
       .def("enqueue", [](const RiemannPlan& p, uintptr_t s, int slot, int hidx) { p.enqueue(stream(s), slot, hidx); })
       .def("device_result", [](const RiemannPlan& p, int slot) { return reinterpret_cast<uintptr_t>(p.device_result(slot)); });
 
+  auto partials_fn = [](int integrand, double a, double h, double off, uint64_t i_begin,
+                        uint64_t n, std::vector<double> coef, double p0, double p1, DType dtype,
+                        DivMode div, int grid, uintptr_t table, int table_n, uintptr_t partials,
+                        uintptr_t s, const std::string& tile) {
+    const RiemannParams p = make_params(integrand, a, h, off, i_begin, n, coef, p0, p1, tile);
+    launch_riemann_partials(p, dtype, div, {grid, kRiemannBlock}, ptr<const double>(table),
+                            table_n, ptr<double>(partials), stream(s));
+  };
   m.def("launch_riemann_partials",
-        [](int integrand, double a, double h, double off, uint64_t i_begin, uint64_t n,
-           std::vector<double> coef, double p0, double p1, DType dtype, DivMode div, int grid,
-           uintptr_t table, int table_n, uintptr_t partials, uintptr_t s) {
-          const RiemannParams p = make_params(integrand, a, h, off, i_begin, n, coef, p0, p1);
-          launch_riemann_partials(p, dtype, div, {grid, kRiemannBlock}, ptr<const double>(table),
-                                  table_n, ptr<double>(partials), stream(s));
+        [partials_fn](int integrand, double a, double h, double off, uint64_t i_begin, uint64_t n,
+                      std::vector<double> coef, double p0, double p1, DType dtype, DivMode div,
+                      int grid, uintptr_t table, int table_n, uintptr_t partials, uintptr_t s) {
+          partials_fn(integrand, a, h, off, i_begin, n, coef, p0, p1, dtype, div, grid, table,
+                      table_n, partials, s, "auto");
         });
+  m.def("launch_riemann_partials", partials_fn);
   m.def("riemann_tile_len",
         [](int integrand, double a, double h, double off, uint64_t i_begin, uint64_t n,
            std::vector<double> coef, double p0, double p1, DType dtype, DivMode div) {
           return riemann_tile_len(make_params(integrand, a, h, off, i_begin, n, coef, p0, p1),
                                   dtype, div);
         });
+  m.def("riemann_tile_len",
+        [](int integrand, double a, double h, double off, uint64_t i_begin, uint64_t n,
+           std::vector<double> coef, double p0, double p1, DType dtype, DivMode div,
+           const std::string& tile) {
+          return riemann_tile_len(
+              make_params(integrand, a, h, off, i_begin, n, coef, p0, p1, tile), dtype, div);
+        });
+  m.attr("PI4_LONG_TILE") = kSeriesHalfSpanLong * 2;
+  m.def("series_ok_long", &series_ok_long);
   m.def("riemann_effective_div",
         [](int integrand, double a, double h, double off, uint64_t i_begin, uint64_t n,
            std::vector<double> coef, double p0, double p1, DType dtype, DivMode div) {
@@ -457,27 +478,47 @@
   m.attr("FAST_TRIG_MAX_N") = kFastTrigMaxN;
   m.attr("PI4_SERIES_MAX_X") = kPi4SeriesMaxX;
   m.attr("PI4_F32_SERIES_MAX_X") = kPi4SeriesMaxXF32;
+  auto fused_fn = [](int integrand, double a, double h, double off, uint64_t i_begin, uint64_t n,
+                     std::vector<double> coef, double p0, double p1, DType dtype, DivMode div,
+                     int grid, uintptr_t table, int table_n, uintptr_t partials, uintptr_t ticket,
+                     double scale, uintptr_t out, uintptr_t s, const std::string& tile) {
+    const RiemannParams p = make_params(integrand, a, h, off, i_begin, n, coef, p0, p1, tile);
+    launch_riemann_fused(p, dtype, div, {grid, kRiemannBlock}, ptr<const double>(table), table_n,
+                         ptr<double>(partials), ptr<unsigned>(ticket), scale, ptr<double>(out),
+                         stream(s));
+  };
   m.def("launch_riemann_fused",
-        [](int integrand, double a, double h, double off, uint64_t i_begin, uint64_t n,
-           std::vector<double> coef, double p0, double p1, DType dtype, DivMode div, int grid,
-           uintptr_t table, int table_n, uintptr_t partials, uintptr_t ticket, double scale,
-           uintptr_t out, uintptr_t s) {
-          const RiemannParams p = make_params(integrand, a, h, off, i_begin, n, coef, p0, p1);
-          launch_riemann_fused(p, dtype, div, {grid, kRiemannBlock}, ptr<const double>(table),
-                               table_n, ptr<double>(partials), ptr<unsigned>(ticket), scale,
-                               ptr<double>(out), stream(s));
+        [fused_fn](int integrand, double a, double h, double off, uint64_t i_begin, uint64_t n,
+                   std::vector<double> coef, double p0, double p1, DType dtype, DivMode div,
+                   int grid, uintptr_t table, int table_n, uintptr_t partials, uintptr_t ticket,
+                   double scale, uintptr_t out, uintptr_t s) {
+          fused_fn(integrand, a, h, off, i_begin, n, coef, p0, p1, dtype, div, grid, table,
+                   table_n, partials, ticket, scale, out, s, "auto");
         });
+  m.def("launch_riemann_fused", fused_fn);
+  auto points_fn = [](int integrand, double a, double h, double off, uint64_t i_begin,
+                      uint64_t n, std::vector<double> coef, double p0, double p1, DivMode div,
+                      uintptr_t table, int table_n, uintptr_t out, uintptr_t s,
+                      const std::string& tile) {
+    const RiemannParams p = make_params(integrand, a, h, off, i_begin, n, coef, p0, p1, tile);
+    launch_riemann_point_values(p, div, ptr<const double>(table), table_n, ptr<double>(out),
+                                stream(s));
+  };
   m.def("launch_riemann_point_values",
-        [](int integrand, double a, double h, double off, uint64_t i_begin, uint64_t n,
-           std::vector<double> coef, double p0, double p1, DivMode div, uintptr_t table,
-           int table_n, uintptr_t out, uintptr_t s) {
-          const RiemannParams p = make_params(integrand, a, h, off, i_begin, n, coef, p0, p1);
-          launch_riemann_point_values(p, div, ptr<const double>(table), table_n, ptr<double>(out),
-                                      stream(s));
+        [points_fn](int integrand, double a, double h, double off, uint64_t i_begin, uint64_t n,
+                    std::vector<double> coef, double p0, double p1, DivMode div, uintptr_t table,
+                    int table_n, uintptr_t out, uintptr_t s) {
+          points_fn(integrand, a, h, off, i_begin, n, coef, p0, p1, div, table, table_n, out, s,
+                    "auto");
         });
+  m.def("launch_riemann_point_values", points_fn);
   m.def("launch_pi4_recip_narrow", [](uintptr_t d, uint64_t n, uintptr_t out, uintptr_t s) {
     launch_pi4_recip_narrow(ptr<const double>(d), n, ptr<double>(out), stream(s));
   });
+  m.def("launch_pk_modifier_check",
+        [](uintptr_t ac, uint64_t n, float ka, float kb, uintptr_t out, uintptr_t s) {
+          launch_pk_modifier_check(ptr<const float>(ac), n, ka, kb, ptr<float>(out), stream(s));
+        });
   m.def("launch_pi4_recip_narrow_f32", [](uintptr_t d, uint64_t n, uintptr_t out, uintptr_t s) {
     launch_pi4_recip_narrow_f32(ptr<const float>(d), n, ptr<float>(out), stream(s));
   });
diff --git a/csrc/runtime/integrator.cpp b/csrc/runtime/integrator.cpp
--- a/csrc/runtime/integrator.cpp
+++ b/csrc/runtime/integrator.cpp
@@ -49,6 +49,10 @@
   for (size_t i = 0; i < cfg.coef.size(); ++i) params_.coef[i] = cfg.coef[i];
   params_.p0 = cfg.p0;
   params_.p1 = cfg.p1;
+  params_.tile = tile_form_of(cfg.tile);
+  long_tile_ = pi4_tile_long(params_, cfg.dtype, miint::effective_div(params_, cfg.div, cfg.dtype),
+                             std::getenv("MIINT_PI4_TILE"), kPi4LongTileAuto);
+  params_.tile = long_tile_ ? kTileLong : kTileShort;
   scale_ = params_.h * integrand_scale(cfg.integrand);
 
   const DeviceInfo info = device_info(device);
@@ -64,8 +68,10 @@
   shape_.grid = static_cast<int>(std::min<uint64_t>(static_cast<uint64_t>(shape_.grid), need));
   if (cfg.grid <= 0) {
     const uint64_t cus = static_cast<uint64_t>(info.num_cus);
+    const uint64_t tl4 = long_tile_ ? std::min<uint64_t>(tl, 2 * kSeriesHalfSpan) : tl;
+    const uint64_t tiles4 = (params_.n + tl4 - 1) / tl4;
     const uint64_t four =
-        std::max<uint64_t>(cus, (tiles + 4 * bs - 1) / (4 * bs));
+        std::max<uint64_t>(cus, (tiles4 + 4 * bs - 1) / (4 * bs));
     uint64_t g = std::min<uint64_t>(static_cast<uint64_t>(shape_.grid), four);
     if (g > cus) g -= g % cus;
     shape_.grid = static_cast<int>(g);
diff --git a/cuda_v_mpi_amd/integrate.py b/cuda_v_mpi_amd/integrate.py
--- a/cuda_v_mpi_amd/integrate.py
+++ b/cuda_v_mpi_amd/integrate.py
@@ -53,7 +53,7 @@
                  slice_of: tuple[int, int] | None = None, step_streams: int = 0,
                  block: int = 256, multistep: bool = True, close: str = "auto",
                  allreduce_to_host: bool = True, timeout_s: float = 300.0,
-                 work: str = "auto", queue_wg_per_cu: int = 0, **spec_kw):
+                 work: str = "auto", queue_wg_per_cu: int = 0, tile: str = "auto", **spec_kw):
         spec = integrands.get(integrand, **spec_kw) if isinstance(integrand, str) else integrand
         if a is not None or b is not None:
             spec = dataclasses.replace(spec, a=spec.a if a is None else a,
@@ -102,6 +102,9 @@
                 raise ValueError("work must be auto|static|queue")
             cfg.work = work
             cfg.queue_wg_per_cu = queue_wg_per_cu
+            if tile not in ("auto", "short", "long"):
+                raise ValueError("tile must be auto|short|long")
+            cfg.tile = tile
             cfg.allreduce_to_host = allreduce_to_host
             cfg.timeout_s = timeout_s
             if slice_of is not None:
diff --git a/cuda_v_mpi_amd/ops/kernels.py b/cuda_v_mpi_amd/ops/kernels.py
--- a/cuda_v_mpi_amd/ops/kernels.py
+++ b/cuda_v_mpi_amd/ops/kernels.py
@@ -42,7 +42,7 @@
 
 def riemann_partials(spec: IntegrandSpec, n: int, rule: str = "left", dtype: str = "fp64",
                      div: str = "series_exact", grid: int | None = None, i_begin: int = 0,
-                     n_local: int | None = None) -> torch.Tensor:
+                     n_local: int | None = None, tile: str = "auto") -> torch.Tensor:
     m = native()
     dev = _device()
     grid = grid or default_grid()
@@ -55,7 +55,7 @@
                               list(spec.coef), spec.p0, spec.p1, dt, dv, grid,
                               table.data_ptr() if table is not None else 0,
                               table.numel() if table is not None else 0,
-                              partials.data_ptr(), _stream())
+                              partials.data_ptr(), _stream(), tile)
     return partials
 
 
@@ -98,7 +98,8 @@
 def riemann(spec: IntegrandSpec, n: int, rule: str = "left", dtype: str = "fp64",
             div: str = "series_exact", grid: int | None = None, i_begin: int = 0,
             n_local: int | None = None, out: torch.Tensor | None = None,
-            workspace: FusedWorkspace | None = None, fused: bool = True) -> torch.Tensor:
+            workspace: FusedWorkspace | None = None, fused: bool = True,
+            tile: str = "auto") -> torch.Tensor:
     m = native()
     dev = _device()
     grid = grid or (workspace.grid if workspace else default_grid())
@@ -107,7 +108,7 @@
     scale = h * spec.scale
     out = torch.empty(1, dtype=torch.float64, device=dev) if out is None else out
     if not fused:
-        p = riemann_partials(spec, n, rule, dtype, div, grid, i_begin, n_local)
+        p = riemann_partials(spec, n, rule, dtype, div, grid, i_begin, n_local, tile)
         return finalize(p, scale, out)
     ws = workspace or FusedWorkspace(grid, dev)
     table = _table_tensor(spec, dev)
@@ -117,12 +118,13 @@
                            table.data_ptr() if table is not None else 0,
                            table.numel() if table is not None else 0,
                            ws.partials.data_ptr(), ws.ticket.data_ptr(), scale, out.data_ptr(),
-                           _stream())
+                           _stream(), tile)
     return out
 
 
 def point_values(spec: IntegrandSpec, n: int, rule: str = "left", div: str = "series",
-                 i_begin: int = 0, n_local: int | None = None) -> torch.Tensor:
+                 i_begin: int = 0, n_local: int | None = None,
+                 tile: str = "auto") -> torch.Tensor:
     m = native()
     dev = _device()
     n_local = n if n_local is None else n_local
@@ -133,8 +135,18 @@
                                   getattr(m.DivMode, div),
                                   table.data_ptr() if table is not None else 0,
                                   table.numel() if table is not None else 0,
-                                  out.data_ptr(), _stream())
-    return out
+                                  out.data_ptr(), _stream(), tile)
+    return out
+
+
+def riemann_tile_len(spec: IntegrandSpec, n: int, rule: str = "left", dtype: str = "fp64",
+                     div: str = "series_exact", i_begin: int = 0, n_local: int | None = None,
+                     tile: str = "auto") -> int:
+    m = native()
+    n_local = n if n_local is None else n_local
+    dt, dv = _enums(dtype, div)
+    return m.riemann_tile_len(spec.native_id, spec.a, (spec.b - spec.a) / n, _RULE_OFF[rule],
+                              i_begin, n_local, list(spec.coef), spec.p0, spec.p1, dt, dv, tile)
 
 
 def pi4_recip_narrow(d: torch.Tensor) -> torch.Tensor:
@@ -143,6 +155,16 @@
     out = torch.empty_like(d)
     launch = native().launch_pi4_recip_narrow_f32 if f32 else native().launch_pi4_recip_narrow
     launch(d.data_ptr(), d.numel(), out.data_ptr(), _stream())
+    return out
+
+
+def pk_modifier_check(ac: torch.Tensor, ka: float, kb: float) -> torch.Tensor:
+    _check(ac, dtype=torch.float32, name="ac")
+    if ac.dim() != 2 or ac.shape[1] != 4:
+        raise ValueError("ac must be n x 4")
+    out = torch.empty((ac.shape[0], 16), dtype=torch.float32, device=ac.device)
+    native().launch_pk_modifier_check(ac.data_ptr(), ac.shape[0], float(ka), float(kb),
+                                      out.data_ptr(), _stream())
     return out
 
 
diff --git a/cuda_v_mpi_amd/utils/pi4_truth.py b/cuda_v_mpi_amd/utils/pi4_truth.py
--- a/cuda_v_mpi_amd/utils/pi4_truth.py
+++ b/cuda_v_mpi_amd/utils/pi4_truth.py
@@ -15,6 +15,7 @@
 
 SCALE = 4.0
 TILE64 = 384
+TILE64_LONG = 1536
 TILE32 = 192
 TILE_PER_SAMPLE = 32
 HALF_SPAN_H = 2.0e-6
@@ -36,13 +37,24 @@
                 "fp32acc-series")
 
 
+LONG_PATH = "fp64-series_exact-long"
+
+
+def _series(path: str) -> bool:
+    return path in SERIES_PATHS or path == LONG_PATH
+
+
+def long_tile_admitted(h: float) -> bool:
+    return 0.0 < abs(h) and (TILE64_LONG // 2) * abs(h) <= HALF_SPAN_H
+
+
 def tile_len(path: str) -> int:
     return {"fp64-series_exact": TILE64, "fp64-series": TILE64, "fp32-series": TILE32,
-            "fp32acc-series": TILE32}.get(path, TILE_PER_SAMPLE)
+            "fp32acc-series": TILE32, LONG_PATH: TILE64_LONG}.get(path, TILE_PER_SAMPLE)
 
 
 def seed_residual(path: str) -> float:
-    return {"fp64-series_exact": EM_RAW64, "fp64-series": EM_RAW64,
+    return {"fp64-series_exact": EM_RAW64, "fp64-series": EM_RAW64, LONG_PATH: EM_RAW64,
             "fp64-series_direct": 2.0 ** -45}.get(path, EM_NEWTON32)
 
 
@@ -184,7 +196,7 @@
 
 def tile_anchor(g: Geometry, path: str, tile: int = 0) -> float:
     T = tile_len(path)
-    mid = path in ("fp64-series_exact", "fp64-series", "fp32-series", "fp32acc-series")
+    mid = path in ("fp64-series_exact", "fp64-series", "fp32-series", "fp32acc-series", LONG_PATH)
     ib = base_index(g) + float(tile * T) + (0.5 * (T - 1) if mid else 0.0)
     return fma64(ib, g.h, g.a)
 
@@ -222,7 +234,7 @@
         return {"xm": _fr(xm), "h": _fr(hf), "dm": _fr(fma32(xm, xm, np.float32(1.0)))}
     if path == "fp64-series":
         return {"xm": _fr(xa), "h": Fraction(g.h), "dm": _fr(fma64(xa, xa, 1.0))}
-    if path == "fp64-series_exact":
+    if path in ("fp64-series_exact", LONG_PATH):
         return {"xm": _fr(xa), "h": Fraction(g.h), "dm": 1 + _fr(xa) ** 2}
     raise ValueError(path)
 
@@ -377,6 +389,12 @@
         rel = (off_unit + 4.0 * U64 * EM_RAW64 + 2.0 * U64 * E
                + 2.0 * U64 * (192.0 * h) ** 2 / 3.0 + 2.2e-18 + 96.0 * U32 * E * E
                + 2.0 * U64 * E + E ** 3 / (1.0 - E)) * (1.0 + 2.0 * E) + 2.0 * U64
+    elif path == LONG_PATH:
+        off_unit = 2.0 ** -54 if g.x_abs_max + 768.0 * h > 1.0 else 0.0
+        squares = 2.0 * E * 5.0 * U32 * E + U32 * E * E + 2.0 * E * 651.0 * h * h
+        rel = (off_unit + 4.0 * U64 * EM_RAW64 + 2.0 * U64 * E
+               + 2.0 * U64 * (768.0 * h) ** 2 / 3.0 + squares + 384.0 * U32 * E * E
+               + 2.0 * U64 * E + E ** 3 / (1.0 - E)) * (1.0 + 2.0 * E) + 2.0 * U64
     elif path == "fp64-series_direct":
         rel = (19.0 * U64 * E + 33.0 * U64 * E * E + E ** 3 / (1.0 - E)) * (1.0 + 2.0 * E) + U64
     else:
@@ -386,7 +404,7 @@
 
 def defn_truth_rel(path: str, g: Geometry) -> float:
     h = abs(g.h)
-    if path == "fp64-series_exact":
+    if path in ("fp64-series_exact", LONG_PATH):
         rel = coord_rel(g, 1)
     elif path == "fp64-series":
         rel = coord_rel(g, 1) + U64 * (1.0 + 2.0 * 192.0 * h)
@@ -423,7 +441,7 @@
 def tile_truth_bound(path: str, g: Geometry, true_tile_sum: float) -> float:
     S = abs(true_tile_sum)
     T = tile_len(path)
-    if path in SERIES_PATHS:
+    if _series(path):
         rel = tile_defn_rel(path, g) + defn_truth_rel(path, g)
     elif path == "fp64-ieee":
         rel = ieee_rel(path, g) + 32.0 * U64
@@ -442,7 +460,7 @@
 def launch_sum_bound(path: str, g: Geometry, true_total: float, grid: int, block: int = BLOCK) -> float:
     T = tile_len(path)
     S = abs(true_total)
-    if path in SERIES_PATHS:
+    if _series(path):
         rel = tile_defn_rel(path, g) + defn_truth_rel(path, g)
     elif path == "fp64-ieee":
         rel = ieee_rel(path, g) + 32.0 * U64
```

Result: faster. 33940 billion, median of 6 (+6.0%).
